# paultsw/wavenet-speech

Hardware: AMD Instinct MI355X
Metric: samples/sec fwd+bwd, 256-ch 30-block WaveNet @16k seq (higher is better)
Workload: dtype f32; 1 GPU; BASELINE.json configs[2]: WaveNet 256 ch, 30 blocks (3 x dilation 1..512), k=2, seq_len 16000, batch 16 per GPU, f32, full step (fwd+bwd+grad all-reduce+Adam); channels=256, blocks=30, seq_len=16000, batch_per_gpu=16, global_batch=16, parallelism=dp1, params=16037632, input=dense one-hot, init=reference

## Files before the change

include/wavenet_amd.h:

```cpp
#ifndef WAVENET_AMD_H
#define WAVENET_AMD_H

#include <stddef.h>

#ifdef __cplusplus
extern "C" {
#endif

#define WN_VERSION 300

typedef void* wn_stream_t;

typedef enum wn_status {
    WN_OK = 0,
    WN_ERR_BAD_SHAPE = -1,
    WN_ERR_UNSUPPORTED = -2,
    WN_ERR_NULL = -3,
    WN_ERR_HIP = -4,
    WN_ERR_WORKSPACE = -5
} wn_status;

#define WN_MAX_TAPS 8
#define WN_MAX_CHANNELS 1024

typedef struct wn_block_shape {
    int batch;
    int length;
    int in_channels;
    int out_channels;
    int skip_rows;
    int kernel_width;
    int dilation;
    int causal;
    int ld;
    int halo;
} wn_block_shape;

typedef struct wn_block_params {
    float* w_tanh;
    float* b_tanh;
    float* w_sigmoid;
    float* b_sigmoid;
    float* w_res;
    float* b_res;
    float* w_skip;
    float* b_skip;
    float* w_proj;
    float* b_proj;
} wn_block_params;

int wn_version(void);
const char* wn_strerror(int status);
const char* wn_last_hip_error(void);

int wn_round_up(int x, int multiple);
int wn_autopad(int kernel_width, int dilation);
int wn_tap_offsets(int kernel_width, int dilation, int causal, int* off );
int wn_series_layout(int length, int max_abs_offset, int* ld, int* halo);
size_t wn_series_floats(int batch, int channels, int ld);

size_t wn_block_packed_bytes(const wn_block_shape* s);
int wn_block_pack(const wn_block_shape* s, const wn_block_params* p, void* packed, wn_stream_t stream);

int wn_block_forward(const wn_block_shape* s, const void* packed, const float* x,
                     float* r_out, float* skip, int skip_accumulate,
                     float* sg, float* z, wn_stream_t stream);

#define WN_MAX_STACK_GROUP 32
typedef struct wn_skipsum_shape {
    int batch, length, skip_rows, nblocks, ld, halo;
    int channels[WN_MAX_STACK_GROUP];
} wn_skipsum_shape;
size_t wn_skipsum_packed_bytes(const wn_skipsum_shape* s);
int wn_skipsum_pack(const wn_skipsum_shape* s, const float* const* w_skip, const float* bias_total ,
                    void* packed, wn_stream_t stream);
int wn_skipsum_forward(const wn_skipsum_shape* s, const void* packed, const float* const* z, float* skip,
                       int accumulate, wn_stream_t stream);

int wn_block_backward_data(const wn_block_shape* s, const void* packed,
                           const float* dr, const float* dskip, const float* z, const float* sg,
                           float* da, float* dg, float* dx, wn_stream_t stream);

size_t wn_block_wgrad_workspace_bytes(const wn_block_shape* s);
int wn_block_backward_weights(const wn_block_shape* s, const float* x, const float* z,
                              const float* da, const float* dg, const float* dr, const float* dskip,
                              const wn_block_params* grads, void* workspace, size_t workspace_bytes,
                              wn_stream_t stream);

typedef struct wn_conv_shape {
    int batch, length, in_channels, out_channels, kernel_width, dilation, causal, ld, halo;
} wn_conv_shape;
size_t wn_conv_packed_bytes(const wn_conv_shape* s);
int wn_conv_pack(const wn_conv_shape* s, const float* weight , const float* bias ,
                 void* packed, wn_stream_t stream);
int wn_conv_forward(const wn_conv_shape* s, const void* packed, const float* x, float* y, wn_stream_t stream);
int wn_conv_backward_data(const wn_conv_shape* s, const void* packed, const float* dy, float* dx, wn_stream_t stream);
size_t wn_conv_wgrad_workspace_bytes(const wn_conv_shape* s);
int wn_conv_backward_weights(const wn_conv_shape* s, const float* x, const float* dy,
                             float* dweight, float* dbias ,
                             void* workspace, size_t workspace_bytes, wn_stream_t stream);

size_t wn_nll_partials(int batch, int length);
int wn_nll_forward(const float* logits, const long long* target, float* lse, float* partial, int* bad_targets,
                   int batch, int classes, int length, wn_stream_t stream);
int wn_nll_backward(const float* logits, const long long* target, const float* lse, const float* gscale, float* dlogits,
                    int batch, int classes, int length, wn_stream_t stream);

int wn_embed_forward(const long long* levels, const float* weight, const float* bias, float* y, int batch, int length,
                     int classes, int out_channels, int kernel_width, int* bad_levels, wn_stream_t stream);
size_t wn_synth_workspace_bytes(int batch, int length);
int wn_synth_bases(unsigned long long seed, int batch, int nbases, long long* bases, wn_stream_t stream);
int wn_synth_signal(const long long* bases, int batch, int nbases, int length, int upsampling, const double* means,
                    const double* stdvs, unsigned long long seed, const double* noise , double* picoamps,
                    void* workspace, size_t workspace_bytes, int* bad_bases , wn_stream_t stream);
int wn_synth_quantize(const double* picoamps, const void* workspace, size_t workspace_bytes, int batch, int length,
                      int num_levels, const double* edges, long long* levels, float* one_hot ,
                      wn_stream_t stream);

size_t wn_ctc_workspace_bytes(int batch, int classes, int length, int max_label_len);
int wn_ctc_loss(const float* logits, const long long* labels, const long long* label_lengths,
                const long long* input_lengths , int batch, int classes, int length, int max_label_len,
                int blank, float* nll, float* dlogits , void* workspace, size_t workspace_bytes,
                int* bad_labels , wn_stream_t stream);

size_t wn_ctc_decode_workspace_bytes(int batch, int classes, int length, int beam_width);
int wn_ctc_greedy_decode(const float* x, long long sb, long long sc, long long st, const long long* input_lengths ,
                         int batch, int classes, int length, int blank, int* labels, int* frames , int* lengths,
                         int* bad , wn_stream_t stream);
int wn_ctc_beam_decode(const float* x, long long sb, long long sc, long long st, int input_kind,
                       const long long* input_lengths , int batch, int classes, int length, int blank,
                       int beam_width, int* labels, int* frames , int* lengths, float* scores, void* workspace,
                       size_t workspace_bytes, int* bad , wn_stream_t stream);

size_t wn_ctc_align_workspace_bytes(int batch, int classes, int length, int max_label_len);
int wn_ctc_align(const float* x, long long sb, long long sc, long long st, int input_kind, const long long* labels,
                 const long long* label_lengths, const long long* input_lengths , int batch, int classes,
                 int length, int max_label_len, int blank, int* states, int* frame_labels ,
                 int* spans , float* score, void* workspace, size_t workspace_bytes, int* bad ,
                 wn_stream_t stream);

size_t wn_pair_align_workspace_bytes(int batch, int max_ref_len, int max_query_len);
int wn_pair_align(const int* ref, long long ref_stride, const int* ref_lengths, const int* query, long long query_stride,
                  const int* query_lengths, int batch, int max_ref_len, int max_query_len, int match, int mismatch,
                  int gap_open, int gap_extend, int end_gaps_free, int* score, int* stats ,
                  unsigned char* ops , int* ops_len , void* workspace, size_t workspace_bytes,
                  int* bad , wn_stream_t stream);

enum { WN_DWELL_FIXED = 0, WN_DWELL_UNIFORM = 1, WN_DWELL_GAMMA = 2 };
size_t wn_reads_workspace_bytes(int batch, int max_bases);
int wn_reads_plan(unsigned long long seed, int batch, int min_bases, int max_bases, int window, int dwell_model, double dwell_p0,
                  double dwell_p1, double dwell_p2, int max_dwell, const int* base_lengths_in ,
                  const int* bases_in , const int* dwell_in , int* base_lengths, int* bases,
                  int* dwell, int* starts, int* signal_lengths, void* workspace, size_t workspace_bytes,
                  int* bad , int* clamped , wn_stream_t stream);
int wn_reads_signal(const int* base_lengths, const int* starts, const int* signal_lengths, const void* workspace,
                    size_t workspace_bytes, int batch, int max_bases, int window, int ld, const double* means,
                    const double* stdvs, unsigned long long seed, const double* noise , float* signal,
                    int* sample_kmer , int* clipped_lengths , int* bad ,
                    wn_stream_t stream);

int wn_chunk_gather(const void* signal, int signal_is_int16, int batch, int ld, const int* signal_lengths,
                    const float* scale , const float* shift , const int* plan, int n_chunks,
                    int chunk, float* out, int* bad , wn_stream_t stream);
int wn_chunk_stitch(const float* y, long long stride_n, long long stride_c, long long stride_t, int y_frames, const int* plan,
                    int n_chunks, int classes, int batch, float* out, long long out_stride_b, long long out_stride_c,
                    int out_frames, const int* frame_lengths, int* bad , wn_stream_t stream);

size_t wn_read_select_workspace_bytes(int batch, int K, int signal_is_int16, int has_center);
int wn_read_select(const void* signal, int signal_is_int16, int batch, int ld, const int* signal_lengths, const int* ranks, int K,
                   const float* center , float* out, void* workspace, size_t workspace_bytes,
                   int* bad , wn_stream_t stream);

int wn_ctc_base_quality(const float* x, long long sb, long long sc, long long st, int input_kind,
                        const long long* input_lengths , const int* labels, long long labels_stride,
                        const int* frames, long long frames_stride, const int* lengths, int batch, int classes, int length,
                        int max_labels, int blank, int stat , float qscale, float qbias,
                        float* error , unsigned char* qual , int* dwell ,
                        float* read_error , int* bad , wn_stream_t stream);

int wn_quality_profile(const unsigned char* ops, long long ops_stride, const int* ops_len, const int* ref, long long ref_stride,
                       const int* ref_lengths, const int* query, long long query_stride, const int* query_lengths,
                       const unsigned char* qual , long long qual_stride, const int* dwell ,
                       long long dwell_stride, int batch, int max_ref_len, int max_query_len, int max_ops, int classes,
                       int count_ends, long long* q_counts , long long* dwell_counts ,
                       long long* confusion , int* read_counts ,
                       unsigned char* outcome , int* ref_index , int* bad ,
                       wn_stream_t stream);

typedef enum wn_precision { WN_F32 = 0, WN_F16X3 = 1, WN_F16 = 2, WN_BF16 = 3 } wn_precision;

int wn_hseries_layout(int length, int max_abs_offset, int* ld, int* halo);
size_t wn_hseries_bytes(int precision, int batch, int channels, int ld);
float wn_hseries_residual_scale(void);
int wn_hseries_load(int precision, const float* dense, void* series, int batch, int channels, int length, int ld, int halo,
                    float scale, const float* dyn_scale, unsigned* overflow_flag, wn_stream_t stream);

size_t wn_hblock_packed_bytes(const wn_block_shape* s, int precision);
int wn_hblock_pack(const wn_block_shape* s, int precision, const wn_block_params* p, void* packed, wn_stream_t stream);
int wn_hblock_pack_checked(const wn_block_shape* s, int precision, const wn_block_params* p, void* packed, unsigned* overflow_flag,
                           wn_stream_t stream);
int wn_hblock_forward_is_fused(const wn_block_shape* s, int precision);
int wn_hblock_forward(const wn_block_shape* s, int precision, const void* packed, const void* x, void* r_out,
                      float* skip_dense, int skip_accumulate, void* sg, void* z, unsigned* overflow_flag,
                      wn_stream_t stream);
size_t wn_hskipsum_packed_bytes(const wn_skipsum_shape* s, int precision);
int wn_hskipsum_pack(const wn_skipsum_shape* s, int precision, const float* const* w_skip, const float* bias_total,
                     void* packed, wn_stream_t stream);
int wn_hskipsum_forward(const wn_skipsum_shape* s, int precision, const void* packed, const void* const* z,
                        float* skip_dense, int accumulate, wn_stream_t stream);
int wn_hblock_backward_data(const wn_block_shape* s, int precision, const void* packed, const void* dr, const void* dskip,
                            const void* z, const void* sg, void* da, void* dg, void* dx, float* dx_dense,
                            const float* dyn_inv_scale, unsigned* overflow_flag, wn_stream_t stream);
size_t wn_hblock_wgrad_workspace_bytes(const wn_block_shape* s, int precision);
int wn_hblock_backward_weights(const wn_block_shape* s, int precision, const void* x, const void* z, const void* da,
                               const void* dg, const void* dr, const void* dskip, const wn_block_params* grads,
                               const float* dyn_inv_scale, void* workspace, size_t workspace_bytes, wn_stream_t stream);

int wn_hskipsum_forward_series(const wn_skipsum_shape* s, int precision, const void* packed, const void* const* z, void* out_series,
                               float out_scale, float leaky_slope, unsigned* overflow_flag, wn_stream_t stream);
int wn_hconv_forward_series(const wn_conv_shape* s, int precision, const void* packed, const void* x, void* y_series, float out_scale,
                            float leaky_slope, unsigned* overflow_flag, wn_stream_t stream);
int wn_hconv_backward_data_series(const wn_conv_shape* s, int precision, const void* packed, const void* dy, const void* act,
                                  float leaky_slope, void* dx_series, unsigned* overflow_flag, wn_stream_t stream);

int wn_hblock_backward_pair_is_fused(const wn_block_shape* upper, const wn_block_shape* lower, int precision);
int wn_hblock_backward_pair(const wn_block_shape* upper, const void* packed_upper, const wn_block_shape* lower, const void* packed_lower,
                            int precision, const void* dr_upper, const void* da_upper, const void* dg_upper, const void* dskip,
                            const void* z_lower, const void* sg_lower, void* dx_upper, void* da_lower, void* dg_lower,
                            unsigned* overflow_flag, wn_stream_t stream);
int wn_hblock_backward_input(const wn_block_shape* s, int precision, const void* packed, const void* dr, const void* da, const void* dg,
                             void* dx, float* dx_dense, const float* dyn_inv_scale, const void* x_act, float leaky_slope,
                             unsigned* overflow_flag, wn_stream_t stream);

int wn_hblock_backward_data_masked(const wn_block_shape* s, int precision, const void* packed, const void* dr, const void* dskip,
                                   const void* z, const void* sg, void* da, void* dg, void* dx, const void* x_act, float leaky_slope,
                                   unsigned* overflow_flag, wn_stream_t stream);

int wn_hfeature_forward(int precision, const float* x, const float* weight, const float* bias, void* y_series, int batch, int length,
                        int features, int kernel_width, int ld, int halo, float out_scale, float leaky_slope, unsigned* overflow_flag,
                        wn_stream_t stream);
size_t wn_hfeature_wgrad_workspace_bytes(int batch, int length, int features, int kernel_width);
int wn_hfeature_backward_weights(int precision, const float* x, const void* dy_series, float dy_scale, float* dweight, float* dbias,
                                 int batch, int length, int features, int kernel_width, int ld, int halo, const float* dyn_inv_scale,
                                 void* workspace, size_t workspace_bytes, wn_stream_t stream);
int wn_hseries_load_pooled(int precision, const float* dense, void* series, int batch, int channels, int length, int pool, int ld, int halo,
                           float scale, const float* dyn_scale, unsigned* overflow_flag, wn_stream_t stream);
int wn_series_load_pooled(const float* dense, float* series, int batch, int channels, int length, int pool, int ld, int halo,
                          wn_stream_t stream);
int wn_pool_backward(const float* dpooled, float* dx, int batch, int channels, int length, int pool, wn_stream_t stream);
int wn_grad_scale(const float* x, long long count, float target, float* scale_and_inverse, unsigned* accumulator, wn_stream_t stream);

int wn_hblocks_wgrad_group_max(const wn_block_shape* s, int precision);
size_t wn_hblocks_wgrad_workspace_bytes(const wn_block_shape* shapes, int nblocks, int precision);
int wn_hblocks_backward_weights(const wn_block_shape* shapes, int nblocks, int precision, const void* const* x, const void* const* z,
                                const void* const* da, const void* const* dg, const void* const* dr, const void* const* dskip,
                                const wn_block_params* grads, const float* dyn_inv_scale, void* workspace, size_t workspace_bytes,
                                wn_stream_t stream);

typedef struct wn_mem_range { const void* base; size_t bytes; } wn_mem_range;
size_t wn_hstack_pack_table_bytes(int nblocks);
int wn_hstack_pack_table_build(const wn_block_shape* shapes, const wn_block_params* params, int nblocks, int precision,
                               int with_skipsum, const wn_mem_range* dynamic, int ndynamic, void* table_host, size_t table_bytes,
                               size_t* block_offsets, size_t* skipsum_offsets, size_t* packed_total, int* njobs,
                               int* launch_blocks);
int wn_hstack_pack_run(const void* table_dev, int nblocks, int njobs, int launch_blocks, const void* const* dynamic_bases,
                       int ndynamic, void* packed, unsigned* overflow_flag , wn_stream_t stream);

int wn_prof_enable(int on);
int wn_prof_reset(void);
int wn_prof_collect(void);
int wn_prof_num_kernels(void);
const char* wn_prof_kernel_name(int kernel_class);
int wn_prof_get(int kernel_class, double* total_ms, long long* launches, double* flops);

size_t wn_hconv_packed_bytes(const wn_conv_shape* s, int precision);
int wn_hconv_pack(const wn_conv_shape* s, int precision, const float* weight , const float* bias ,
                  float input_scale, void* packed, wn_stream_t stream);
int wn_hconv_forward(const wn_conv_shape* s, int precision, const void* packed, const void* x, float* y_dense, wn_stream_t stream);
int wn_hconv_backward_data(const wn_conv_shape* s, int precision, const void* packed, const void* dy, float* dx_dense,
                           const float* dyn_inv_scale , wn_stream_t stream);
size_t wn_hconv_wgrad_workspace_bytes(const wn_conv_shape* s, int precision);
int wn_hconv_backward_weights(const wn_conv_shape* s, int precision, const void* x, const void* dy, float input_scale,
                              float* dweight, float* dbias , const float* dyn_inv_scale ,
                              void* workspace, size_t workspace_bytes, wn_stream_t stream);

#ifdef __cplusplus
}
#endif
#endif
```

wavenet_speech_amd/_lib.py:

```python
import ctypes
import os
from ctypes import POINTER, Structure, c_char_p, c_double, c_float, c_int, c_longlong, c_size_t, c_ulonglong, c_void_p

_HERE = os.path.dirname(os.path.abspath(__file__))
LIB_PATH = os.path.join(_HERE, "libwavenet_amd.so")

MAX_TAPS = 8
MAX_CHANNELS = 1024

c_float_p = c_void_p


class BlockShape(Structure):
    _fields_ = [("batch", c_int), ("length", c_int), ("in_channels", c_int), ("out_channels", c_int),
                ("skip_rows", c_int), ("kernel_width", c_int), ("dilation", c_int), ("causal", c_int),
                ("ld", c_int), ("halo", c_int)]


class BlockParams(Structure):
    _fields_ = [(n, c_float_p) for n in ("w_tanh", "b_tanh", "w_sigmoid", "b_sigmoid", "w_res", "b_res",
                                         "w_skip", "b_skip", "w_proj", "b_proj")]


MAX_STACK_GROUP = 32


class SkipSumShape(Structure):
    _fields_ = [("batch", c_int), ("length", c_int), ("skip_rows", c_int), ("nblocks", c_int), ("ld", c_int),
                ("halo", c_int), ("channels", c_int * MAX_STACK_GROUP)]


class MemRange(Structure):
    _fields_ = [("base", c_void_p), ("bytes", c_size_t)]


class ConvShape(Structure):
    _fields_ = [("batch", c_int), ("length", c_int), ("in_channels", c_int), ("out_channels", c_int),
                ("kernel_width", c_int), ("dilation", c_int), ("causal", c_int), ("ld", c_int), ("halo", c_int)]


SIGNATURES = {
    "wn_version": (c_int, []),
    "wn_strerror": (c_char_p, [c_int]),
    "wn_last_hip_error": (c_char_p, []),
    "wn_round_up": (c_int, [c_int, c_int]),
    "wn_autopad": (c_int, [c_int, c_int]),
    "wn_tap_offsets": (c_int, [c_int, c_int, c_int, POINTER(c_int)]),
    "wn_series_layout": (c_int, [c_int, c_int, POINTER(c_int), POINTER(c_int)]),
    "wn_series_floats": (c_size_t, [c_int, c_int, c_int]),
    "wn_block_packed_bytes": (c_size_t, [POINTER(BlockShape)]),
    "wn_block_pack": (c_int, [POINTER(BlockShape), POINTER(BlockParams), c_void_p, c_void_p]),
    "wn_block_forward": (c_int, [POINTER(BlockShape), c_void_p, c_float_p, c_float_p, c_float_p, c_int,
                                 c_float_p, c_float_p, c_void_p]),
    "wn_skipsum_packed_bytes": (c_size_t, [POINTER(SkipSumShape)]),
    "wn_skipsum_pack": (c_int, [POINTER(SkipSumShape), POINTER(c_void_p), c_float_p, c_void_p, c_void_p]),
    "wn_skipsum_forward": (c_int, [POINTER(SkipSumShape), c_void_p, POINTER(c_void_p), c_float_p, c_int, c_void_p]),
    "wn_block_backward_data": (c_int, [POINTER(BlockShape), c_void_p, c_float_p, c_float_p, c_float_p, c_float_p,
                                       c_float_p, c_float_p, c_float_p, c_void_p]),
    "wn_block_wgrad_workspace_bytes": (c_size_t, [POINTER(BlockShape)]),
    "wn_block_backward_weights": (c_int, [POINTER(BlockShape), c_float_p, c_float_p, c_float_p, c_float_p, c_float_p,
                                          c_float_p, POINTER(BlockParams), c_void_p, c_size_t, c_void_p]),
    "wn_conv_packed_bytes": (c_size_t, [POINTER(ConvShape)]),
    "wn_conv_pack": (c_int, [POINTER(ConvShape), c_float_p, c_float_p, c_void_p, c_void_p]),
    "wn_conv_forward": (c_int, [POINTER(ConvShape), c_void_p, c_float_p, c_float_p, c_void_p]),
    "wn_conv_backward_data": (c_int, [POINTER(ConvShape), c_void_p, c_float_p, c_float_p, c_void_p]),
    "wn_conv_wgrad_workspace_bytes": (c_size_t, [POINTER(ConvShape)]),
    "wn_conv_backward_weights": (c_int, [POINTER(ConvShape), c_float_p, c_float_p, c_float_p, c_float_p,
                                         c_void_p, c_size_t, c_void_p]),
    "wn_hseries_layout": (c_int, [c_int, c_int, POINTER(c_int), POINTER(c_int)]),
    "wn_hseries_bytes": (c_size_t, [c_int, c_int, c_int, c_int]),
    "wn_hseries_residual_scale": (c_float, []),
    "wn_hseries_load": (c_int, [c_int, c_float_p, c_void_p, c_int, c_int, c_int, c_int, c_int, c_float, c_float_p, c_void_p,
                                c_void_p]),
    "wn_hblock_packed_bytes": (c_size_t, [POINTER(BlockShape), c_int]),
    "wn_hblock_pack": (c_int, [POINTER(BlockShape), c_int, POINTER(BlockParams), c_void_p, c_void_p]),
    "wn_hblock_pack_checked": (c_int, [POINTER(BlockShape), c_int, POINTER(BlockParams), c_void_p, c_void_p, c_void_p]),
    "wn_hblock_forward_is_fused": (c_int, [POINTER(BlockShape), c_int]),
    "wn_hblock_backward_pair_is_fused": (c_int, [POINTER(BlockShape), POINTER(BlockShape), c_int]),
    "wn_hblock_backward_pair": (c_int, [POINTER(BlockShape), c_void_p, POINTER(BlockShape), c_void_p, c_int, c_void_p, c_void_p, c_void_p,
                                        c_void_p, c_void_p, c_void_p, c_void_p, c_void_p, c_void_p, c_void_p, c_void_p]),
    "wn_hblock_backward_input": (c_int, [POINTER(BlockShape), c_int, c_void_p, c_void_p, c_void_p, c_void_p, c_void_p, c_float_p, c_float_p,
                                         c_void_p, c_float, c_void_p, c_void_p]),
    "wn_hblock_forward": (c_int, [POINTER(BlockShape), c_int, c_void_p, c_void_p, c_void_p, c_float_p, c_int, c_void_p,
                                  c_void_p, c_void_p, c_void_p]),
    "wn_hskipsum_packed_bytes": (c_size_t, [POINTER(SkipSumShape), c_int]),
    "wn_hskipsum_pack": (c_int, [POINTER(SkipSumShape), c_int, POINTER(c_void_p), c_float_p, c_void_p, c_void_p]),
    "wn_hskipsum_forward": (c_int, [POINTER(SkipSumShape), c_int, c_void_p, POINTER(c_void_p), c_float_p, c_int, c_void_p]),
    "wn_hblock_backward_data": (c_int, [POINTER(BlockShape), c_int, c_void_p, c_void_p, c_void_p, c_void_p, c_void_p,
                                        c_void_p, c_void_p, c_void_p, c_float_p, c_float_p, c_void_p, c_void_p]),
    "wn_hblock_backward_data_masked": (c_int, [POINTER(BlockShape), c_int, c_void_p, c_void_p, c_void_p, c_void_p, c_void_p, c_void_p,
                                               c_void_p, c_void_p, c_void_p, c_float, c_void_p, c_void_p]),
    "wn_hfeature_forward": (c_int, [c_int, c_float_p, c_float_p, c_float_p, c_void_p, c_int, c_int, c_int, c_int, c_int, c_int, c_float,
                                    c_float, c_void_p, c_void_p]),
    "wn_hfeature_wgrad_workspace_bytes": (c_size_t, [c_int, c_int, c_int, c_int]),
    "wn_hfeature_backward_weights": (c_int, [c_int, c_float_p, c_void_p, c_float, c_float_p, c_float_p, c_int, c_int, c_int, c_int, c_int,
                                             c_int, c_float_p, c_void_p, c_size_t, c_void_p]),
    "wn_hseries_load_pooled": (c_int, [c_int, c_float_p, c_void_p, c_int, c_int, c_int, c_int, c_int, c_int, c_float, c_float_p, c_void_p,
                                       c_void_p]),
    "wn_series_load_pooled": (c_int, [c_float_p, c_float_p, c_int, c_int, c_int, c_int, c_int, c_int, c_void_p]),
    "wn_grad_scale": (c_int, [c_float_p, c_longlong, c_float, c_float_p, c_void_p, c_void_p]),
    "wn_pool_backward": (c_int, [c_float_p, c_float_p, c_int, c_int, c_int, c_int, c_void_p]),
    "wn_hskipsum_forward_series": (c_int, [POINTER(SkipSumShape), c_int, c_void_p, POINTER(c_void_p), c_void_p, c_float, c_float, c_void_p,
                                           c_void_p]),
    "wn_hconv_forward_series": (c_int, [POINTER(ConvShape), c_int, c_void_p, c_void_p, c_void_p, c_float, c_float, c_void_p, c_void_p]),
    "wn_hconv_backward_data_series": (c_int, [POINTER(ConvShape), c_int, c_void_p, c_void_p, c_void_p, c_float, c_void_p, c_void_p,
                                              c_void_p]),
    "wn_hblocks_wgrad_group_max": (c_int, [POINTER(BlockShape), c_int]),
    "wn_hblocks_wgrad_workspace_bytes": (c_size_t, [POINTER(BlockShape), c_int, c_int]),
    "wn_hblocks_backward_weights": (c_int, [POINTER(BlockShape), c_int, c_int, POINTER(c_void_p), POINTER(c_void_p), POINTER(c_void_p),
                                            POINTER(c_void_p), POINTER(c_void_p), POINTER(c_void_p), POINTER(BlockParams), c_float_p,
                                            c_void_p, c_size_t, c_void_p]),
    "wn_hstack_pack_table_bytes": (c_size_t, [c_int]),
    "wn_hstack_pack_table_build": (c_int, [POINTER(BlockShape), POINTER(BlockParams), c_int, c_int, c_int, POINTER(MemRange), c_int,
                                           c_void_p, c_size_t, POINTER(c_size_t), POINTER(c_size_t), POINTER(c_size_t),
                                           POINTER(c_int), POINTER(c_int)]),
    "wn_hstack_pack_run": (c_int, [c_void_p, c_int, c_int, c_int, POINTER(c_void_p), c_int, c_void_p, c_void_p, c_void_p]),
    "wn_hblock_wgrad_workspace_bytes": (c_size_t, [POINTER(BlockShape), c_int]),
    "wn_hblock_backward_weights": (c_int, [POINTER(BlockShape), c_int, c_void_p, c_void_p, c_void_p, c_void_p, c_void_p,
                                           c_void_p, POINTER(BlockParams), c_float_p, c_void_p, c_size_t, c_void_p]),
    "wn_hconv_packed_bytes": (c_size_t, [POINTER(ConvShape), c_int]),
    "wn_hconv_pack": (c_int, [POINTER(ConvShape), c_int, c_float_p, c_float_p, c_float, c_void_p, c_void_p]),
    "wn_hconv_forward": (c_int, [POINTER(ConvShape), c_int, c_void_p, c_void_p, c_float_p, c_void_p]),
    "wn_hconv_backward_data": (c_int, [POINTER(ConvShape), c_int, c_void_p, c_void_p, c_float_p, c_float_p, c_void_p]),
    "wn_hconv_wgrad_workspace_bytes": (c_size_t, [POINTER(ConvShape), c_int]),
    "wn_hconv_backward_weights": (c_int, [POINTER(ConvShape), c_int, c_void_p, c_void_p, c_float, c_float_p, c_float_p, c_float_p,
                                          c_void_p, c_size_t, c_void_p]),
    "wn_embed_forward": (c_int, [c_void_p, c_float_p, c_float_p, c_float_p, c_int, c_int, c_int, c_int, c_int, c_void_p, c_void_p]),
    "wn_synth_workspace_bytes": (c_size_t, [c_int, c_int]),
    "wn_synth_bases": (c_int, [c_ulonglong, c_int, c_int, c_void_p, c_void_p]),
    "wn_synth_signal": (c_int, [c_void_p, c_int, c_int, c_int, c_int, c_void_p, c_void_p, c_ulonglong, c_void_p, c_void_p,
                                c_void_p, c_size_t, c_void_p, c_void_p]),
    "wn_synth_quantize": (c_int, [c_void_p, c_void_p, c_size_t, c_int, c_int, c_int, c_void_p, c_void_p, c_void_p, c_void_p]),
    "wn_ctc_workspace_bytes": (c_size_t, [c_int, c_int, c_int, c_int]),
    "wn_ctc_loss": (c_int, [c_float_p, c_void_p, c_void_p, c_void_p, c_int, c_int, c_int, c_int, c_int, c_float_p, c_float_p,
                            c_void_p, c_size_t, c_void_p, c_void_p]),
    "wn_ctc_decode_workspace_bytes": (c_size_t, [c_int, c_int, c_int, c_int]),
    "wn_ctc_greedy_decode": (c_int, [c_float_p, c_longlong, c_longlong, c_longlong, c_void_p, c_int, c_int, c_int, c_int, c_void_p,
                                     c_void_p, c_void_p, c_void_p, c_void_p]),
    "wn_ctc_beam_decode": (c_int, [c_float_p, c_longlong, c_longlong, c_longlong, c_int, c_void_p, c_int, c_int, c_int, c_int, c_int,
                                   c_void_p, c_void_p, c_void_p, c_float_p, c_void_p, c_size_t, c_void_p, c_void_p]),
    "wn_ctc_align_workspace_bytes": (c_size_t, [c_int, c_int, c_int, c_int]),
    "wn_ctc_align": (c_int, [c_float_p, c_longlong, c_longlong, c_longlong, c_int, c_void_p, c_void_p, c_void_p, c_int, c_int, c_int,
                             c_int, c_int, c_void_p, c_void_p, c_void_p, c_float_p, c_void_p, c_size_t, c_void_p, c_void_p]),
    "wn_pair_align_workspace_bytes": (c_size_t, [c_int, c_int, c_int]),
    "wn_pair_align": (c_int, [c_void_p, c_longlong, c_void_p, c_void_p, c_longlong, c_void_p, c_int, c_int, c_int, c_int, c_int, c_int,
                              c_int, c_int, c_void_p, c_void_p, c_void_p, c_void_p, c_void_p, c_size_t, c_void_p, c_void_p]),
    "wn_reads_workspace_bytes": (c_size_t, [c_int, c_int]),
    "wn_reads_plan": (c_int, [c_ulonglong, c_int, c_int, c_int, c_int, c_int, c_double, c_double, c_double, c_int, c_void_p, c_void_p,
                              c_void_p, c_void_p, c_void_p, c_void_p, c_void_p, c_void_p, c_void_p, c_size_t, c_void_p, c_void_p,
                              c_void_p]),
    "wn_reads_signal": (c_int, [c_void_p, c_void_p, c_void_p, c_void_p, c_size_t, c_int, c_int, c_int, c_int, c_void_p, c_void_p,
                                c_ulonglong, c_void_p, c_void_p, c_void_p, c_void_p, c_void_p, c_void_p]),
    "wn_chunk_gather": (c_int, [c_void_p, c_int, c_int, c_int, c_void_p, c_void_p, c_void_p, c_void_p, c_int, c_int, c_void_p,
                                c_void_p, c_void_p]),
    "wn_chunk_stitch": (c_int, [c_void_p, c_longlong, c_longlong, c_longlong, c_int, c_void_p, c_int, c_int, c_int, c_void_p,
                                c_longlong, c_longlong, c_int, c_void_p, c_void_p, c_void_p]),
    "wn_read_select_workspace_bytes": (c_size_t, [c_int, c_int, c_int, c_int]),
    "wn_read_select": (c_int, [c_void_p, c_int, c_int, c_int, c_void_p, c_void_p, c_int, c_void_p, c_void_p, c_void_p, c_size_t,
                               c_void_p, c_void_p]),
    "wn_ctc_base_quality": (c_int, [c_float_p, c_longlong, c_longlong, c_longlong, c_int, c_void_p, c_void_p, c_longlong, c_void_p,
                                    c_longlong, c_void_p, c_int, c_int, c_int, c_int, c_int, c_int, c_float, c_float, c_float_p,
                                    c_void_p, c_void_p, c_float_p, c_void_p, c_void_p]),
    "wn_quality_profile": (c_int, [c_void_p, c_longlong, c_void_p, c_void_p, c_longlong, c_void_p, c_void_p, c_longlong, c_void_p,
                                   c_void_p, c_longlong, c_void_p, c_longlong, c_int, c_int, c_int, c_int, c_int, c_int, c_void_p,
                                   c_void_p, c_void_p, c_void_p, c_void_p, c_void_p, c_void_p, c_void_p]),
    "wn_nll_partials":(c_size_t, [c_int, c_int]),
    "wn_nll_forward": (c_int, [c_float_p, c_void_p, c_float_p, c_float_p, c_void_p, c_int, c_int, c_int, c_void_p]),
    "wn_nll_backward": (c_int, [c_float_p, c_void_p, c_float_p, c_float_p, c_float_p, c_int, c_int, c_int, c_void_p]),
    "wn_prof_enable": (c_int, [c_int]),
    "wn_prof_reset": (c_int, []),
    "wn_prof_collect": (c_int, []),
    "wn_prof_num_kernels": (c_int, []),
    "wn_prof_kernel_name": (c_char_p, [c_int]),
    "wn_prof_get": (c_int, [c_int, POINTER(c_double), POINTER(c_longlong), POINTER(c_double)]),
}

_lib = None


def load():
    global _lib
    if _lib is not None:
        return _lib
    if not os.path.exists(LIB_PATH):
        raise RuntimeError(
            "wavenet_speech_amd: %s not found. Build it with `python __graft_entry__.py` or "
            "`make -C wavenet_speech_amd/csrc` (hipcc, --offload-arch=gfx950). There is no CPU fallback." % LIB_PATH)
    lib = ctypes.CDLL(LIB_PATH)
    for name, (res, args) in SIGNATURES.items():
        fn = getattr(lib, name)
        fn.restype = res
        fn.argtypes = args
    if lib.wn_version() < 300:
        raise RuntimeError("libwavenet_amd.so too old")
    _lib = lib
    return lib


def check(status, what):
    if status != 0:
        lib = load()
        msg = lib.wn_strerror(status).decode()
        hip = lib.wn_last_hip_error().decode()
        raise RuntimeError("%s failed: %s%s" % (what, msg, (" [" + hip + "]") if hip and status == -4 else ""))


def tap_offsets(k, d, causal):
    off = (c_int * k)()
    check(load().wn_tap_offsets(k, d, int(bool(causal)), off), "wn_tap_offsets")
    return list(off)


def series_layout(length, max_abs_offset):
    ld, halo = c_int(), c_int()
    check(load().wn_series_layout(length, max_abs_offset, ctypes.byref(ld), ctypes.byref(halo)), "wn_series_layout")
    return ld.value, halo.value


PRECISIONS = {"f32": 0, "f16x3": 1, "f16": 2, "bf16": 3}


def hseries_layout(length, max_abs_offset):
    ld, halo = c_int(), c_int()
    check(load().wn_hseries_layout(length, max_abs_offset, ctypes.byref(ld), ctypes.byref(halo)), "wn_hseries_layout")
    return ld.value, halo.value


def profile_read():
    lib = load()
    check(lib.wn_prof_collect(), "wn_prof_collect")
    out = {}
    for i in range(lib.wn_prof_num_kernels()):
        ms, n, fl = c_double(), c_longlong(), c_double()
        check(lib.wn_prof_get(i, ctypes.byref(ms), ctypes.byref(n), ctypes.byref(fl)), "wn_prof_get")
        out[lib.wn_prof_kernel_name(i).decode()] = (ms.value, n.value, fl.value)
    return out
```

wavenet_speech_amd/csrc/wn_api.hip:

```cpp
#include <hip/hip_runtime.h>

#include <algorithm>
#include <cstdio>
#include <cstdlib>
#include <cstdint>
#include <cstring>
#include <mutex>
#include <string>
#include <vector>

#include "../../include/wavenet_amd.h"
#include "wn_kernels.h"

using namespace wn;

#ifdef WN_STAMPS
namespace wn { extern int g_debug_kc; }
#endif

namespace {

thread_local std::string g_hip_err;

int hip_fail(hipError_t e, const char* what) {
    g_hip_err = std::string(what) + ": " + hipGetErrorString(e);
    return WN_ERR_HIP;
}
#define WN_HIP(call, what)                                  \
    do {                                                    \
        hipError_t e__ = (call);                            \
        if (e__ != hipSuccess) return hip_fail(e__, what);  \
    } while (0)

}
namespace wn {
int hip_fail_shared(hipError_t e, const char* what) { return hip_fail(e, what); }
}
namespace {
inline int rup(int x, int m) { return (x + m - 1) / m * m; }
inline int cdiv(int a, int b) { return (a + b - 1) / b; }
inline int tiles32(int c) { return cdiv(c, 32); }
inline int cp8(int c) { return rup(c, 8); }
inline int pick_mt(int ntiles) { return ntiles > 2 ? 4 : (ntiles == 2 ? 2 : 1); }
inline size_t align256(size_t b) { return (b + 255) / 256 * 256; }

enum KernelClass {
    KC_PACK = 0, KC_GATE_GEMM, KC_OUT_GEMM, KC_DZ_GEMM, KC_DX_GEMM, KC_WGRAD, KC_WGRAD_REDUCE,
    KC_CONV_FWD, KC_CONV_BWD_DATA, KC_SKIP_GEMM, KC_HLOAD, KC_HGATE, KC_HRES, KC_HDZ, KC_HDX, KC_HSKIP, KC_HWGRAD, KC_EMBED,
    KC_SYNTH, KC_CTC, KC_HFUSED, KC_HCONV_FWD, KC_HCONV_BWD_DATA, KC_HCOL_DZ, KC_HCOL_DX, KC_HCOL_DXDZ, KC_HCOL_SKIP,
    KC_COUNT
};
const char* const kKernelNames[KC_COUNT] = {
    "pack_kernel", "series_gemm_kernel<gate>", "series_gemm_kernel<res>", "series_gemm_kernel<dz,dgate>",
    "series_gemm_kernel<dx>", "wgrad_kernel", "wgrad_reduce_kernel", "series_gemm_kernel<conv_fwd>",
    "series_gemm_kernel<conv_bwd_data>", "series_gemm_kernel<skips_sum>", "hload_kernel", "hgemm_kernel<gate>",
    "hgemm_kernel<res>", "hgemm_kernel<dz,dgate>", "hgemm_kernel<dx>", "hgemm_kernel<skips_sum>", "hwgrad_kernel",
    "embed_kernel", "synth_kernel", "ctc_kernel", "hfused_fwd_kernel",
    "hgemm_kernel<conv_fwd>", "hgemm_kernel<conv_bwd_data>", "hcol_kernel<dz,dgate>", "hcol_kernel<dx>", "hcol2_kernel<dx+dz>", "hcol_kernel<skips_sum>"};

struct ProfRec { int kc; hipEvent_t e0, e1; double flops; };
struct Prof {
    std::mutex mu;
    bool on = false;
    std::vector<ProfRec> pending;
    std::vector<hipEvent_t> pool;
    double ms[KC_COUNT] = {0};
    long long n[KC_COUNT] = {0};
    double flops[KC_COUNT] = {0};
} g_prof;

struct ProfScope {
    bool active = false;
    ProfRec rec{};
    hipStream_t st;
    ProfScope(int kc, double flops, hipStream_t s) : st(s) {
#ifdef WN_STAMPS
        wn::g_debug_kc = kc;
#endif
        std::lock_guard<std::mutex> lk(g_prof.mu);
        if (!g_prof.on) return;
        auto get = [&]() {
            hipEvent_t e;
            if (!g_prof.pool.empty()) { e = g_prof.pool.back(); g_prof.pool.pop_back(); return e; }
            if (hipEventCreate(&e) != hipSuccess) return (hipEvent_t) nullptr;
            return e;
        };
        rec.kc = kc; rec.flops = flops; rec.e0 = get(); rec.e1 = get();
        if (!rec.e0 || !rec.e1) return;
        active = hipEventRecord(rec.e0, st) == hipSuccess;
    }
    ~ProfScope() {
        if (!active) return;
        (void)hipEventRecord(rec.e1, st);
        std::lock_guard<std::mutex> lk(g_prof.mu);
        g_prof.pending.push_back(rec);
    }
};

}
namespace wn {
struct ProfScopeShared {
    void* impl;
    ProfScopeShared(int kc, double flops, hipStream_t st);
    ~ProfScopeShared();
};
ProfScopeShared::ProfScopeShared(int kc, double flops, hipStream_t st) : impl(new ProfScope(kc, flops, st)) {}
ProfScopeShared::~ProfScopeShared() { delete static_cast<ProfScope*>(impl); }
}
namespace {
int tap_offsets(int k, int d, int causal, int* off) {
    const int p = causal ? (k - 1) * d : wn_autopad(k, d);
    for (int j = 0; j < k; ++j) off[j] = j * d - p;
    return 0;
}

int check_layout(int B, int L, int ld, int halo, int max_abs_off) {
    if (B <= 0 || L <= 0) return WN_ERR_BAD_SHAPE;
    if (halo < 0 || (halo & 3) || (ld & 3)) return WN_ERR_BAD_SHAPE;
    if (halo < max_abs_off) return WN_ERR_BAD_SHAPE;
    if (ld < 2 * halo + rup(L, kColTile)) return WN_ERR_BAD_SHAPE;
    if ((double)WN_MAX_CHANNELS * (double)ld * 4.0 >= 4294967296.0) return WN_ERR_UNSUPPORTED;
    return WN_OK;
}

int check_block(const wn_block_shape* s, int* off) {
    if (!s) return WN_ERR_NULL;
    if (s->in_channels <= 0 || s->out_channels <= 0 || s->skip_rows <= 0 || s->dilation <= 0) return WN_ERR_BAD_SHAPE;
    if (s->kernel_width < 1) return WN_ERR_BAD_SHAPE;
    if (s->kernel_width > WN_MAX_TAPS) return WN_ERR_UNSUPPORTED;
    if (s->in_channels > WN_MAX_CHANNELS || s->out_channels > WN_MAX_CHANNELS || s->skip_rows > WN_MAX_CHANNELS)
        return WN_ERR_UNSUPPORTED;
    tap_offsets(s->kernel_width, s->dilation, s->causal, off);
    int mx = 0;
    for (int j = 0; j < s->kernel_width; ++j) mx = std::max(mx, std::abs(off[j]));
    return check_layout(s->batch, s->length, s->ld, s->halo, mx);
}

struct GemmPlan {
    int MT = 1, nslab = 0, nseg = 0;
    int seg_nkb[kMaxSeg] = {0};
    long long slab_woff[kMaxSlab] = {0};
    int slab_nseg[kMaxSlab] = {0}, slab_row0[kMaxSlab] = {0}, slab_dst[kMaxSlab] = {0}, slab_boff[kMaxSlab] = {0};
    long long wfloats = 0;
    int bfloats = 0;
    void add_slab(int nseg_used, int row0, int dst) {
        const int s = nslab++;
        long long kb = 0;
        for (int i = 0; i < nseg_used; ++i) kb += seg_nkb[i];
        slab_woff[s] = wfloats;
        slab_nseg[s] = nseg_used;
        slab_row0[s] = row0;
        slab_dst[s] = dst;
        slab_boff[s] = bfloats;
        wfloats += kb * MT * 256;
        bfloats += MT * 32;
    }
    size_t bytes() const { return align256((size_t)wfloats * 4) + align256((size_t)bfloats * 4); }
};

struct BlockPlan {
    GemmPlan fa, fb, ka, kb;
    int fb_first_skip_slab = 0;
    size_t off_fa = 0, off_fb = 0, off_ka = 0, off_kb = 0, total = 0;
};

BlockPlan plan_block(const wn_block_shape* s) {
    BlockPlan p;
    static const int mt2 = getenv("WN_MT2_MASK") ? atoi(getenv("WN_MT2_MASK")) : 0;
    const int Ci = s->in_channels, Co = s->out_channels, Ms = s->skip_rows, k = s->kernel_width;
    {
        GemmPlan& g = p.fa;
        const int pairs = tiles32(Co);
        g.MT = (pairs >= 2 && !(mt2 & 1)) ? 4 : 2;
        g.nseg = k;
        for (int j = 0; j < k; ++j) g.seg_nkb[j] = cp8(Ci) / 8;
        const int ns = cdiv(2 * pairs, g.MT);
        for (int i = 0; i < ns; ++i) g.add_slab(k, i * (g.MT / 2) * 32, 0);
    }
    {
        GemmPlan& g = p.fb;
        const int rt = tiles32(Co), st = tiles32(Ms);
        g.MT = pick_mt(std::max(rt, st));
        if ((mt2 & 2) && g.MT == 4) g.MT = 2;
        g.nseg = 2;
        g.seg_nkb[0] = cp8(Co) / 8;
        g.seg_nkb[1] = cp8(Ci) / 8;
        for (int i = 0; i < cdiv(rt, g.MT); ++i) g.add_slab(2, i * g.MT * 32, 0);
        p.fb_first_skip_slab = g.nslab;
        for (int i = 0; i < cdiv(st, g.MT); ++i) g.add_slab(1, i * g.MT * 32, 1);
    }
    {
        GemmPlan& g = p.ka;
        const int zt = tiles32(Co);
        g.MT = pick_mt(zt);
        static const int dz_mt = getenv("WN_DZ_MT") ? atoi(getenv("WN_DZ_MT")) : 2;
        if (dz_mt == 2 && zt >= 2) g.MT = 2;
        g.nseg = 2;
        g.seg_nkb[0] = cp8(Ms) / 8;
        g.seg_nkb[1] = cp8(Co) / 8;
        for (int i = 0; i < cdiv(zt, g.MT); ++i) g.add_slab(2, i * g.MT * 32, 0);
    }
    {
        GemmPlan& g = p.kb;
        const int xt = tiles32(Ci);
        g.MT = pick_mt(xt);
        if ((mt2 & 4) && g.MT == 4) g.MT = 2;
        g.nseg = 2 * k + 1;
        for (int j = 0; j < 2 * k + 1; ++j) g.seg_nkb[j] = cp8(Co) / 8;
        for (int i = 0; i < cdiv(xt, g.MT); ++i) g.add_slab(2 * k + 1, i * g.MT * 32, 0);
    }
    p.off_fa = 0;
    p.off_fb = p.off_fa + p.fa.bytes();
    p.off_ka = p.off_fb + p.fb.bytes();
    p.off_kb = p.off_ka + p.ka.bytes();
    p.total = p.off_kb + p.kb.bytes();
    return p;
}

inline const float* plan_w(const void* packed, size_t off) { return reinterpret_cast<const float*>((const char*)packed + off); }
inline const float* plan_b(const void* packed, size_t off, const GemmPlan& g) {
    return reinterpret_cast<const float*>((const char*)packed + off + align256((size_t)g.wfloats * 4));
}

void fill_pack_common(PackArgs& a, const GemmPlan& g, void* packed, size_t off) {
    std::memset(&a, 0, sizeof(a));
    a.nslab = g.nslab;
    a.MT = g.MT;
    for (int i = 0; i < kMaxSeg; ++i) a.seg_nkb[i] = g.seg_nkb[i];
    for (int i = 0; i < g.nslab; ++i) {
        a.slab_woff[i] = g.slab_woff[i];
        a.slab_nseg[i] = g.slab_nseg[i];
        a.slab_boff[i] = g.slab_boff[i];
    }
    a.wpacked = reinterpret_cast<float*>((char*)packed + off);
    a.bias = reinterpret_cast<float*>((char*)packed + off + align256((size_t)g.wfloats * 4));
    a.total = g.wfloats;
}

void fill_gemm_common(GemmArgs& a, const GemmPlan& g, const void* packed, size_t off, int first_slab, int nslab,
                      int B, int L, int ld, int halo) {
    std::memset(&a, 0, sizeof(a));
    a.wpacked = plan_w(packed, off);
    a.bias = plan_b(packed, off, g);
    a.nslab = nslab;
    for (int i = 0; i < nslab; ++i) {
        GemmSlab& s = a.slab[i];
        s.woff = g.slab_woff[first_slab + i];
        s.nseg = g.slab_nseg[first_slab + i];
        s.dst = g.slab_dst[first_slab + i];
        s.row0 = g.slab_row0[first_slab + i];
        s.boff = g.slab_boff[first_slab + i];
    }
    a.B = B; a.L = L; a.ld = ld; a.halo = halo;
    a.tiles_per_row = cdiv(L, kColTile);
    a.ncol = B * a.tiles_per_row;
}

inline void set_seg(GemmArgs& a, int i, const float* base, int c, int off, int nkb) {
    a.seg[i].base = base; a.seg[i].cp = cp8(c); a.seg[i].off = off; a.seg[i].nkb = nkb;
}

inline PackSrc mk_src(const float* p, int rows, int cols, int sr, int sc) {
    PackSrc s; s.ptr = p; s.rows = rows; s.cols = cols; s.stride_r = sr; s.stride_c = sc; return s;
}

struct WgradPlan {
    int WT = 1, npair = 0, ntile_total = 0, nsplit = 1;
    int Mp[kMaxPair], Np[kMaxPair], mt[kMaxPair], nt[kMaxPair], tile0[kMaxPair], rs_off[kMaxPair];
    long long slab_off[kMaxPair];
    long long slab_floats = 0;
    int rs_floats = 0;
    void add(int M, int N) {
        const int T = 64 * WT, i = npair++;
        mt[i] = cdiv(M, T); nt[i] = cdiv(N, T);
        Mp[i] = mt[i] * T; Np[i] = nt[i] * T;
        tile0[i] = ntile_total; ntile_total += mt[i] * nt[i];
        slab_off[i] = slab_floats; slab_floats += (long long)Mp[i] * Np[i];
        rs_off[i] = rs_floats; rs_floats += Mp[i];
    }
    void finish(int nchunk) {
        nsplit = std::max(1, 512 / std::max(1, ntile_total));
        nsplit = std::min(nsplit, std::max(1, nchunk));
        if (nsplit >= 16) nsplit = nsplit / 8 * 8;
    }
    bool xcd_map() const { return nsplit % 8 == 0; }
    size_t bytes() const { return (size_t)nsplit * (size_t)(slab_floats + rs_floats) * 4; }
};
inline int pick_wt(int maxdim) { return maxdim > 128 ? 4 : (maxdim > 64 ? 2 : 1); }

}


int wn_version(void) { return WN_VERSION; }

const char* wn_strerror(int status) {
    switch (status) {
        case WN_OK: return "ok";
        case WN_ERR_BAD_SHAPE: return "bad shape or series layout (dimension <= 0, ld/halo not multiples of 4, halo smaller than the taps reach, or ld too small)";
        case WN_ERR_UNSUPPORTED: return "unsupported configuration (kernel_width > WN_MAX_TAPS or channels > WN_MAX_CHANNELS)";
        case WN_ERR_NULL: return "required pointer is NULL";
        case WN_ERR_HIP: return "HIP runtime / kernel launch error (see wn_last_hip_error)";
        case WN_ERR_WORKSPACE: return "workspace too small";
    }
    return "unknown wn_status";
}

const char* wn_last_hip_error(void) { return g_hip_err.c_str(); }

int wn_round_up(int x, int multiple) { return multiple > 0 ? rup(x, multiple) : x; }

int wn_autopad(int k, int d) {
    const int total = (k - 1) * d;
    return (total % 2 == 1) ? (total - 1) / 2 + 1 : total / 2;
}

int wn_tap_offsets(int k, int d, int causal, int* off) {
    if (!off) return WN_ERR_NULL;
    if (k < 1 || d < 1) return WN_ERR_BAD_SHAPE;
    return tap_offsets(k, d, causal, off);
}

int wn_series_layout(int length, int max_abs_offset, int* ld, int* halo) {
    if (!ld || !halo) return WN_ERR_NULL;
    if (length <= 0 || max_abs_offset < 0) return WN_ERR_BAD_SHAPE;
    *halo = rup(max_abs_offset, 4);
    *ld = 2 * (*halo) + rup(length, kColTile);
    return WN_OK;
}

size_t wn_series_floats(int batch, int channels, int ld) { return (size_t)batch * cp8(channels) * (size_t)ld; }

size_t wn_block_packed_bytes(const wn_block_shape* s) {
    int off[WN_MAX_TAPS];
    if (check_block(s, off) != WN_OK) return 0;
    return plan_block(s).total;
}

int wn_block_pack(const wn_block_shape* s, const wn_block_params* p, void* packed, wn_stream_t stream) {
    int off[WN_MAX_TAPS];
    int rc = check_block(s, off);
    if (rc != WN_OK) return rc;
    if (!p || !packed || !p->w_tanh || !p->w_sigmoid || !p->w_res || !p->w_skip || !p->w_proj) return WN_ERR_NULL;
    hipStream_t st = (hipStream_t)stream;
    const BlockPlan bp = plan_block(s);
    const int Ci = s->in_channels, Co = s->out_channels, Ms = s->skip_rows, k = s->kernel_width;
    ProfScope prof(KC_PACK, 0.0, st);
    PackArgs a;
    {
        const GemmPlan& g = bp.fa;
        fill_pack_common(a, g, packed, bp.off_fa);
        for (int j = 0; j < k; ++j) {
            a.set[0].seg[j] = mk_src(p->w_tanh + j, Co, Ci, Ci * k, k);
            a.set[1].seg[j] = mk_src(p->w_sigmoid + j, Co, Ci, Ci * k, k);
        }
        a.set[0].bias0 = p->b_tanh; a.set[0].bias_rows = Co;
        a.set[1].bias0 = p->b_sigmoid; a.set[1].bias_rows = Co;
        const int pairs = tiles32(Co);
        for (int sl = 0; sl < g.nslab; ++sl)
            for (int m = 0; m < g.MT; ++m) {
                const int pair = sl * (g.MT / 2) + m / 2;
                a.tile[sl * g.MT + m].set = m & 1;
                a.tile[sl * g.MT + m].row0 = pair < pairs ? 32 * pair : -1;
            }
        WN_HIP(launch_pack(a, st), "pack(gate)");
    }
    {
        const GemmPlan& g = bp.fb;
        fill_pack_common(a, g, packed, bp.off_fb);
        a.set[0].seg[0] = mk_src(p->w_res, Co, Co, Co, 1);
        a.set[0].seg[1] = mk_src(p->w_proj, Co, Ci, Ci, 1);
        a.set[0].bias0 = p->b_res; a.set[0].bias1 = p->b_proj; a.set[0].bias_rows = Co;
        a.set[1].seg[0] = mk_src(p->w_skip, Ms, Co, Co, 1);
        a.set[1].bias0 = p->b_skip; a.set[1].bias_rows = Ms;
        for (int sl = 0; sl < g.nslab; ++sl)
            for (int m = 0; m < g.MT; ++m) {
                const bool skip = sl >= bp.fb_first_skip_slab;
                const int row0 = g.slab_row0[sl] + 32 * m;
                a.tile[sl * g.MT + m].set = skip ? 1 : 0;
                a.tile[sl * g.MT + m].row0 = row0 < (skip ? Ms : Co) ? row0 : -1;
            }
        WN_HIP(launch_pack(a, st), "pack(res+skip)");
    }
    {
        const GemmPlan& g = bp.ka;
        fill_pack_common(a, g, packed, bp.off_ka);
        a.set[0].seg[0] = mk_src(p->w_skip, Co, Ms, 1, Co);
        a.set[0].seg[1] = mk_src(p->w_res, Co, Co, 1, Co);
        for (int sl = 0; sl < g.nslab; ++sl)
            for (int m = 0; m < g.MT; ++m) {
                const int row0 = g.slab_row0[sl] + 32 * m;
                a.tile[sl * g.MT + m].set = 0;
                a.tile[sl * g.MT + m].row0 = row0 < Co ? row0 : -1;
            }
        WN_HIP(launch_pack(a, st), "pack(dz)");
    }
    {
        const GemmPlan& g = bp.kb;
        fill_pack_common(a, g, packed, bp.off_kb);
        for (int j = 0; j < k; ++j) {
            a.set[0].seg[2 * j] = mk_src(p->w_tanh + j, Ci, Co, k, Ci * k);
            a.set[0].seg[2 * j + 1] = mk_src(p->w_sigmoid + j, Ci, Co, k, Ci * k);
        }
        a.set[0].seg[2 * k] = mk_src(p->w_proj, Ci, Co, 1, Ci);
        for (int sl = 0; sl < g.nslab; ++sl)
            for (int m = 0; m < g.MT; ++m) {
                const int row0 = g.slab_row0[sl] + 32 * m;
                a.tile[sl * g.MT + m].set = 0;
                a.tile[sl * g.MT + m].row0 = row0 < Ci ? row0 : -1;
            }
        WN_HIP(launch_pack(a, st), "pack(dx)");
    }
    return WN_OK;
}

int wn_block_forward(const wn_block_shape* s, const void* packed, const float* x, float* r_out, float* skip,
                     int skip_accumulate, float* sg, float* z, wn_stream_t stream) {
    int off[WN_MAX_TAPS];
    int rc = check_block(s, off);
    if (rc != WN_OK) return rc;
    if (!packed || !x || !z) return WN_ERR_NULL;
    hipStream_t st = (hipStream_t)stream;
    const BlockPlan bp = plan_block(s);
    const int Ci = s->in_channels, Co = s->out_channels, Ms = s->skip_rows, k = s->kernel_width;
    const double BL = (double)s->batch * s->length;
    GemmArgs a;
    {
        const GemmPlan& g = bp.fa;
        fill_gemm_common(a, g, packed, bp.off_fa, 0, g.nslab, s->batch, s->length, s->ld, s->halo);
        for (int j = 0; j < k; ++j) set_seg(a, j, x, Ci, off[j], g.seg_nkb[j]);
        a.sg = sg; a.z = z; a.gate_cp = cp8(Co); a.gate_rows = Co;
        ProfScope prof(KC_GATE_GEMM, 2.0 * (2.0 * Co) * (double)(k * Ci) * BL, st);
        WN_HIP(launch_gemm(g.MT, EPI_GATE, a, st), "series_gemm<gate>");
    }
    {
        const GemmPlan& g = bp.fb;
        const double fl_r = 2.0 * Co * (double)(Co + Ci) * BL, fl_s = 2.0 * Ms * (double)Co * BL;
        if (r_out) {
            fill_gemm_common(a, g, packed, bp.off_fb, 0, bp.fb_first_skip_slab, s->batch, s->length, s->ld, s->halo);
            set_seg(a, 0, z, Co, 0, g.seg_nkb[0]);
            set_seg(a, 1, x, Ci, 0, g.seg_nkb[1]);
            a.dst[0].base = r_out; a.dst[0].cp = cp8(Co); a.dst[0].rows = Co; a.dst[0].accumulate = 0;
            ProfScope prof(KC_OUT_GEMM, fl_r, st);
            WN_HIP(launch_gemm(g.MT, EPI_LINEAR, a, st), "series_gemm<res>");
        }
        if (skip) {
            fill_gemm_common(a, g, packed, bp.off_fb, bp.fb_first_skip_slab, g.nslab - bp.fb_first_skip_slab, s->batch,
                             s->length, s->ld, s->halo);
            set_seg(a, 0, z, Co, 0, g.seg_nkb[0]);
            a.dst[1].base = skip; a.dst[1].cp = cp8(Ms); a.dst[1].rows = Ms; a.dst[1].accumulate = skip_accumulate ? 1 : 0;
            ProfScope prof(KC_SKIP_GEMM, fl_s, st);
            WN_HIP(launch_gemm(g.MT, skip_accumulate ? EPI_ACCUM : EPI_LINEAR, a, st), "series_gemm<skip>");
        }
    }
    return WN_OK;
}

int wn_block_backward_data(const wn_block_shape* s, const void* packed, const float* dr, const float* dskip,
                           const float* z, const float* sg, float* da, float* dg, float* dx, wn_stream_t stream) {
    int off[WN_MAX_TAPS];
    int rc = check_block(s, off);
    if (rc != WN_OK) return rc;
    if (!packed || !dskip || !z || !sg || !da || !dg) return WN_ERR_NULL;
    hipStream_t st = (hipStream_t)stream;
    const BlockPlan bp = plan_block(s);
    const int Ci = s->in_channels, Co = s->out_channels, Ms = s->skip_rows, k = s->kernel_width;
    const double BL = (double)s->batch * s->length;
    GemmArgs a;
    {
        const GemmPlan& g = bp.ka;
        fill_gemm_common(a, g, packed, bp.off_ka, 0, g.nslab, s->batch, s->length, s->ld, s->halo);
        a.bias = nullptr;
        set_seg(a, 0, dskip, Ms, 0, g.seg_nkb[0]);
        set_seg(a, 1, dr, Co, 0, g.seg_nkb[1]);
        const int nseg = dr ? 2 : 1;
        for (int i = 0; i < a.nslab; ++i) a.slab[i].nseg = nseg;
        a.z = const_cast<float*>(z); a.sg = const_cast<float*>(sg); a.da = da; a.dg = dg;
        a.gate_cp = cp8(Co); a.gate_rows = Co;
        ProfScope prof(KC_DZ_GEMM, 2.0 * Co * (double)(Ms + (dr ? Co : 0)) * BL, st);
        WN_HIP(launch_gemm(g.MT, EPI_DGATE, a, st), "series_gemm<dz>");
    }
    if (dx) {
        const GemmPlan& g = bp.kb;
        fill_gemm_common(a, g, packed, bp.off_kb, 0, g.nslab, s->batch, s->length, s->ld, s->halo);
        a.bias = nullptr;
        for (int j = 0; j < k; ++j) {
            set_seg(a, 2 * j, da, Co, -off[j], g.seg_nkb[2 * j]);
            set_seg(a, 2 * j + 1, dg, Co, -off[j], g.seg_nkb[2 * j + 1]);
        }
        set_seg(a, 2 * k, dr, Co, 0, g.seg_nkb[2 * k]);
        const int nseg = 2 * k + (dr ? 1 : 0);
        for (int i = 0; i < a.nslab; ++i) a.slab[i].nseg = nseg;
        a.dst[0].base = dx; a.dst[0].cp = cp8(Ci); a.dst[0].rows = Ci; a.dst[0].accumulate = 0;
        ProfScope prof(KC_DX_GEMM, 2.0 * Ci * (double)(2 * k * Co + (dr ? Co : 0)) * BL, st);
        WN_HIP(launch_gemm(g.MT, EPI_LINEAR, a, st), "series_gemm<dx>");
    }
    return WN_OK;
}

namespace {
int check_skipsum(const wn_skipsum_shape* s) {
    if (!s) return WN_ERR_NULL;
    if (s->nblocks < 1 || s->skip_rows <= 0) return WN_ERR_BAD_SHAPE;
    if (s->nblocks > WN_MAX_STACK_GROUP || s->skip_rows > WN_MAX_CHANNELS) return WN_ERR_UNSUPPORTED;
    for (int l = 0; l < s->nblocks; ++l) {
        if (s->channels[l] <= 0) return WN_ERR_BAD_SHAPE;
        if (s->channels[l] > WN_MAX_CHANNELS) return WN_ERR_UNSUPPORTED;
    }
    return check_layout(s->batch, s->length, s->ld, s->halo, 0);
}
GemmPlan plan_skipsum(const wn_skipsum_shape* s) {
    GemmPlan g;
    const int t = tiles32(s->skip_rows);
    g.MT = pick_mt(t);
    g.nseg = s->nblocks;
    for (int l = 0; l < s->nblocks; ++l) g.seg_nkb[l] = cp8(s->channels[l]) / 8;
    for (int i = 0; i < cdiv(t, g.MT); ++i) g.add_slab(s->nblocks, i * g.MT * 32, 0);
    return g;
}
}

size_t wn_skipsum_packed_bytes(const wn_skipsum_shape* s) {
    if (check_skipsum(s) != WN_OK) return 0;
    return plan_skipsum(s).bytes();
}

int wn_skipsum_pack(const wn_skipsum_shape* s, const float* const* w_skip, const float* bias_total, void* packed,
                    wn_stream_t stream) {
    int rc = check_skipsum(s);
    if (rc != WN_OK) return rc;
    if (!w_skip || !packed) return WN_ERR_NULL;
    for (int l = 0; l < s->nblocks; ++l) if (!w_skip[l]) return WN_ERR_NULL;
    hipStream_t st = (hipStream_t)stream;
    const GemmPlan g = plan_skipsum(s);
    ProfScope prof(KC_PACK, 0.0, st);
    PackArgs a;
    fill_pack_common(a, g, packed, 0);
    for (int l = 0; l < s->nblocks; ++l) a.set[0].seg[l] = mk_src(w_skip[l], s->skip_rows, s->channels[l], s->channels[l], 1);
    a.set[0].bias0 = bias_total; a.set[0].bias_rows = s->skip_rows;
    for (int sl = 0; sl < g.nslab; ++sl)
        for (int m = 0; m < g.MT; ++m) {
            const int row0 = g.slab_row0[sl] + 32 * m;
            a.tile[sl * g.MT + m].set = 0;
            a.tile[sl * g.MT + m].row0 = row0 < s->skip_rows ? row0 : -1;
        }
    WN_HIP(launch_pack(a, st), "pack(skipsum)");
    return WN_OK;
}

int wn_skipsum_forward(const wn_skipsum_shape* s, const void* packed, const float* const* z, float* skip, int accumulate,
                       wn_stream_t stream) {
    int rc = check_skipsum(s);
    if (rc != WN_OK) return rc;
    if (!packed || !z || !skip) return WN_ERR_NULL;
    for (int l = 0; l < s->nblocks; ++l) if (!z[l]) return WN_ERR_NULL;
    hipStream_t st = (hipStream_t)stream;
    const GemmPlan g = plan_skipsum(s);
    GemmArgs a;
    fill_gemm_common(a, g, packed, 0, 0, g.nslab, s->batch, s->length, s->ld, s->halo);
    double ksum = 0;
    for (int l = 0; l < s->nblocks; ++l) { set_seg(a, l, z[l], s->channels[l], 0, g.seg_nkb[l]); ksum += s->channels[l]; }
    a.dst[0].base = skip; a.dst[0].cp = cp8(s->skip_rows); a.dst[0].rows = s->skip_rows; a.dst[0].accumulate = accumulate ? 1 : 0;
    ProfScope prof(KC_SKIP_GEMM, 2.0 * s->skip_rows * ksum * (double)s->batch * s->length, st);
    WN_HIP(launch_gemm(g.MT, accumulate ? EPI_ACCUM : EPI_LINEAR, a, st), "series_gemm<skipsum>");
    return WN_OK;
}

namespace {
struct PairSpec { const float* A; int a_rows; const float* Bm; int b_rows; int off; int rowsum;
                  float* w; int sm, sn; float* b0; float* b1; };

int run_wgrad(const std::vector<PairSpec>& ps, int maxdim, int B, int L, int ld, int halo, void* workspace,
              size_t workspace_bytes, bool dry, size_t* need, int kc, hipStream_t st) {
    WgradPlan wp;
    wp.WT = pick_wt(maxdim);
    for (const PairSpec& p : ps) wp.add(p.a_rows, p.b_rows);
    const int cpr = cdiv(L, 32);
    wp.finish(B * cpr);
    if (need) *need = wp.bytes();
    if (dry) return WN_OK;
    for (const PairSpec& p : ps)
        if ((double)cp8(std::max(p.a_rows, p.b_rows)) * (double)ld * 4.0 >= 4294967296.0) return WN_ERR_UNSUPPORTED;
    if (ps.empty()) return WN_OK;
    if (!workspace) return WN_ERR_NULL;
    if (workspace_bytes < wp.bytes() || (reinterpret_cast<uintptr_t>(workspace) & 15)) return WN_ERR_WORKSPACE;
    WgradArgs a;
    std::memset(&a, 0, sizeof(a));
    ReduceArgs r;
    std::memset(&r, 0, sizeof(r));
    double flops = 0;
    for (int i = 0; i < wp.npair; ++i) {
        WgradPair& q = a.pair[i];
        q.A = ps[i].A; q.Bm = ps[i].Bm; q.a_cp = cp8(ps[i].a_rows); q.b_cp = cp8(ps[i].b_rows);
        q.off = ps[i].off; q.mt = wp.mt[i]; q.nt = wp.nt[i]; q.tile0 = wp.tile0[i];
        q.slab_off = wp.slab_off[i]; q.Mp = wp.Mp[i]; q.Np = wp.Np[i];
        q.rowsum = ps[i].rowsum; q.rs_off = wp.rs_off[i];
        ReduceDst& d = r.d[i];
        d.w = ps[i].w; d.M = ps[i].a_rows; d.N = ps[i].b_rows; d.sm = ps[i].sm; d.sn = ps[i].sn;
        d.slab_off = wp.slab_off[i]; d.Np = wp.Np[i];
        d.b0 = ps[i].rowsum ? ps[i].b0 : nullptr; d.b1 = ps[i].rowsum ? ps[i].b1 : nullptr; d.rs_off = wp.rs_off[i];
        d.post = 1.0f;
        flops += 2.0 * ps[i].a_rows * (double)ps[i].b_rows * (double)B * L;
    }
    a.npair = wp.npair; a.ntile_total = wp.ntile_total; a.nsplit = wp.nsplit; a.xcd_map = wp.xcd_map() ? 1 : 0;
    a.B = B; a.L = L; a.ld = ld; a.halo = halo; a.chunks_per_row = cpr; a.nchunk = B * cpr;
    a.slab = reinterpret_cast<float*>(workspace);
    a.rowsum = a.slab + (size_t)wp.nsplit * wp.slab_floats;
    a.slab_floats = wp.slab_floats; a.rs_floats = wp.rs_floats;
    r.npair = wp.npair; r.nsplit = wp.nsplit; r.slab = a.slab; r.rowsum = a.rowsum;
    r.slab_floats = wp.slab_floats; r.rs_floats = wp.rs_floats;
    {
        ProfScope prof(kc, flops, st);
        WN_HIP(launch_wgrad(wp.WT, a, st), "wgrad");
    }
    {
        ProfScope prof(KC_WGRAD_REDUCE, 0.0, st);
        WN_HIP(launch_wgrad_reduce(r, st), "wgrad_reduce");
    }
    return WN_OK;
}

std::vector<PairSpec> block_pairs(const wn_block_shape* s, const int* off, const float* x, const float* z,
                                  const float* da, const float* dg, const float* dr, const float* dskip,
                                  const wn_block_params* g) {
    const int Ci = s->in_channels, Co = s->out_channels, Ms = s->skip_rows, k = s->kernel_width;
    std::vector<PairSpec> ps;
    for (int j = 0; j < k; ++j) {
        ps.push_back({da, Co, x, Ci, off[j], j == 0, g ? g->w_tanh + j : nullptr, Ci * k, k, g ? g->b_tanh : nullptr, nullptr});
        ps.push_back({dg, Co, x, Ci, off[j], j == 0, g ? g->w_sigmoid + j : nullptr, Ci * k, k, g ? g->b_sigmoid : nullptr, nullptr});
    }
    ps.push_back({dskip, Ms, z, Co, 0, 1, g ? g->w_skip : nullptr, Co, 1, g ? g->b_skip : nullptr, nullptr});
    if (dr) {
        ps.push_back({dr, Co, z, Co, 0, 1, g ? g->w_res : nullptr, Co, 1, g ? g->b_res : nullptr, g ? g->b_proj : nullptr});
        ps.push_back({dr, Co, x, Ci, 0, 0, g ? g->w_proj : nullptr, Ci, 1, nullptr, nullptr});
    }
    return ps;
}
}

size_t wn_block_wgrad_workspace_bytes(const wn_block_shape* s) {
    int off[WN_MAX_TAPS];
    if (check_block(s, off) != WN_OK) return 0;
    static const float dummy = 0;
    size_t need = 0;
    for (int with_dr = 0; with_dr < 2; ++with_dr) {
        std::vector<PairSpec> ps = block_pairs(s, off, &dummy, &dummy, &dummy, &dummy, with_dr ? &dummy : nullptr, &dummy, nullptr);
        size_t n = 0;
        run_wgrad(ps, std::max(std::max(s->in_channels, s->out_channels), s->skip_rows), s->batch, s->length, s->ld,
                  s->halo, nullptr, 0, true, &n, KC_WGRAD, nullptr);
        need = std::max(need, n);
    }
    return need;
}

int wn_block_backward_weights(const wn_block_shape* s, const float* x, const float* z, const float* da, const float* dg,
                              const float* dr, const float* dskip, const wn_block_params* grads, void* workspace,
                              size_t workspace_bytes, wn_stream_t stream) {
    int off[WN_MAX_TAPS];
    int rc = check_block(s, off);
    if (rc != WN_OK) return rc;
    if (!x || !z || !da || !dg || !dskip || !grads) return WN_ERR_NULL;
    if (!grads->w_tanh || !grads->b_tanh || !grads->w_sigmoid || !grads->b_sigmoid || !grads->w_skip || !grads->b_skip)
        return WN_ERR_NULL;
    if (dr && (!grads->w_res || !grads->b_res || !grads->w_proj || !grads->b_proj)) return WN_ERR_NULL;
    hipStream_t st = (hipStream_t)stream;
    const int Ci = s->in_channels, Co = s->out_channels;
    if (!dr) {
        if (grads->w_res) WN_HIP(hipMemsetAsync(grads->w_res, 0, (size_t)Co * Co * 4, st), "memset dW_res");
        if (grads->b_res) WN_HIP(hipMemsetAsync(grads->b_res, 0, (size_t)Co * 4, st), "memset db_res");
        if (grads->w_proj) WN_HIP(hipMemsetAsync(grads->w_proj, 0, (size_t)Co * Ci * 4, st), "memset dW_proj");
        if (grads->b_proj) WN_HIP(hipMemsetAsync(grads->b_proj, 0, (size_t)Co * 4, st), "memset db_proj");
    }
    std::vector<PairSpec> ps = block_pairs(s, off, x, z, da, dg, dr, dskip, grads);
    return run_wgrad(ps, std::max(std::max(Ci, Co), s->skip_rows), s->batch, s->length, s->ld, s->halo, workspace,
                     workspace_bytes, false, nullptr, KC_WGRAD, st);
}

namespace {
int check_conv(const wn_conv_shape* s, int* off) {
    if (!s) return WN_ERR_NULL;
    if (s->in_channels <= 0 || s->out_channels <= 0 || s->dilation <= 0 || s->kernel_width < 1) return WN_ERR_BAD_SHAPE;
    if (s->kernel_width > WN_MAX_TAPS) return WN_ERR_UNSUPPORTED;
    if (s->in_channels > WN_MAX_CHANNELS || s->out_channels > WN_MAX_CHANNELS) return WN_ERR_UNSUPPORTED;
    tap_offsets(s->kernel_width, s->dilation, s->causal, off);
    int mx = 0;
    for (int j = 0; j < s->kernel_width; ++j) mx = std::max(mx, std::abs(off[j]));
    return check_layout(s->batch, s->length, s->ld, s->halo, mx);
}
struct ConvPlan { GemmPlan cf, cb; size_t off_cf = 0, off_cb = 0, total = 0; };
ConvPlan plan_conv(const wn_conv_shape* s) {
    ConvPlan p;
    const int Ci = s->in_channels, Co = s->out_channels, k = s->kernel_width;
    {
        GemmPlan& g = p.cf;
        const int t = tiles32(Co);
        g.MT = pick_mt(t); g.nseg = k;
        for (int j = 0; j < k; ++j) g.seg_nkb[j] = cp8(Ci) / 8;
        for (int i = 0; i < cdiv(t, g.MT); ++i) g.add_slab(k, i * g.MT * 32, 0);
    }
    {
        GemmPlan& g = p.cb;
        const int t = tiles32(Ci);
        g.MT = pick_mt(t); g.nseg = k;
        for (int j = 0; j < k; ++j) g.seg_nkb[j] = cp8(Co) / 8;
        for (int i = 0; i < cdiv(t, g.MT); ++i) g.add_slab(k, i * g.MT * 32, 0);
    }
    p.off_cf = 0; p.off_cb = p.cf.bytes(); p.total = p.off_cb + p.cb.bytes();
    return p;
}
}

size_t wn_conv_packed_bytes(const wn_conv_shape* s) {
    int off[WN_MAX_TAPS];
    if (check_conv(s, off) != WN_OK) return 0;
    return plan_conv(s).total;
}

int wn_conv_pack(const wn_conv_shape* s, const float* weight, const float* bias, void* packed, wn_stream_t stream) {
    int off[WN_MAX_TAPS];
    int rc = check_conv(s, off);
    if (rc != WN_OK) return rc;
    if (!weight || !packed) return WN_ERR_NULL;
    hipStream_t st = (hipStream_t)stream;
    const ConvPlan cp = plan_conv(s);
    const int Ci = s->in_channels, Co = s->out_channels, k = s->kernel_width;
    ProfScope prof(KC_PACK, 0.0, st);
    PackArgs a;
    {
        const GemmPlan& g = cp.cf;
        fill_pack_common(a, g, packed, cp.off_cf);
        for (int j = 0; j < k; ++j) a.set[0].seg[j] = mk_src(weight + j, Co, Ci, Ci * k, k);
        a.set[0].bias0 = bias; a.set[0].bias_rows = Co;
        for (int sl = 0; sl < g.nslab; ++sl)
            for (int m = 0; m < g.MT; ++m) {
                const int row0 = g.slab_row0[sl] + 32 * m;
                a.tile[sl * g.MT + m].set = 0;
                a.tile[sl * g.MT + m].row0 = row0 < Co ? row0 : -1;
            }
        WN_HIP(launch_pack(a, st), "pack(conv fwd)");
    }
    {
        const GemmPlan& g = cp.cb;
        fill_pack_common(a, g, packed, cp.off_cb);
        for (int j = 0; j < k; ++j) a.set[0].seg[j] = mk_src(weight + j, Ci, Co, k, Ci * k);
        for (int sl = 0; sl < g.nslab; ++sl)
            for (int m = 0; m < g.MT; ++m) {
                const int row0 = g.slab_row0[sl] + 32 * m;
                a.tile[sl * g.MT + m].set = 0;
                a.tile[sl * g.MT + m].row0 = row0 < Ci ? row0 : -1;
            }
        WN_HIP(launch_pack(a, st), "pack(conv bwd)");
    }
    return WN_OK;
}

int wn_conv_forward(const wn_conv_shape* s, const void* packed, const float* x, float* y, wn_stream_t stream) {
    int off[WN_MAX_TAPS];
    int rc = check_conv(s, off);
    if (rc != WN_OK) return rc;
    if (!packed || !x || !y) return WN_ERR_NULL;
    hipStream_t st = (hipStream_t)stream;
    const ConvPlan cp = plan_conv(s);
    const GemmPlan& g = cp.cf;
    GemmArgs a;
    fill_gemm_common(a, g, packed, cp.off_cf, 0, g.nslab, s->batch, s->length, s->ld, s->halo);
    for (int j = 0; j < s->kernel_width; ++j) set_seg(a, j, x, s->in_channels, off[j], g.seg_nkb[j]);
    a.dst[0].base = y; a.dst[0].cp = cp8(s->out_channels); a.dst[0].rows = s->out_channels; a.dst[0].accumulate = 0;
    ProfScope prof(KC_CONV_FWD, 2.0 * s->out_channels * (double)(s->kernel_width * s->in_channels) * s->batch * s->length, st);
    WN_HIP(launch_gemm(g.MT, EPI_LINEAR, a, st), "series_gemm<conv fwd>");
    return WN_OK;
}

int wn_conv_backward_data(const wn_conv_shape* s, const void* packed, const float* dy, float* dx, wn_stream_t stream) {
    int off[WN_MAX_TAPS];
    int rc = check_conv(s, off);
    if (rc != WN_OK) return rc;
    if (!packed || !dy || !dx) return WN_ERR_NULL;
    hipStream_t st = (hipStream_t)stream;
    const ConvPlan cp = plan_conv(s);
    const GemmPlan& g = cp.cb;
    GemmArgs a;
    fill_gemm_common(a, g, packed, cp.off_cb, 0, g.nslab, s->batch, s->length, s->ld, s->halo);
    a.bias = nullptr;
    for (int j = 0; j < s->kernel_width; ++j) set_seg(a, j, dy, s->out_channels, -off[j], g.seg_nkb[j]);
    a.dst[0].base = dx; a.dst[0].cp = cp8(s->in_channels); a.dst[0].rows = s->in_channels; a.dst[0].accumulate = 0;
    ProfScope prof(KC_CONV_BWD_DATA, 2.0 * s->in_channels * (double)(s->kernel_width * s->out_channels) * s->batch * s->length, st);
    WN_HIP(launch_gemm(g.MT, EPI_LINEAR, a, st), "series_gemm<conv bwd>");
    return WN_OK;
}

namespace {
std::vector<PairSpec> conv_pairs(const wn_conv_shape* s, const int* off, const float* x, const float* dy, float* dw, float* db) {
    std::vector<PairSpec> ps;
    const int Ci = s->in_channels, Co = s->out_channels, k = s->kernel_width;
    for (int j = 0; j < k; ++j)
        ps.push_back({dy, Co, x, Ci, off[j], (j == 0 && db) ? 1 : 0, dw ? dw + j : nullptr, Ci * k, k, db, nullptr});
    return ps;
}
}

size_t wn_conv_wgrad_workspace_bytes(const wn_conv_shape* s) {
    int off[WN_MAX_TAPS];
    if (check_conv(s, off) != WN_OK) return 0;
    static const float dummy = 0;
    std::vector<PairSpec> ps = conv_pairs(s, off, &dummy, &dummy, nullptr, nullptr);
    size_t need = 0;
    run_wgrad(ps, std::max(s->in_channels, s->out_channels), s->batch, s->length, s->ld, s->halo, nullptr, 0, true, &need,
              KC_WGRAD, nullptr);
    return need;
}

int wn_conv_backward_weights(const wn_conv_shape* s, const float* x, const float* dy, float* dweight, float* dbias,
                             void* workspace, size_t workspace_bytes, wn_stream_t stream) {
    int off[WN_MAX_TAPS];
    int rc = check_conv(s, off);
    if (rc != WN_OK) return rc;
    if (!x || !dy || !dweight) return WN_ERR_NULL;
    std::vector<PairSpec> ps = conv_pairs(s, off, x, dy, dweight, dbias);
    return run_wgrad(ps, std::max(s->in_channels, s->out_channels), s->batch, s->length, s->ld, s->halo, workspace,
                     workspace_bytes, false, nullptr, KC_WGRAD, (hipStream_t)stream);
}

size_t wn_nll_partials(int batch, int length) {
    if (batch <= 0 || length <= 0) return 0;
    return (size_t)(((long long)batch * ((length + 3) / 4) + 255) / 256);
}

int wn_nll_forward(const float* logits, const long long* target, float* lse, float* partial, int* bad_targets, int batch,
                   int classes, int length, wn_stream_t stream) {
    if (batch <= 0 || classes <= 0 || length <= 0) return WN_ERR_BAD_SHAPE;
    if (!logits || !target || !lse || !partial) return WN_ERR_NULL;
    WN_HIP(launch_nll_forward(logits, target, lse, partial, bad_targets, batch, classes, length, (hipStream_t)stream), "nll_forward");
    return WN_OK;
}

int wn_nll_backward(const float* logits, const long long* target, const float* lse, const float* gscale, float* dlogits,
                    int batch, int classes, int length, wn_stream_t stream) {
    if (batch <= 0 || classes <= 0 || length <= 0) return WN_ERR_BAD_SHAPE;
    if (!logits || !target || !lse || !gscale || !dlogits) return WN_ERR_NULL;
    WN_HIP(launch_nll_backward(logits, target, lse, gscale, dlogits, batch, classes, length, (hipStream_t)stream), "nll_backward");
    return WN_OK;
}

int wn_prof_enable(int on) {
    std::lock_guard<std::mutex> lk(g_prof.mu);
    g_prof.on = on != 0;
    return WN_OK;
}

int wn_prof_reset(void) {
    std::lock_guard<std::mutex> lk(g_prof.mu);
    for (ProfRec& r : g_prof.pending) { g_prof.pool.push_back(r.e0); g_prof.pool.push_back(r.e1); }
    g_prof.pending.clear();
    for (int i = 0; i < KC_COUNT; ++i) { g_prof.ms[i] = 0; g_prof.n[i] = 0; g_prof.flops[i] = 0; }
    return WN_OK;
}

int wn_prof_collect(void) {
    std::lock_guard<std::mutex> lk(g_prof.mu);
    for (ProfRec& r : g_prof.pending) {
        WN_HIP(hipEventSynchronize(r.e1), "hipEventSynchronize");
        float ms = 0;
        WN_HIP(hipEventElapsedTime(&ms, r.e0, r.e1), "hipEventElapsedTime");
        g_prof.ms[r.kc] += ms; g_prof.n[r.kc] += 1; g_prof.flops[r.kc] += r.flops;
        g_prof.pool.push_back(r.e0); g_prof.pool.push_back(r.e1);
    }
    g_prof.pending.clear();
    return WN_OK;
}

int wn_prof_num_kernels(void) { return KC_COUNT; }
const char* wn_prof_kernel_name(int kc) { return (kc >= 0 && kc < KC_COUNT) ? kKernelNames[kc] : ""; }

int wn_prof_get(int kc, double* total_ms, long long* launches, double* flops) {
    if (kc < 0 || kc >= KC_COUNT) return WN_ERR_BAD_SHAPE;
    std::lock_guard<std::mutex> lk(g_prof.mu);
    if (total_ms) *total_ms = g_prof.ms[kc];
    if (launches) *launches = g_prof.n[kc];
    if (flops) *flops = g_prof.flops[kc];
    return WN_OK;
}
```

wavenet_speech_amd/csrc/wn_gemm.hip:

```cpp
#include <cstdlib>

#include "wn_kernels.h"

namespace wn {

__device__ __forceinline__ int rowof(int r, int h) { return (r & 3) + 8 * (r >> 2) + 4 * h; }

__device__ __forceinline__ float sigmoid_f(float x) {
    const float e = __builtin_amdgcn_exp2f(-1.44269504088896341f * x);
    return __builtin_amdgcn_rcpf(1.0f + e);
}
__device__ __forceinline__ float tanh_f(float x) {
    const float ax = __builtin_fabsf(x);
    const float e = __builtin_amdgcn_exp2f(-2.88539008177792681f * ax);
    const float big = (1.0f - e) * __builtin_amdgcn_rcpf(1.0f + e);
    const float x2 = x * x;
    const float small = ax * (1.0f + x2 * (-0.333333333f + x2 * (0.133333333f + x2 * -0.0539682540f)));
    return __builtin_copysignf(ax < 0.125f ? small : big, x);
}

template <int NT> struct BVec;
template <> struct BVec<4> { typedef f32x4 reg_t; };
template <> struct BVec<2> { typedef float __attribute__((ext_vector_type(2))) reg_t; };

template <int MT, int NT, int EPI, int PFB, int WPS>
__global__ __launch_bounds__(64, WPS) void series_gemm_kernel(const GemmArgs a) {
    typedef typename BVec<NT>::reg_t breg_t;
    constexpr int COLS = 32 * NT;
    const int lane = threadIdx.x;
    const int n0 = lane & 31, h0 = lane >> 5;
#ifdef WN_STAMPS
    const unsigned long long st_t0 = __builtin_amdgcn_s_memtime(), st_r0 = __builtin_amdgcn_s_memrealtime();
    unsigned long long st_t1 = 0, st_t2 = 0;
#endif

    const int id = blockIdx.x;
    const int xcd = id & 7, local = id >> 3;
    const int slab_i = local % a.nslab;
    const int coltile = (local / a.nslab) * 8 + xcd;
    if (coltile >= a.ncol) return;
    const int b = coltile / a.tiles_per_row;
    const int t0 = (coltile - b * a.tiles_per_row) * COLS;
    const GemmSlab sl = a.slab[slab_i];
    const int ld = a.ld;

    f32x16 acc[MT][NT];
    const float* bias_p = (a.bias ? a.bias : a.wpacked) + sl.boff;
    const float bias_on = a.bias ? 1.0f : 0.0f;
#pragma unroll
    for (int m = 0; m < MT; ++m) {
#pragma unroll
        for (int r = 0; r < 16; ++r) {
            const float bv = bias_p[32 * m + rowof(r, h0)] * bias_on;
#pragma unroll
            for (int t = 0; t < NT; ++t) acc[m][t][r] = bv;
        }
    }

    int nkb = 0;
    for (int s = 0; s < sl.nseg; ++s) nkb += a.seg[s].nkb;

    constexpr unsigned kRsrcFlags = 0x00020000u;
    auto resource = [&](const float* base) {
        return __builtin_amdgcn_make_buffer_rsrc(const_cast<float*>(base), 0, 0xffffffffu, kRsrcFlags);
    };
    const __amdgpu_buffer_rsrc_t wrs = resource(a.wpacked + sl.woff);
    const unsigned a_off = lane * 16u;
    unsigned a_soff = 0;
    const long tilebase = (long)a.halo + t0;
    unsigned b_off[4];
#pragma unroll
    for (int q = 0; q < 4; ++q) b_off[q] = 4u * ((unsigned)(4 * h0 + q) * (unsigned)ld + (unsigned)(NT * n0));
    int seg = 0;
    int seg_left = a.seg[0].nkb;
    __amdgpu_buffer_rsrc_t brs = resource(a.seg[0].base + (long)b * a.seg[0].cp * ld);
    unsigned b_soff = 4u * (unsigned)(tilebase + a.seg[0].off);
    int b_left = nkb;
    const unsigned a_last = (unsigned)(nkb > 0 ? nkb - 1 : 0) * (MT * 1024u);

    f32x4 A[2][MT];
    breg_t B[4][4];
    auto loadA = [&](f32x4 (&dst)[MT]) {
#pragma unroll
        for (int m = 0; m < MT; ++m)
            dst[m] = __builtin_bit_cast(f32x4, __builtin_amdgcn_raw_buffer_load_b128(wrs, a_off + m * 1024u, a_soff, 0));
        a_soff = min(a_soff + MT * 1024u, a_last);
    };
    auto loadB = [&](breg_t (&dst)[4]) {
#pragma unroll
        for (int q = 0; q < 4; ++q) {
            if constexpr (NT == 4) dst[q] = __builtin_bit_cast(breg_t, __builtin_amdgcn_raw_buffer_load_b128(brs, b_off[q], b_soff, 0));
            else dst[q] = __builtin_bit_cast(breg_t, __builtin_amdgcn_raw_buffer_load_b64(brs, b_off[q], b_soff, 0));
        }
        const int more = min(b_left - 1, 1);
        b_left -= more;
        b_soff += (unsigned)more * (32u * (unsigned)ld);
        seg_left -= more;
        if (b_left > 1 - more && seg_left == 0) {
            ++seg;
            const GemmSeg ns = a.seg[seg];
            seg_left = ns.nkb;
            brs = resource(ns.base + (long)b * ns.cp * ld);
            b_soff = 4u * (unsigned)(tilebase + ns.off);
        }
    };
    auto compute = [&](const f32x4 (&fa)[MT], const breg_t (&fb)[4]) {
#pragma unroll
        for (int q = 0; q < 4; ++q)
#pragma unroll
            for (int m = 0; m < MT; ++m)
#pragma unroll
                for (int t = 0; t < NT; ++t)
                    acc[m][t] = __builtin_amdgcn_mfma_f32_32x32x2f32(fa[m][q], fb[q][t], acc[m][t], 0, 0, 0);
    };

    loadA(A[0]);
#pragma unroll
    for (int p = 0; p < PFB; ++p) loadB(B[p]);
#ifdef WN_STAMPS
    __builtin_amdgcn_sched_barrier(0);
    st_t1 = __builtin_amdgcn_s_memtime();
    __builtin_amdgcn_sched_barrier(0);
#endif
    int g0 = 0;
    for (; g0 + 4 <= nkb; g0 += 4) {
#pragma unroll
        for (int j = 0; j < 4; ++j) {
            loadA(A[(j + 1) & 1]);
            loadB(B[(j + PFB) & 3]);
            __builtin_amdgcn_sched_barrier(0);
            compute(A[j & 1], B[j & 3]);
            __builtin_amdgcn_sched_barrier(0);
        }
    }
#pragma unroll
    for (int j = 0; j < 3; ++j) {
        if (g0 + j < nkb) {
            loadA(A[(j + 1) & 1]);
            loadB(B[(j + PFB) & 3]);
            __builtin_amdgcn_sched_barrier(0);
            compute(A[j & 1], B[j & 3]);
            __builtin_amdgcn_sched_barrier(0);
        }
    }

#ifdef WN_STAMPS
    __builtin_amdgcn_sched_barrier(0);
    st_t2 = __builtin_amdgcn_s_memtime();
    __builtin_amdgcn_sched_barrier(0);
    struct StampOut {
        unsigned long long* p; unsigned long long t0, r0, t1, t2; int lane;
        __device__ ~StampOut() {
            __builtin_amdgcn_sched_barrier(0);
            const unsigned long long t_issued = __builtin_amdgcn_s_memtime();
            __builtin_amdgcn_sched_barrier(0);
            asm volatile("s_waitcnt vmcnt(0)" ::: "memory");
            if (p && lane == 0) {
                p[0] = t0; p[1] = t1; p[2] = t2; p[3] = __builtin_amdgcn_s_memtime();
                p[4] = r0; p[5] = __builtin_amdgcn_s_memrealtime();
                p[6] = __builtin_amdgcn_s_getreg(63492);
                p[7] = (unsigned long long)__builtin_amdgcn_s_getreg(63508) | ((t_issued - t2) << 32);
            }
        }
    } stamp_out{a.stamps ? a.stamps + 8ull * blockIdx.x : nullptr, st_t0, st_r0, st_t1, st_t2, lane};
#endif
    const int lane_e = (int)__builtin_amdgcn_mbcnt_hi(~0u, __builtin_amdgcn_mbcnt_lo(~0u, 0u));
    const int n = lane_e & 31, h = lane_e >> 5;
    const long colbase = tilebase + NT * n;
    const int c0 = t0 + NT * n;
    if (c0 >= a.L) return;
    auto clip = [&](breg_t v) {
#pragma unroll
        for (int t = 1; t < NT; ++t)
            if (c0 + t >= a.L) v[t] = 0.0f;
        return v;
    };

    if constexpr (EPI == EPI_LINEAR) {
        const GemmDst d = a.dst[sl.dst];
#pragma unroll
        for (int m = 0; m < MT; ++m) {
#pragma unroll
            for (int r = 0; r < 16; ++r) {
                const int row = sl.row0 + 32 * m + rowof(r, h);
                if (row < d.rows) {
                    float* p = d.base + ((long)b * d.cp + row) * ld + colbase;
                    breg_t v;
#pragma unroll
                    for (int t = 0; t < NT; ++t) v[t] = acc[m][t][r];
                    *reinterpret_cast<breg_t*>(p) = clip(v);
                }
            }
            __builtin_amdgcn_sched_barrier(0);
        }
    } else if constexpr (EPI == EPI_ACCUM) {
        const GemmDst d = a.dst[sl.dst];
        constexpr int RB = 8, BPT = 16 / RB, NBATCH = MT * BPT;
        breg_t old[2][RB];
        float* const tile = d.base + (long)b * d.cp * ld + colbase;
        auto fetch = [&](int bi, breg_t (&dst)[RB]) {
            const int m = bi / BPT, r0 = (bi % BPT) * RB;
#pragma unroll
            for (int i = 0; i < RB; ++i) {
                int row = sl.row0 + 32 * m + rowof(r0 + i, h);
                row = row < d.rows ? row : d.rows - 1;
                dst[i] = *reinterpret_cast<const breg_t*>(tile + (long)row * ld);
            }
        };
        fetch(0, old[0]);
#pragma unroll
        for (int bi = 0; bi < NBATCH; ++bi) {
            if (bi + 1 < NBATCH) fetch(bi + 1, old[(bi + 1) & 1]);
            __builtin_amdgcn_sched_barrier(0);
            const int m = bi / BPT, r0 = (bi % BPT) * RB;
#pragma unroll
            for (int i = 0; i < RB; ++i) {
                const int row = sl.row0 + 32 * m + rowof(r0 + i, h);
                if (row < d.rows) {
                    breg_t v;
#pragma unroll
                    for (int t = 0; t < NT; ++t) v[t] = acc[m][t][r0 + i] + old[bi & 1][i][t];
                    *reinterpret_cast<breg_t*>(tile + (long)row * ld) = clip(v);
                }
            }
            __builtin_amdgcn_sched_barrier(0);
        }
    } else if constexpr (EPI == EPI_GATE) {
#pragma unroll
        for (int i = 0; i < MT / 2; ++i) {
#pragma unroll
            for (int r = 0; r < 16; ++r) {
                const int ch = sl.row0 + 32 * i + rowof(r, h);
                if (ch < a.gate_rows) {
                    breg_t vs, vz;
#pragma unroll
                    for (int t = 0; t < NT; ++t) {
                        const float tt = tanh_f(acc[2 * i][t][r]);
                        const float ss = sigmoid_f(acc[2 * i + 1][t][r]);
                        vs[t] = ss;
                        vz[t] = tt * ss;
                    }
                    const long o = ((long)b * a.gate_cp + ch) * ld + colbase;
                    *reinterpret_cast<breg_t*>(a.z + o) = clip(vz);
                    if (a.sg) *reinterpret_cast<breg_t*>(a.sg + o) = clip(vs);
                }
            }
            __builtin_amdgcn_sched_barrier(0);
        }
    } else {
        constexpr int RB = (MT == 4) ? 8 : 4;
        constexpr int BPT = 16 / RB;
        constexpr int NBATCH = MT * BPT;
        breg_t vt[2][RB], vs[2][RB];
        auto fetch = [&](int bi, breg_t (&ft)[RB], breg_t (&fs)[RB]) {
            const int m = bi / BPT, r0 = (bi % BPT) * RB;
#pragma unroll
            for (int i = 0; i < RB; ++i) {
                int ch = sl.row0 + 32 * m + rowof(r0 + i, h);
                ch = ch < a.gate_rows ? ch : a.gate_rows - 1;
                const long o = ((long)b * a.gate_cp + ch) * ld + colbase;
                ft[i] = *reinterpret_cast<const breg_t*>(a.z + o);
                fs[i] = *reinterpret_cast<const breg_t*>(a.sg + o);
            }
        };
        fetch(0, vt[0], vs[0]);
#pragma unroll
        for (int bi = 0; bi < NBATCH; ++bi) {
            if (bi + 1 < NBATCH) fetch(bi + 1, vt[(bi + 1) & 1], vs[(bi + 1) & 1]);
            __builtin_amdgcn_sched_barrier(0);
            const int m = bi / BPT, r0 = (bi % BPT) * RB;
#pragma unroll
            for (int i = 0; i < RB; ++i) {
                const int r = r0 + i;
                const int ch = sl.row0 + 32 * m + rowof(r, h);
                if (ch < a.gate_rows) {
                    const long o = ((long)b * a.gate_cp + ch) * ld + colbase;
                    const breg_t z_ = vt[bi & 1][i], sg_ = vs[bi & 1][i];
                    breg_t va, vg;
#pragma unroll
                    for (int t = 0; t < NT; ++t) {
                        const float dz = acc[m][t][r];
                        const float tt = sg_[t] > 0.0f ? z_[t] / sg_[t] : 0.0f;
                        va[t] = dz * (sg_[t] - z_[t] * tt);
                        vg[t] = dz * z_[t] * (1.0f - sg_[t]);
                    }
                    *reinterpret_cast<breg_t*>(a.da + o) = clip(va);
                    *reinterpret_cast<breg_t*>(a.dg + o) = clip(vg);
                }
            }
            __builtin_amdgcn_sched_barrier(0);
        }
    }
}

#ifdef WN_STAMPS
static unsigned long long* g_stamp_buf = nullptr;
static int g_stamp_kc = -1;
int g_debug_kc = -1;
extern "C" void wn_debug_set_stamp_buffer(void* p) { g_stamp_buf = (unsigned long long*)p; }
extern "C" void wn_debug_set_stamp_class(int kc) { g_stamp_kc = kc; }
extern "C" unsigned wn_debug_last_grid = 0;
#endif

template <int MT, int NT, int EPI, int PFB, int WPS>
static hipError_t launch_one(GemmArgs a, hipStream_t st) {
#ifdef WN_STAMPS
    const bool stamp_this = g_stamp_buf && (g_stamp_kc < 0 || g_stamp_kc == g_debug_kc);
    a.stamps = stamp_this ? g_stamp_buf : nullptr;
#endif
    a.tiles_per_row = (a.L + 32 * NT - 1) / (32 * NT);
    a.ncol = a.B * a.tiles_per_row;
    const int ncol8 = (a.ncol + 7) / 8 * 8;
    const unsigned grid = (unsigned)(a.nslab * ncol8);
#ifdef WN_STAMPS
    if (stamp_this) wn_debug_last_grid = grid;
#endif
    hipLaunchKernelGGL((series_gemm_kernel<MT, NT, EPI, PFB, WPS>), dim3(grid), dim3(64), 0, st, a);
    return hipGetLastError();
}

static int gemm_variant() {
    static int v = -1;
    if (v < 0) {
        const char* e = getenv("WN_GEMM_VARIANT");
        v = e ? atoi(e) : 0;
    }
    return v;
}

template <int EPI>
static hipError_t launch_epi(int MT, const GemmArgs& a, hipStream_t st) {
    const int v = gemm_variant();
    if (MT == 4) {
        if (v == 1) return launch_one<4, 4, EPI, 1, 1>(a, st);
        return launch_one<4, 4, EPI, 3, 1>(a, st);
    }
    if (MT == 2) return launch_one<2, 4, EPI, 3, 2>(a, st);
    if constexpr (EPI != EPI_GATE) {
        if (MT == 1) return launch_one<1, 4, EPI, 3, 2>(a, st);
    }
    return hipErrorInvalidValue;
}

hipError_t launch_gemm(int MT, int epi, const GemmArgs& a, hipStream_t st) {
    if (a.nslab <= 0 || a.B <= 0 || a.L <= 0) return hipSuccess;
    switch (epi) {
        case EPI_LINEAR: return launch_epi<EPI_LINEAR>(MT, a, st);
        case EPI_GATE: return launch_epi<EPI_GATE>(MT, a, st);
        case EPI_DGATE: return launch_epi<EPI_DGATE>(MT, a, st);
        case EPI_ACCUM: return launch_epi<EPI_ACCUM>(MT, a, st);
    }
    return hipErrorInvalidValue;
}

}
```

wavenet_speech_amd/csrc/wn_kernels.h:

```cpp
#pragma once
#include <hip/hip_runtime.h>
#include <stdint.h>

namespace wn {

typedef float f32x16 __attribute__((ext_vector_type(16)));
typedef float f32x4 __attribute__((ext_vector_type(4)));

constexpr int kMaxSeg = 32;
constexpr int kMaxSlab = 32;
constexpr int kMaxDst = 2;
constexpr int kColTile = 128;

struct GemmSeg {
    const float* base;
    int cp;
    int off;
    int nkb;
    int _pad;
};

struct GemmSlab {
    long long woff;
    int nseg;
    int dst;
    int row0;
    int boff;
};

struct GemmDst {
    float* base;
    int cp;
    int rows;
    int accumulate;
    int _pad;
};

struct GemmArgs {
    const float* wpacked;
    const float* bias;
    GemmSeg seg[kMaxSeg];
    GemmSlab slab[kMaxSlab];
    GemmDst dst[kMaxDst];
    float* sg;
    float* z;
    float* da;
    float* dg;
    int gate_cp;
    int gate_rows;
    int nslab;
    int B, L, ld, halo;
    int tiles_per_row;
    int ncol;
    unsigned long long* stamps;
};

enum { EPI_LINEAR = 0, EPI_GATE = 1, EPI_DGATE = 2, EPI_ACCUM = 3 };

struct PackSrc {
    const float* ptr;
    int rows, cols;
    int stride_r, stride_c;
};
struct PackSet {
    PackSrc seg[kMaxSeg];
    const float* bias0;
    const float* bias1;
    int bias_rows;
    int _pad;
};
struct PackTile { int set; int row0; };
struct PackArgs {
    PackSet set[2];
    PackTile tile[kMaxSlab * 4];
    int seg_nkb[kMaxSeg];
    long long slab_woff[kMaxSlab];
    int slab_nseg[kMaxSlab];
    int slab_boff[kMaxSlab];
    int nslab, MT;
    float* wpacked;
    float* bias;
    long long total;
};

constexpr int kMaxPair = 2 * 8 + 3;
constexpr int kMaxReduceDst = 56;
struct WgradPair {
    const float* A; const float* Bm;
    int a_cp, b_cp;
    int off;
    int mt, nt;
    int tile0;
    long long slab_off;
    int Mp, Np;
    int rowsum;
    int rs_off;
};
struct WgradArgs {
    WgradPair pair[kMaxPair];
    int npair;
    int ntile_total;
    int nsplit;
    int B, L, ld, halo;
    int chunks_per_row;
    int nchunk;
    float* slab;
    float* rowsum;
    long long slab_floats;
    int rs_floats;
    int xcd_map;
};

struct ReduceDst {
    float* w;
    int M, N, sm, sn;
    long long slab_off; int Np;
    float* b0; float* b1;
    int rs_off;
    float post;
};
struct ReduceArgs {
    ReduceDst d[kMaxReduceDst];
    int npair, nsplit;
    const float* slab; const float* rowsum;
    long long slab_floats; int rs_floats;
    const float* dyn_inv;
};

static_assert(sizeof(ReduceArgs) <= 4096 && sizeof(WgradArgs) <= 4096, "kernel arguments are limited to 4 KiB");

hipError_t launch_gemm(int MT, int epi, const GemmArgs& a, hipStream_t st);
hipError_t launch_pack(const PackArgs& a, hipStream_t st);
hipError_t launch_wgrad(int WT, const WgradArgs& a, hipStream_t st);
hipError_t launch_wgrad_reduce(const ReduceArgs& a, hipStream_t st);
hipError_t launch_nll_forward(const float* logits, const long long* target, float* lse, float* partial, int* bad_targets, int B,
                              int C, int L, hipStream_t st);
hipError_t launch_nll_backward(const float* logits, const long long* target, const float* lse, const float* gscale,
                               float* dlogits, int B, int C, int L, hipStream_t st);

}
```

wavenet_speech_amd/csrc/wn_pack.hip:

```cpp
#include "wn_kernels.h"

namespace wn {

__global__ __launch_bounds__(256) void pack_kernel(const PackArgs a) {
    const long long idx = (long long)blockIdx.x * 256 + threadIdx.x;
    if (idx < a.total) {
        int slab = 0;
        while (slab + 1 < a.nslab && idx >= a.slab_woff[slab + 1]) ++slab;
        const long long rel = idx - a.slab_woff[slab];
        const int q = (int)(rel & 3);
        const int lane = (int)((rel >> 2) & 63);
        const long long gm = rel >> 8;
        const int m = (int)(gm % a.MT);
        int g = (int)(gm / a.MT);
        int s = 0;
        while (g >= a.seg_nkb[s]) { g -= a.seg_nkb[s]; ++s; }
        const int c = 8 * g + 4 * (lane >> 5) + q;
        const PackTile t = a.tile[slab * a.MT + m];
        float v = 0.0f;
        if (t.row0 >= 0) {
            const PackSrc src = a.set[t.set].seg[s];
            const int r = t.row0 + (lane & 31);
            if (src.ptr && r < src.rows && c < src.cols) v = src.ptr[(long long)r * src.stride_r + (long long)c * src.stride_c];
        }
        a.wpacked[idx] = v;
    }
    const long long nb = (long long)a.nslab * a.MT * 32;
    if (idx < nb && a.bias) {
        const int slab = (int)(idx / (a.MT * 32));
        const int rr = (int)(idx % (a.MT * 32));
        const PackTile t = a.tile[slab * a.MT + rr / 32];
        float v = 0.0f;
        if (t.row0 >= 0) {
            const PackSet& ps = a.set[t.set];
            const int r = t.row0 + (rr & 31);
            if (r < ps.bias_rows) {
                if (ps.bias0) v += ps.bias0[r];
                if (ps.bias1) v += ps.bias1[r];
            }
        }
        a.bias[a.slab_boff[slab] + rr] = v;
    }
}

hipError_t launch_pack(const PackArgs& a, hipStream_t st) {
    long long n = a.total;
    const long long nb = (long long)a.nslab * a.MT * 32;
    if (nb > n) n = nb;
    if (n <= 0) return hipSuccess;
    hipLaunchKernelGGL(pack_kernel, dim3((unsigned)((n + 255) / 256)), dim3(256), 0, st, a);
    return hipGetLastError();
}

}
```

wavenet_speech_amd/functional.py:

```python
import ctypes
import os

import torch
from torch.autograd.function import once_differentiable

from . import _flags, _lib
from .series import Lease, SeriesLayout, fresh_series, load_series, window

PARAMS_PER_BLOCK = 10


class BlockSpec(object):
    __slots__ = ("ci", "co", "ms", "k", "d", "causal")

    def __init__(self, ci, co, ms, k, d, causal):
        self.ci, self.co, self.ms, self.k, self.d, self.causal = int(ci), int(co), int(ms), int(k), int(d), bool(causal)

    def offsets(self):
        return _lib.tap_offsets(self.k, self.d, self.causal)

    def reach(self):
        return max(abs(o) for o in self.offsets())


def _on_device_of_first_tensor(fn):
    import functools

    @functools.wraps(fn)
    def wrapper(ctx, *args):
        dev = next((a.device for a in args if isinstance(a, torch.Tensor) and a.is_cuda), None)
        if dev is None:
            return fn(ctx, *args)
        with torch.cuda.device(dev):
            return fn(ctx, *args)
    return wrapper


def _require_device(t, what):
    if not t.is_cuda:
        raise RuntimeError("wavenet_speech_amd: %s is a CPU tensor; the HIP path needs ROCm device tensors "
                           "(there is no CPU fallback)" % what)
    if t.dtype != torch.float32:
        raise RuntimeError("wavenet_speech_amd: %s must be float32, got %s" % (what, t.dtype))


def _own(view):
    return view.clone(memory_format=torch.contiguous_format)


def _stream():
    return ctypes.c_void_p(torch.cuda.current_stream().cuda_stream)


def _p(x):
    if x is None:
        return None
    if isinstance(x, int):
        return ctypes.c_void_p(x)
    if isinstance(x, Lease):
        return ctypes.c_void_p(x.ptr)
    return ctypes.c_void_p(x.data_ptr())


def _shape(spec, batch, layout):
    return _lib.BlockShape(batch, layout.length, spec.ci, spec.co, spec.ms, spec.k, spec.d, int(spec.causal),
                           layout.ld, layout.halo)


def _params_struct(tensors):
    return _lib.BlockParams(*[_p(t) for t in tensors])


def _prep_params(tensors, spec):
    want = [(spec.co, spec.ci, spec.k), (spec.co,), (spec.co, spec.ci, spec.k), (spec.co,),
            (spec.co, spec.co), (spec.co,), (spec.ms, spec.co), (spec.ms,), (spec.co, spec.ci), (spec.co,)]
    out = []
    for t, w in zip(tensors, want):
        _require_device(t, "parameter")
        if t.dim() == 3 and len(w) == 2:
            t = t[:, :, 0]
        if tuple(t.shape) != w:
            raise RuntimeError("wavenet_speech_amd: parameter shape %s, expected %s" % (tuple(t.shape), w))
        out.append(t.detach().contiguous())
    return out


def _pack_block(lib, shape, params, device):
    nbytes = lib.wn_block_packed_bytes(ctypes.byref(shape))
    if nbytes == 0:
        _lib.check(-1, "wn_block_packed_bytes")
    packed = torch.empty(nbytes, dtype=torch.uint8, device=device)
    ps = _params_struct(params)
    _lib.check(lib.wn_block_pack(ctypes.byref(shape), ctypes.byref(ps), _p(packed), _stream()), "wn_block_pack")
    return packed


def _block_backward(lib, shape, spec, packed, x, sg, z, dr, dskip, want_dx, layout, batch, device):
    da, dg = Lease(batch, spec.co, layout, device), Lease(batch, spec.co, layout, device)
    dx = Lease(batch, spec.ci, layout, device) if want_dx else None
    _lib.check(lib.wn_block_backward_data(ctypes.byref(shape), _p(packed), _p(dr), _p(dskip), _p(z), _p(sg),
                                          _p(da), _p(dg), _p(dx), _stream()), "wn_block_backward_data")
    k = spec.k
    shapes = [(spec.co, spec.ci, k), (spec.co,), (spec.co, spec.ci, k), (spec.co,), (spec.co, spec.co), (spec.co,),
              (spec.ms, spec.co), (spec.ms,), (spec.co, spec.ci), (spec.co,)]
    unused = (4, 5, 8, 9) if dr is None else ()
    grads = [None if i in unused else torch.empty(s, dtype=torch.float32, device=device) for i, s in enumerate(shapes)]
    ws_bytes = lib.wn_block_wgrad_workspace_bytes(ctypes.byref(shape))
    ws = torch.empty(max(ws_bytes, 16), dtype=torch.uint8, device=device)
    gs = _params_struct(grads)
    _lib.check(lib.wn_block_backward_weights(ctypes.byref(shape), _p(x), _p(z), _p(da), _p(dg), _p(dr), _p(dskip),
                                             ctypes.byref(gs), _p(ws), ws_bytes, _stream()),
               "wn_block_backward_weights")
    return dx, grads


def _stack_skip_sum(lib, specs, zs, skip_w, skip_b, S, batch, layout, device):
    bias_total = torch.stack(skip_b).sum(0).contiguous()
    G = _lib.MAX_STACK_GROUP
    for g0 in range(0, len(specs), G):
        idx = range(g0, min(g0 + G, len(specs)))
        n = len(idx)
        shape = _lib.SkipSumShape(batch, layout.length, specs[0].ms, n, layout.ld, layout.halo)
        for i, l in enumerate(idx):
            shape.channels[i] = specs[l].co
        nbytes = lib.wn_skipsum_packed_bytes(ctypes.byref(shape))
        if nbytes == 0:
            _lib.check(-1, "wn_skipsum_packed_bytes")
        packed = torch.empty(nbytes, dtype=torch.uint8, device=device)
        wptrs = (ctypes.c_void_p * n)(*[skip_w[l].data_ptr() for l in idx])
        zptrs = (ctypes.c_void_p * n)(*[zs[l].ptr for l in idx])
        _lib.check(lib.wn_skipsum_pack(ctypes.byref(shape), wptrs, _p(bias_total) if g0 == 0 else None, _p(packed),
                                       _stream()), "wn_skipsum_pack")
        _lib.check(lib.wn_skipsum_forward(ctypes.byref(shape), _p(packed), zptrs, _p(S), 0 if g0 == 0 else 1, _stream()),
                   "wn_skipsum_forward")


class _ResidualStackFn(torch.autograd.Function):

    @staticmethod
    @_on_device_of_first_tensor
    def forward(ctx, x, specs, grad_enabled, pack_cache, pool, *flat):
        lib = _lib.load()
        _require_device(x, "input")
        n = len(specs)
        assert len(flat) == n * PARAMS_PER_BLOCK
        B, C0, L = x.shape
        ctx.pool, ctx.in_length = int(pool), L
        if pool > 1:
            L = L // pool
            if L < 1:
                raise RuntimeError("wavenet_speech_amd: sequence shorter than the pooling window")
        if C0 != specs[0].ci:
            raise RuntimeError("wavenet_speech_amd: input has %d channels, first block expects %d" % (C0, specs[0].ci))
        for l in range(1, n):
            if specs[l].ci != specs[l - 1].co:
                raise RuntimeError("wavenet_speech_amd: block %d expects %d input channels but block %d produces %d"
                                   % (l, specs[l].ci, l - 1, specs[l - 1].co))
        dev = x.device
        layout = SeriesLayout(L, max(s.reach() for s in specs))
        training = bool(grad_enabled) and any(ctx.needs_input_grad)
        ctx.training = training
        cur = Lease(B, C0, layout, dev)
        if pool > 1:
            _lib.check(lib.wn_series_load_pooled(_p(x.detach().contiguous()), _p(cur), B, C0, ctx.in_length, int(pool), layout.ld,
                                                 layout.halo, _stream()), "wn_series_load_pooled")
        else:
            load_series(cur.t, x.detach(), layout)
        ms = specs[0].ms
        S = fresh_series(B, ms, layout, dev)
        saved, skip_w, skip_b = [], [], []
        zbuf = None
        for l, spec in enumerate(specs):
            if spec.ms != ms:
                raise RuntimeError("wavenet_speech_amd: all blocks of a stack must share out_dim")
            shape = _shape(spec, B, layout)
            params = _prep_params(flat[l * PARAMS_PER_BLOCK:(l + 1) * PARAMS_PER_BLOCK], spec)
            if pack_cache is not None and pack_cache.frozen and not grad_enabled:
                packed = pack_cache.get(l, layout, B)
                if packed is None:
                    packed = pack_cache.put(l, layout, B, _pack_block(lib, shape, params, dev))
            else:
                packed = _pack_block(lib, shape, params, dev)
            r = Lease(B, spec.co, layout, dev) if l + 1 < n else None
            if training:
                sg, z = (Lease(B, spec.co, layout, dev) for _ in range(2))
            else:
                sg = None
                if zbuf is None or zbuf.channels != spec.co:
                    zbuf = Lease(B, spec.co, layout, dev)
                z = zbuf
            _lib.check(lib.wn_block_forward(ctypes.byref(shape), _p(packed), _p(cur), _p(r), None if training else _p(S),
                                            1, _p(sg), _p(z), _stream()), "wn_block_forward")
            if training:
                saved.append((cur, sg, z, packed, shape))
                skip_w.append(params[6])
                skip_b.append(params[7])
            cur = r
        if training:
            _stack_skip_sum(lib, specs, [sv[2] for sv in saved], skip_w, skip_b, S, B, layout, dev)
        ctx.specs, ctx.saved, ctx.layout, ctx.batch = specs, saved, layout, B
        ctx.param_shapes = [tuple(t.shape) for t in flat]
        return window(S, ms, layout).clone(memory_format=torch.contiguous_format)

    @staticmethod
    @once_differentiable
    @_on_device_of_first_tensor
    def backward(ctx, d_skips):
        lib = _lib.load()
        specs, layout, B = ctx.specs, ctx.layout, ctx.batch
        dev = d_skips.device
        dS = Lease(B, specs[0].ms, layout, dev)
        load_series(dS.t, d_skips, layout)
        dr = None
        grads_flat = [None] * (len(specs) * PARAMS_PER_BLOCK)
        for l in range(len(specs) - 1, -1, -1):
            spec = specs[l]
            x, sg, z, packed, shape = ctx.saved[l]
            want_dx = l > 0 or ctx.needs_input_grad[0]
            dx, grads = _block_backward(lib, shape, spec, packed, x, sg, z, dr, dS, want_dx, layout, B, dev)
            grads_flat[l * PARAMS_PER_BLOCK:(l + 1) * PARAMS_PER_BLOCK] = grads
            dr = dx
            ctx.saved[l] = None
        dx0 = window(dr.t, specs[0].ci, layout).clone(memory_format=torch.contiguous_format) if ctx.needs_input_grad[0] else None
        if dx0 is not None and ctx.pool > 1:
            dx0 = _unpool(lib, dx0, ctx.in_length, ctx.pool)
        grads_flat = [None if g is None else g.view(shp) for g, shp in zip(grads_flat, ctx.param_shapes)]
        return (dx0, None, None, None, None) + tuple(grads_flat)


def _unpool(lib, dpooled, length, pool):
    B, C, _ = dpooled.shape
    dx = torch.empty(B, C, length, dtype=torch.float32, device=dpooled.device)
    _lib.check(lib.wn_pool_backward(_p(dpooled.contiguous()), _p(dx), B, C, length, int(pool), _stream()), "wn_pool_backward")
    return dx


class PackCache(object):

    def __init__(self):
        self.key = None
        self.packed = {}
        self.hits = 0
        self.tables = {}
        self.frozen = False

    def validate(self, params, extra=()):
        key = tuple((id(p), p._version, p.data_ptr(), p.device) for p in params) + tuple(extra)
        if key != self.key:
            self.key = key
            self.packed = {}
            self.__dict__["_shapes"] = []

    MAX_SHAPES = 4

    def get(self, l, layout, batch):
        shape = (layout.key(), batch)
        t = self.packed.get((l,) + shape)
        if t is not None:
            self.hits += 1
            self._touch(shape)
        return t

    def put(self, l, layout, batch, t):
        shape = (layout.key(), batch)
        self._touch(shape)
        self.packed[(l,) + shape] = t
        return t

    def _touch(self, shape):
        order = self.__dict__.setdefault("_shapes", [])
        if shape in order:
            order.remove(shape)
        order.append(shape)
        while len(order) > self.MAX_SHAPES:
            old = order.pop(0)
            for k in [k for k in self.packed if k[1:] == old]:
                del self.packed[k]


def residual_stack(x, specs, flat_params, precision="f32", pack_cache=None, head=None, front=None, pool=1):
    if precision != "f32":
        from . import functional_half
        return functional_half.residual_stack(x, specs, flat_params, precision, pack_cache, head, front, pool)
    if head is not None or front is not None:
        raise ValueError("the fused output block / feature layer exist in the half-precision modes only")
    return _ResidualStackFn.apply(x, tuple(specs), torch.is_grad_enabled(), pack_cache, int(pool), *flat_params)


class _ResidualBlockFn(torch.autograd.Function):

    @staticmethod
    @_on_device_of_first_tensor
    def forward(ctx, x, spec, grad_enabled, *params):
        lib = _lib.load()
        _require_device(x, "input")
        B, C0, L = x.shape
        if C0 != spec.ci:
            raise RuntimeError("wavenet_speech_amd: input has %d channels, block expects %d" % (C0, spec.ci))
        dev = x.device
        layout = SeriesLayout(L, spec.reach())
        shape = _shape(spec, B, layout)
        prm = _prep_params(params, spec)
        packed = _pack_block(lib, shape, prm, dev)
        xin = Lease(B, C0, layout, dev)
        load_series(xin.t, x.detach(), layout)
        r = Lease(B, spec.co, layout, dev)
        s = Lease(B, spec.ms, layout, dev)
        training = bool(grad_enabled) and any(ctx.needs_input_grad)
        sg = Lease(B, spec.co, layout, dev) if training else None
        z = Lease(B, spec.co, layout, dev)
        _lib.check(lib.wn_block_forward(ctypes.byref(shape), _p(packed), _p(xin), _p(r), _p(s), 0,
                                        _p(sg), _p(z), _stream()), "wn_block_forward")
        if training:
            ctx.saved = (xin, sg, z, packed, shape)
        ctx.spec, ctx.layout, ctx.batch = spec, layout, B
        ctx.param_shapes = [tuple(t.shape) for t in params]
        return _own(r.view()), _own(s.view())

    @staticmethod
    @once_differentiable
    @_on_device_of_first_tensor
    def backward(ctx, d_r, d_s):
        lib = _lib.load()
        spec, layout, B = ctx.spec, ctx.layout, ctx.batch
        dev = d_r.device
        x, sg, z, packed, shape = ctx.saved
        dr, ds = Lease(B, spec.co, layout, dev), Lease(B, spec.ms, layout, dev)
        load_series(dr.t, d_r, layout)
        load_series(ds.t, d_s, layout)
        dx, grads = _block_backward(lib, shape, spec, packed, x, sg, z, dr, ds, ctx.needs_input_grad[0], layout, B, dev)
        grads = [g.view(shp) for g, shp in zip(grads, ctx.param_shapes)]
        dx0 = _own(dx.view()) if dx is not None else None
        ctx.saved = None
        return (dx0, None, None) + tuple(grads)


def residual_block(x, spec, params):
    return _ResidualBlockFn.apply(x, spec, torch.is_grad_enabled(), *params)


class _DilatedConvFn(torch.autograd.Function):

    @staticmethod
    @_on_device_of_first_tensor
    def forward(ctx, x, weight, bias, dilation, causal, grad_enabled):
        lib = _lib.load()
        _require_device(x, "input")
        _require_device(weight, "weight")
        B, Ci, L = x.shape
        Co, Ci_w, k = weight.shape
        if Ci_w != Ci:
            raise RuntimeError("wavenet_speech_amd: input has %d channels, conv expects %d" % (Ci, Ci_w))
        dev = x.device
        reach = max(abs(o) for o in _lib.tap_offsets(k, dilation, causal))
        layout = SeriesLayout(L, reach)
        shape = _lib.ConvShape(B, L, Ci, Co, k, int(dilation), int(bool(causal)), layout.ld, layout.halo)
        nbytes = lib.wn_conv_packed_bytes(ctypes.byref(shape))
        if nbytes == 0:
            _lib.check(-1 if k <= _lib.MAX_TAPS else -2, "wn_conv_packed_bytes")
        packed = torch.empty(nbytes, dtype=torch.uint8, device=dev)
        w = weight.detach().contiguous()
        b = bias.detach().contiguous() if bias is not None else None
        _lib.check(lib.wn_conv_pack(ctypes.byref(shape), _p(w), _p(b), _p(packed), _stream()), "wn_conv_pack")
        xin = Lease(B, Ci, layout, dev)
        load_series(xin.t, x.detach(), layout)
        y = Lease(B, Co, layout, dev)
        _lib.check(lib.wn_conv_forward(ctypes.byref(shape), _p(packed), _p(xin), _p(y), _stream()), "wn_conv_forward")
        if grad_enabled and any(ctx.needs_input_grad):
            ctx.saved = (xin, packed, shape)
        ctx.layout, ctx.dims, ctx.has_bias = layout, (B, Ci, Co, k), bias is not None
        return _own(y.view())

    @staticmethod
    @once_differentiable
    @_on_device_of_first_tensor
    def backward(ctx, d_y):
        lib = _lib.load()
        xin, packed, shape = ctx.saved
        layout = ctx.layout
        B, Ci, Co, k = ctx.dims
        dev = d_y.device
        dy = Lease(B, Co, layout, dev)
        load_series(dy.t, d_y, layout)
        dx0 = None
        if ctx.needs_input_grad[0]:
            dx = Lease(B, Ci, layout, dev)
            _lib.check(lib.wn_conv_backward_data(ctypes.byref(shape), _p(packed), _p(dy), _p(dx), _stream()),
                       "wn_conv_backward_data")
            dx0 = _own(dx.view())
        dw = torch.empty(Co, Ci, k, dtype=torch.float32, device=dev)
        db = torch.empty(Co, dtype=torch.float32, device=dev) if ctx.has_bias else None
        ws_bytes = lib.wn_conv_wgrad_workspace_bytes(ctypes.byref(shape))
        ws = torch.empty(max(ws_bytes, 16), dtype=torch.uint8, device=dev)
        _lib.check(lib.wn_conv_backward_weights(ctypes.byref(shape), _p(xin), _p(dy), _p(dw), _p(db), _p(ws), ws_bytes,
                                                _stream()), "wn_conv_backward_weights")
        ctx.saved = None
        return dx0, dw, db, None, None, None


def dilated_conv(x, weight, bias, dilation=1, causal=True, precision="f32"):
    if precision != "f32":
        from . import functional_half
        return functional_half.conv(x, weight, bias, dilation, causal, precision)
    return _DilatedConvFn.apply(x, weight, bias, int(dilation), bool(causal), torch.is_grad_enabled())


class _SequenceNLLFn(torch.autograd.Function):

    @staticmethod
    @_on_device_of_first_tensor
    def forward(ctx, logits, target, grad_enabled=True):
        lib = _lib.load()
        _require_device(logits, "logits")
        if target.dtype != torch.int64 or not target.is_cuda:
            raise RuntimeError("wavenet_speech_amd: target must be an int64 device tensor")
        B, C, L = logits.shape
        x = logits.detach().contiguous()
        tg = target.contiguous()
        lse = torch.empty(2, B, L, dtype=torch.float32, device=x.device)
        partial = torch.empty(lib.wn_nll_partials(B, L), dtype=torch.float32, device=x.device)
        bad = torch.zeros(1, dtype=torch.int32, device=x.device)
        _lib.check(lib.wn_nll_forward(_p(x), _p(tg), _p(lse), _p(partial), _p(bad), B, C, L, _stream()), "wn_nll_forward")
        if os.environ.get("WN_NLL_CHECK", "1") != "0":
            _flags.WATCH.poll()
            _flags.WATCH.note(bad, lambda n, C=C: "wavenet_speech_amd: sequence_nll got %d target(s) outside [0, %d)" % (n, C),
                              at_once=not (grad_enabled and ctx.needs_input_grad[0]))
        ctx.save_for_backward(x, tg, lse)
        return partial.sum() / B

    @staticmethod
    @once_differentiable
    @_on_device_of_first_tensor
    def backward(ctx, g):
        lib = _lib.load()
        x, tg, lse = ctx.saved_tensors
        B, C, L = x.shape
        gscale = (g / B).to(torch.float32).reshape(1).contiguous()
        dx = torch.empty_like(x)
        _lib.check(lib.wn_nll_backward(_p(x), _p(tg), _p(lse), _p(gscale), _p(dx), B, C, L, _stream()), "wn_nll_backward")
        return dx, None, None


def sequence_nll(logits, target):
    return _SequenceNLLFn.apply(logits, target, torch.is_grad_enabled())


class _EmbedConvFn(torch.autograd.Function):

    @staticmethod
    @_on_device_of_first_tensor
    def forward(ctx, weight, bias, levels, grad_enabled=True):
        lib = _lib.load()
        _require_device(weight, "weight")
        if levels.dtype != torch.int64 or not levels.is_cuda or levels.dim() != 2:
            raise RuntimeError("wavenet_speech_amd: levels must be an int64 device tensor [B, L]")
        Co, classes, k = weight.shape
        B, L = levels.shape
        q = levels.contiguous()
        w = weight.detach().contiguous()
        b = bias.detach().contiguous() if bias is not None else None
        y = torch.empty(B, Co, L, dtype=torch.float32, device=weight.device)
        bad = torch.zeros(1, dtype=torch.int32, device=weight.device)
        _lib.check(lib.wn_embed_forward(_p(q), _p(w), _p(b), _p(y), B, L, classes, Co, k, _p(bad), _stream()), "wn_embed_forward")
        if os.environ.get("WN_NLL_CHECK", "1") != "0":
            _flags.WATCH.poll()
            _flags.WATCH.note(bad, lambda n, classes=classes: "wavenet_speech_amd: %d thread(s) saw a level outside [0, %d)" % (n, classes),
                              at_once=not (grad_enabled and any(ctx.needs_input_grad)))
        ctx.save_for_backward(q)
        ctx.dims, ctx.has_bias = (B, L, classes, Co, k), bias is not None
        return y

    @staticmethod
    @once_differentiable
    @_on_device_of_first_tensor
    def backward(ctx, d_y):
        lib = _lib.load()
        (q,) = ctx.saved_tensors
        B, L, classes, Co, k = ctx.dims
        dev = d_y.device
        dy = d_y.contiguous()
        dw = torch.empty(Co, classes, k, dtype=torch.float32, device=dev)
        db = torch.empty(Co, dtype=torch.float32, device=dev) if ctx.has_bias else None
        layout = SeriesLayout(L, k - 1)
        shape = _lib.ConvShape(B, L, classes, Co, k, 1, 1, layout.ld, layout.halo)
        xin = Lease(B, classes, layout, dev)
        ok = (q >= 0) & (q < classes)
        window(xin.t, classes, layout).zero_().scatter_(1, q.clamp(0, classes - 1).unsqueeze(1), ok.unsqueeze(1).to(torch.float32))
        dyl = Lease(B, Co, layout, dev)
        load_series(dyl.t, dy, layout)
        ws_bytes = lib.wn_conv_wgrad_workspace_bytes(ctypes.byref(shape))
        ws = torch.empty(max(ws_bytes, 16), dtype=torch.uint8, device=dev)
        _lib.check(lib.wn_conv_backward_weights(ctypes.byref(shape), _p(xin), _p(dyl), _p(dw), _p(db), _p(ws), ws_bytes,
                                                _stream()), "wn_conv_backward_weights")
        return dw, db, None, None


def embed_conv(levels, weight, bias):
    return _EmbedConvFn.apply(weight, bias, levels, torch.is_grad_enabled())


def profile_enable(on=True):
    lib = _lib.load()
    _lib.check(lib.wn_prof_enable(1 if on else 0), "wn_prof_enable")


def profile_reset():
    _lib.check(_lib.load().wn_prof_reset(), "wn_prof_reset")


def profile_read():
    return _lib.profile_read()
```

wavenet_speech_amd/modules/block.py:

```python
import torch
import torch.nn as nn

from .. import functional as HF
from .conv_ops import CausalConv1d, NonCausalConv1d


class GatedActivationUnit(nn.Module):

    def forward(self, x, y):
        return torch.tanh(x) * torch.sigmoid(y)

    def __repr__(self):
        return self.__class__.__name__ + ' ()'


class ResidualBlock(nn.Module):

    def __init__(self, in_channels, out_channels, kernel_width, dilation, causal=True, conditioning=None):
        super(ResidualBlock, self).__init__()
        self.in_channels, self.out_channels = in_channels, out_channels
        self.kernel_width, self.dilation = kernel_width, dilation
        self.causal = causal
        self.conditioning = conditioning is not None
        conv = CausalConv1d if causal else NonCausalConv1d
        self.conv_tanh = conv(in_channels, out_channels, kernel_width, dilation=dilation)
        self.conv_sigmoid = conv(in_channels, out_channels, kernel_width, dilation=dilation)
        self.conv1x1_residual = nn.Conv1d(out_channels, out_channels, kernel_size=1)
        self.conv1x1_skip = nn.Conv1d(out_channels, out_channels, kernel_size=1)
        self.gated_activation = GatedActivationUnit()
        self.residual_proj = nn.Linear(in_channels, out_channels)
        self.receptive_field = self.conv_tanh.receptive_field

    def hip_params(self, skip_weight=None, skip_bias=None):
        return [self.conv_tanh.conv1d.weight, self.conv_tanh.conv1d.bias,
                self.conv_sigmoid.conv1d.weight, self.conv_sigmoid.conv1d.bias,
                self.conv1x1_residual.weight, self.conv1x1_residual.bias,
                self.conv1x1_skip.weight if skip_weight is None else skip_weight,
                self.conv1x1_skip.bias if skip_bias is None else skip_bias,
                self.residual_proj.weight, self.residual_proj.bias]

    def spec(self, skip_rows=None):
        return HF.BlockSpec(self.in_channels, self.out_channels,
                            self.out_channels if skip_rows is None else skip_rows,
                            self.kernel_width, self.dilation, self.causal)

    def forward(self, seq):
        return HF.residual_block(seq, self.spec(), self.hip_params())


def fold_bottleneck(block, bottleneck):
    wb = bottleneck.weight.squeeze(2)
    wk = block.conv1x1_skip.weight.squeeze(2)
    return wb @ wk, wb @ block.conv1x1_skip.bias + bottleneck.bias


def fold_bottlenecks(blocks, bottlenecks):
    shapes = set((tuple(b.weight.shape), tuple(k.conv1x1_skip.weight.shape)) for k, b in zip(blocks, bottlenecks))
    if len(shapes) != 1:
        folded = [fold_bottleneck(k, b) for k, b in zip(blocks, bottlenecks)]
        return [w for w, _ in folded], [b for _, b in folded]
    wb = torch.stack([b.weight.squeeze(2) for b in bottlenecks])
    wk = torch.stack([k.conv1x1_skip.weight.squeeze(2) for k in blocks])
    bk = torch.stack([k.conv1x1_skip.bias for k in blocks]).unsqueeze(2)
    bb = torch.stack([b.bias for b in bottlenecks]).unsqueeze(2)
    wf = torch.bmm(wb, wk)
    bf = torch.baddbmm(bb, wb, bk).squeeze(2)
    return list(wf.unbind(0)), list(bf.unbind(0))


class StackState(object):

    def __init__(self):
        self.precision = "f32"
        self.cache = HF.PackCache()
        self.folded = None


PRECISIONS = ("f32", "f16x3", "f16", "bf16")


def pointwise_precision(precision):
    return precision if precision in ("f16", "bf16") else "f32"


def head_precision(precision):
    import os
    if precision == "f16x3" and not os.environ.get("WN_HEAD_F32"):
        return "f16x3"
    return pointwise_precision(precision)


def set_precision(module, precision):
    if precision not in PRECISIONS:
        raise ValueError("precision must be one of %s" % (PRECISIONS,))
    n = 0
    from .conv_ops import _DilatedConv1d
    for m in module.modules():
        st = getattr(m, "stack_state", None)
        if isinstance(st, StackState):
            st.precision = precision
            st.cache = HF.PackCache()
            n += 1
        if isinstance(m, _DilatedConv1d):
            m.precision = pointwise_precision(precision)
    if n == 0:
        raise ValueError("set_precision: no residual stack in %s" % type(module).__name__)
    return module


def freeze_for_inference(module, on=True):
    n = 0
    for m in module.modules():
        st = getattr(m, "stack_state", None)
        if isinstance(st, StackState):
            tables = st.cache.tables
            st.cache = HF.PackCache()
            st.cache.tables = tables
            st.cache.frozen = bool(on)
            st.folded = None
            n += 1
    if n == 0:
        raise ValueError("freeze_for_inference: no residual stack in %s" % type(module).__name__)
    return module


def fusable_head(head, precision):
    import os
    import torch.nn as nn
    if head is None or os.environ.get("WN_SERIES_HEAD", "1") == "0":
        return None
    if precision == "f32" or head_precision(precision) != precision:
        return None
    mods = list(head)
    if len(mods) != 4 or not (isinstance(mods[0], nn.LeakyReLU) and isinstance(mods[2], nn.LeakyReLU)):
        return None
    for c in (mods[1], mods[3]):
        if not isinstance(c, nn.Conv1d) or c.kernel_size != (1,) or c.stride != (1,) or c.padding != (0,) or c.groups != 1 \
                or c.bias is None:
            return None
    if not (mods[0].negative_slope >= 0 and mods[2].negative_slope >= 0):
        return None
    return (mods[0].negative_slope, mods[2].negative_slope), [mods[1].weight, mods[1].bias, mods[3].weight, mods[3].bias]


def fusable_front(front, precision, x):
    import os
    import torch.nn as nn
    knob = os.environ.get("WN_SERIES_FRONT", "1")
    if front is None or knob == "0":
        return None
    if precision == "f32" or (pointwise_precision(precision) != precision and knob != "force"):
        return None
    if x.requires_grad or x.dim() != 3 or x.shape[1] != 1:
        return None
    mods = list(front)
    if len(mods) != 4 or not (isinstance(mods[1], nn.LeakyReLU) and isinstance(mods[3], nn.LeakyReLU)):
        return None
    c0, c1 = mods[0], mods[2]
    if not (isinstance(c0, nn.Conv1d) and isinstance(c1, nn.Conv1d)) or c0.bias is None or c1.bias is None:
        return None
    k = c0.kernel_size[0]
    if c0.in_channels != 1 or c0.stride != (1,) or c0.dilation != (1,) or c0.groups != 1 or c0.padding != (k - 1,) or k > 8:
        return None
    if c1.kernel_size != (1,) or c1.stride != (1,) or c1.padding != (0,) or c1.groups != 1:
        return None
    if not (mods[1].negative_slope >= 0 and mods[3].negative_slope >= 0):
        return None
    return (mods[1].negative_slope, mods[3].negative_slope), [c0.weight, c0.bias, c1.weight, c1.bias]


def run_stack(out, blocks, bottlenecks, state=None, head=None, front=None, pool=1):
    specs, flat = [], []
    out_dim = bottlenecks[0].out_channels
    blocks, bottlenecks = list(blocks), list(bottlenecks)
    precision = state.precision if state is not None else "f32"
    cache = state.cache if state is not None else None
    if state is not None and cache.frozen and not torch.is_grad_enabled():
        params = [p for m in blocks + bottlenecks for p in m.parameters()]
        old_key = cache.key
        cache.validate(params, (precision,))
        if state.folded is None or cache.key != old_key:
            state.folded = fold_bottlenecks(blocks, bottlenecks)
        wfs, bfs = state.folded
    else:
        wfs, bfs = fold_bottlenecks(blocks, bottlenecks)
        if state is not None:
            state.folded = None
    for blk, w, b in zip(blocks, wfs, bfs):
        specs.append(blk.spec(out_dim))
        flat.extend(blk.hip_params(w, b))
    fh = fusable_head(head, precision)
    res = HF.residual_stack(out, specs, flat, precision=precision, pack_cache=cache, head=fh, front=front, pool=pool)
    return res if head is None else (res, fh is not None)
```

wavenet_speech_amd/modules/wavenet.py:

```python
import torch
import torch.nn as nn
import torch.nn.functional as F

from .. import functional as HF
from .block import ResidualBlock, StackState, run_stack, pointwise_precision, head_precision
from .conv_ops import CausalConv1d
from .pointwise import run_sequential


def _init_weights_and_zero_bias(params):
    for p in params:
        if p.dim() > 1:
            nn.init.kaiming_uniform_(p)
        else:
            p.data.zero_()


class WaveNet(nn.Module):
    def __init__(self, in_dim, entry_kwidth, layers, out_dim, softmax=True):
        super(WaveNet, self).__init__()
        self.in_dim, self.entry_kwidth = in_dim, entry_kwidth
        self.layers, self.num_layers = layers, len(layers)
        self.out_dim, self.softmax = out_dim, softmax
        self.stack_state = StackState()

        self.entry_conv1d = CausalConv1d(in_dim, layers[0][0], entry_kwidth, dilation=1)
        self.convolutions = nn.ModuleList([ResidualBlock(ci, co, k, d) for (ci, co, k, d) in layers])
        self.bottlenecks = nn.ModuleList([nn.Conv1d(co, out_dim, 1) for (_ci, co, _k, _d) in layers])
        self.output_stack = nn.Sequential(nn.LeakyReLU(0.01), nn.Conv1d(out_dim, out_dim, kernel_size=1),
                                          nn.LeakyReLU(0.01), nn.Conv1d(out_dim, out_dim, kernel_size=1))
        _init_weights_and_zero_bias(self.entry_conv1d.parameters())
        _init_weights_and_zero_bias(self.convolutions.parameters())
        for p in self.bottlenecks.parameters():
            if p.dim() == 1:
                p.data.zero_()
        _init_weights_and_zero_bias(self.output_stack.parameters())

    def forward_levels(self, levels):
        if self.entry_conv1d.dilation != 1:
            raise RuntimeError("wavenet_speech_amd: forward_levels needs the reference's dilation-1 entry conv")
        out = HF.embed_conv(levels, self.entry_conv1d.conv1d.weight, self.entry_conv1d.conv1d.bias)
        return self._after_entry(out)

    def forward(self, signal):
        out = self.entry_conv1d(signal)
        return self._after_entry(out)

    def _after_entry(self, out):
        skips_sum, done = run_stack(out, self.convolutions, self.bottlenecks, self.stack_state, head=self.output_stack)
        output_seq = skips_sum if done else run_sequential(self.output_stack, skips_sum, head_precision(self.stack_state.precision))
        if not self.softmax:
            return output_seq
        return F.softmax(output_seq, dim=1)
```

Before: 99.23 samples/s.

## Fuse entry conv and output head into f32 residual stack with batched packing

Extends the f32 residual-stack autograd function so the entry causal conv and the LeakyReLU/1x1-conv output head run inside it on the series layout. The skip-sum GEMM applies the first LeakyReLU in its epilogue, and new series conv forward/backward-data entry points fold in the second activation and its derivative. A table-driven stack packer builds every block, skipsum and conv pack job at once so weights can be packed in one launch instead of many small ones. This is meant to remove layout round-trips, separate PyTorch head and entry ops, and per-block pack launch overhead, at the cost of more complex backward bookkeeping and new code paths.

```diff
diff --git a/include/wavenet_amd.h b/include/wavenet_amd.h
--- a/include/wavenet_amd.h
+++ b/include/wavenet_amd.h
@@ -284,6 +284,23 @@
                               float* dweight, float* dbias , const float* dyn_inv_scale ,
                               void* workspace, size_t workspace_bytes, wn_stream_t stream);
 
+int wn_skipsum_forward_series(const wn_skipsum_shape* s, const void* packed, const float* const* z, float* out_series,
+                              float leaky_slope, wn_stream_t stream);
+int wn_conv_forward_series(const wn_conv_shape* s, const void* packed, const float* x, float* y, float leaky_slope,
+                           wn_stream_t stream);
+int wn_conv_backward_data_series(const wn_conv_shape* s, const void* packed, const float* dy, const float* act,
+                                 float leaky_slope, float* dx, wn_stream_t stream);
+
+typedef struct wn_pack_conv { wn_conv_shape shape; const float* weight ; const float* bias ; } wn_pack_conv;
+size_t wn_stack_pack_table_bytes(int nblocks, int nconvs);
+int wn_stack_pack_table_build(const wn_block_shape* shapes, const wn_block_params* params, int nblocks, int with_skipsum,
+                              const float* skip_bias_total, const wn_pack_conv* convs, int nconvs,
+                              const wn_mem_range* dynamic, int ndynamic, void* table_host, size_t table_bytes,
+                              size_t* block_offsets, size_t* skipsum_offsets, size_t* conv_offsets, size_t* packed_total,
+                              int* njobs, int* launch_blocks);
+int wn_stack_pack_run(const void* table_dev, int njobs, int launch_blocks, const void* const* dynamic_bases, int ndynamic,
+                      void* packed, wn_stream_t stream);
+
 #ifdef __cplusplus
 }
 #endif
diff --git a/wavenet_speech_amd/_lib.py b/wavenet_speech_amd/_lib.py
--- a/wavenet_speech_amd/_lib.py
+++ b/wavenet_speech_amd/_lib.py
@@ -37,6 +37,10 @@
 class ConvShape(Structure):
     _fields_ = [("batch", c_int), ("length", c_int), ("in_channels", c_int), ("out_channels", c_int),
                 ("kernel_width", c_int), ("dilation", c_int), ("causal", c_int), ("ld", c_int), ("halo", c_int)]
+
+
+class PackConv(Structure):
+    _fields_ = [("shape", ConvShape), ("weight", c_float_p), ("bias", c_float_p)]
 
 
 SIGNATURES = {
@@ -67,6 +71,14 @@
     "wn_conv_wgrad_workspace_bytes": (c_size_t, [POINTER(ConvShape)]),
     "wn_conv_backward_weights": (c_int, [POINTER(ConvShape), c_float_p, c_float_p, c_float_p, c_float_p,
                                          c_void_p, c_size_t, c_void_p]),
+    "wn_skipsum_forward_series": (c_int, [POINTER(SkipSumShape), c_void_p, POINTER(c_void_p), c_float_p, c_float, c_void_p]),
+    "wn_conv_forward_series": (c_int, [POINTER(ConvShape), c_void_p, c_float_p, c_float_p, c_float, c_void_p]),
+    "wn_conv_backward_data_series": (c_int, [POINTER(ConvShape), c_void_p, c_float_p, c_float_p, c_float, c_float_p, c_void_p]),
+    "wn_stack_pack_table_bytes": (c_size_t, [c_int, c_int]),
+    "wn_stack_pack_table_build": (c_int, [POINTER(BlockShape), POINTER(BlockParams), c_int, c_int, c_float_p, POINTER(PackConv), c_int,
+                                          POINTER(MemRange), c_int, c_void_p, c_size_t, POINTER(c_size_t), POINTER(c_size_t),
+                                          POINTER(c_size_t), POINTER(c_size_t), POINTER(c_int), POINTER(c_int)]),
+    "wn_stack_pack_run": (c_int, [c_void_p, c_int, c_int, POINTER(c_void_p), c_int, c_void_p, c_void_p]),
     "wn_hseries_layout": (c_int, [c_int, c_int, POINTER(c_int), POINTER(c_int)]),
     "wn_hseries_bytes": (c_size_t, [c_int, c_int, c_int, c_int]),
     "wn_hseries_residual_scale": (c_float, []),
diff --git a/wavenet_speech_amd/csrc/wn_api.hip b/wavenet_speech_amd/csrc/wn_api.hip
--- a/wavenet_speech_amd/csrc/wn_api.hip
+++ b/wavenet_speech_amd/csrc/wn_api.hip
@@ -336,17 +336,11 @@
     return plan_block(s).total;
 }
 
-int wn_block_pack(const wn_block_shape* s, const wn_block_params* p, void* packed, wn_stream_t stream) {
-    int off[WN_MAX_TAPS];
-    int rc = check_block(s, off);
-    if (rc != WN_OK) return rc;
-    if (!p || !packed || !p->w_tanh || !p->w_sigmoid || !p->w_res || !p->w_skip || !p->w_proj) return WN_ERR_NULL;
-    hipStream_t st = (hipStream_t)stream;
-    const BlockPlan bp = plan_block(s);
+namespace {
+void block_pack_jobs(const wn_block_shape* s, const wn_block_params* p, const BlockPlan& bp, void* packed, PackArgs (&out)[4]) {
     const int Ci = s->in_channels, Co = s->out_channels, Ms = s->skip_rows, k = s->kernel_width;
-    ProfScope prof(KC_PACK, 0.0, st);
-    PackArgs a;
-    {
+    {
+        PackArgs& a = out[0];
         const GemmPlan& g = bp.fa;
         fill_pack_common(a, g, packed, bp.off_fa);
         for (int j = 0; j < k; ++j) {
@@ -362,9 +356,9 @@
                 a.tile[sl * g.MT + m].set = m & 1;
                 a.tile[sl * g.MT + m].row0 = pair < pairs ? 32 * pair : -1;
             }
-        WN_HIP(launch_pack(a, st), "pack(gate)");
-    }
-    {
+    }
+    {
+        PackArgs& a = out[1];
         const GemmPlan& g = bp.fb;
         fill_pack_common(a, g, packed, bp.off_fb);
         a.set[0].seg[0] = mk_src(p->w_res, Co, Co, Co, 1);
@@ -379,9 +373,9 @@
                 a.tile[sl * g.MT + m].set = skip ? 1 : 0;
                 a.tile[sl * g.MT + m].row0 = row0 < (skip ? Ms : Co) ? row0 : -1;
             }
-        WN_HIP(launch_pack(a, st), "pack(res+skip)");
-    }
-    {
+    }
+    {
+        PackArgs& a = out[2];
         const GemmPlan& g = bp.ka;
         fill_pack_common(a, g, packed, bp.off_ka);
         a.set[0].seg[0] = mk_src(p->w_skip, Co, Ms, 1, Co);
@@ -392,9 +386,9 @@
                 a.tile[sl * g.MT + m].set = 0;
                 a.tile[sl * g.MT + m].row0 = row0 < Co ? row0 : -1;
             }
-        WN_HIP(launch_pack(a, st), "pack(dz)");
-    }
-    {
+    }
+    {
+        PackArgs& a = out[3];
         const GemmPlan& g = bp.kb;
         fill_pack_common(a, g, packed, bp.off_kb);
         for (int j = 0; j < k; ++j) {
@@ -408,8 +402,25 @@
                 a.tile[sl * g.MT + m].set = 0;
                 a.tile[sl * g.MT + m].row0 = row0 < Ci ? row0 : -1;
             }
-        WN_HIP(launch_pack(a, st), "pack(dx)");
-    }
+    }
+}
+inline bool block_params_complete(const wn_block_params* p) {
+    return p && p->w_tanh && p->w_sigmoid && p->w_res && p->w_skip && p->w_proj;
+}
+}
+
+int wn_block_pack(const wn_block_shape* s, const wn_block_params* p, void* packed, wn_stream_t stream) {
+    int off[WN_MAX_TAPS];
+    int rc = check_block(s, off);
+    if (rc != WN_OK) return rc;
+    if (!packed || !block_params_complete(p)) return WN_ERR_NULL;
+    hipStream_t st = (hipStream_t)stream;
+    const BlockPlan bp = plan_block(s);
+    ProfScope prof(KC_PACK, 0.0, st);
+    PackArgs jobs[4];
+    block_pack_jobs(s, p, bp, packed, jobs);
+    static const char* const what[4] = {"pack(gate)", "pack(res+skip)", "pack(dz)", "pack(dx)"};
+    for (int i = 0; i < 4; ++i) WN_HIP(launch_pack(jobs[i], st), what[i]);
     return WN_OK;
 }
 
@@ -524,6 +535,21 @@
     return plan_skipsum(s).bytes();
 }
 
+namespace {
+void skipsum_pack_job(const wn_skipsum_shape* s, const GemmPlan& g, const float* const* w_skip, const float* bias_total,
+                      void* packed, PackArgs& a) {
+    fill_pack_common(a, g, packed, 0);
+    for (int l = 0; l < s->nblocks; ++l) a.set[0].seg[l] = mk_src(w_skip[l], s->skip_rows, s->channels[l], s->channels[l], 1);
+    a.set[0].bias0 = bias_total; a.set[0].bias_rows = s->skip_rows;
+    for (int sl = 0; sl < g.nslab; ++sl)
+        for (int m = 0; m < g.MT; ++m) {
+            const int row0 = g.slab_row0[sl] + 32 * m;
+            a.tile[sl * g.MT + m].set = 0;
+            a.tile[sl * g.MT + m].row0 = row0 < s->skip_rows ? row0 : -1;
+        }
+}
+}
+
 int wn_skipsum_pack(const wn_skipsum_shape* s, const float* const* w_skip, const float* bias_total, void* packed,
                     wn_stream_t stream) {
     int rc = check_skipsum(s);
@@ -534,21 +560,14 @@
     const GemmPlan g = plan_skipsum(s);
     ProfScope prof(KC_PACK, 0.0, st);
     PackArgs a;
-    fill_pack_common(a, g, packed, 0);
-    for (int l = 0; l < s->nblocks; ++l) a.set[0].seg[l] = mk_src(w_skip[l], s->skip_rows, s->channels[l], s->channels[l], 1);
-    a.set[0].bias0 = bias_total; a.set[0].bias_rows = s->skip_rows;
-    for (int sl = 0; sl < g.nslab; ++sl)
-        for (int m = 0; m < g.MT; ++m) {
-            const int row0 = g.slab_row0[sl] + 32 * m;
-            a.tile[sl * g.MT + m].set = 0;
-            a.tile[sl * g.MT + m].row0 = row0 < s->skip_rows ? row0 : -1;
-        }
+    skipsum_pack_job(s, g, w_skip, bias_total, packed, a);
     WN_HIP(launch_pack(a, st), "pack(skipsum)");
     return WN_OK;
 }
 
-int wn_skipsum_forward(const wn_skipsum_shape* s, const void* packed, const float* const* z, float* skip, int accumulate,
-                       wn_stream_t stream) {
+namespace {
+int skipsum_forward(const wn_skipsum_shape* s, const void* packed, const float* const* z, float* skip, int accumulate,
+                    bool leaky, float slope, wn_stream_t stream) {
     int rc = check_skipsum(s);
     if (rc != WN_OK) return rc;
     if (!packed || !z || !skip) return WN_ERR_NULL;
@@ -560,9 +579,21 @@
     double ksum = 0;
     for (int l = 0; l < s->nblocks; ++l) { set_seg(a, l, z[l], s->channels[l], 0, g.seg_nkb[l]); ksum += s->channels[l]; }
     a.dst[0].base = skip; a.dst[0].cp = cp8(s->skip_rows); a.dst[0].rows = s->skip_rows; a.dst[0].accumulate = accumulate ? 1 : 0;
+    a.slope = slope;
     ProfScope prof(KC_SKIP_GEMM, 2.0 * s->skip_rows * ksum * (double)s->batch * s->length, st);
-    WN_HIP(launch_gemm(g.MT, accumulate ? EPI_ACCUM : EPI_LINEAR, a, st), "series_gemm<skipsum>");
-    return WN_OK;
+    WN_HIP(launch_gemm(g.MT, leaky ? EPI_LEAKY : (accumulate ? EPI_ACCUM : EPI_LINEAR), a, st), "series_gemm<skipsum>");
+    return WN_OK;
+}
+}
+
+int wn_skipsum_forward(const wn_skipsum_shape* s, const void* packed, const float* const* z, float* skip, int accumulate,
+                       wn_stream_t stream) {
+    return skipsum_forward(s, packed, z, skip, accumulate, false, 1.0f, stream);
+}
+
+int wn_skipsum_forward_series(const wn_skipsum_shape* s, const void* packed, const float* const* z, float* out_series,
+                              float leaky_slope, wn_stream_t stream) {
+    return skipsum_forward(s, packed, z, out_series, 0, true, leaky_slope, stream);
 }
 
 namespace {
@@ -715,17 +746,12 @@
     return plan_conv(s).total;
 }
 
-int wn_conv_pack(const wn_conv_shape* s, const float* weight, const float* bias, void* packed, wn_stream_t stream) {
-    int off[WN_MAX_TAPS];
-    int rc = check_conv(s, off);
-    if (rc != WN_OK) return rc;
-    if (!weight || !packed) return WN_ERR_NULL;
-    hipStream_t st = (hipStream_t)stream;
-    const ConvPlan cp = plan_conv(s);
+namespace {
+void conv_pack_jobs(const wn_conv_shape* s, const ConvPlan& cp, const float* weight, const float* bias, void* packed,
+                    PackArgs (&out)[2]) {
     const int Ci = s->in_channels, Co = s->out_channels, k = s->kernel_width;
-    ProfScope prof(KC_PACK, 0.0, st);
-    PackArgs a;
-    {
+    {
+        PackArgs& a = out[0];
         const GemmPlan& g = cp.cf;
         fill_pack_common(a, g, packed, cp.off_cf);
         for (int j = 0; j < k; ++j) a.set[0].seg[j] = mk_src(weight + j, Co, Ci, Ci * k, k);
@@ -736,9 +762,9 @@
                 a.tile[sl * g.MT + m].set = 0;
                 a.tile[sl * g.MT + m].row0 = row0 < Co ? row0 : -1;
             }
-        WN_HIP(launch_pack(a, st), "pack(conv fwd)");
-    }
-    {
+    }
+    {
+        PackArgs& a = out[1];
         const GemmPlan& g = cp.cb;
         fill_pack_common(a, g, packed, cp.off_cb);
         for (int j = 0; j < k; ++j) a.set[0].seg[j] = mk_src(weight + j, Ci, Co, k, Ci * k);
@@ -748,12 +774,154 @@
                 a.tile[sl * g.MT + m].set = 0;
                 a.tile[sl * g.MT + m].row0 = row0 < Ci ? row0 : -1;
             }
-        WN_HIP(launch_pack(a, st), "pack(conv bwd)");
-    }
-    return WN_OK;
-}
-
-int wn_conv_forward(const wn_conv_shape* s, const void* packed, const float* x, float* y, wn_stream_t stream) {
+    }
+}
+}
+
+int wn_conv_pack(const wn_conv_shape* s, const float* weight, const float* bias, void* packed, wn_stream_t stream) {
+    int off[WN_MAX_TAPS];
+    int rc = check_conv(s, off);
+    if (rc != WN_OK) return rc;
+    if (!weight || !packed) return WN_ERR_NULL;
+    hipStream_t st = (hipStream_t)stream;
+    const ConvPlan cp = plan_conv(s);
+    ProfScope prof(KC_PACK, 0.0, st);
+    PackArgs jobs[2];
+    conv_pack_jobs(s, cp, weight, bias, packed, jobs);
+    WN_HIP(launch_pack(jobs[0], st), "pack(conv fwd)");
+    WN_HIP(launch_pack(jobs[1], st), "pack(conv bwd)");
+    return WN_OK;
+}
+
+namespace {
+inline int stack_pack_max_jobs(int nblocks, int nconvs) { return 4 * nblocks + cdiv(nblocks, WN_MAX_STACK_GROUP) + 2 * nconvs; }
+
+bool finish_pack_job(PackJob& j, const wn_mem_range* dyn, int ndyn) {
+    auto rel = [&](const float*& p, signed char& mark) {
+        mark = -1;
+        if (!p) return;
+        const uintptr_t v = reinterpret_cast<uintptr_t>(p);
+        for (int i = 0; i < ndyn; ++i) {
+            const uintptr_t b = reinterpret_cast<uintptr_t>(dyn[i].base);
+            if (v >= b && v < b + dyn[i].bytes) {
+                p = reinterpret_cast<const float*>(v - b);
+                mark = (signed char)i;
+                return;
+            }
+        }
+    };
+    for (int set = 0; set < 2; ++set) {
+        for (int sg = 0; sg < kMaxSeg; ++sg) rel(j.a.set[set].seg[sg].ptr, j.seg_dyn[set][sg]);
+        rel(j.a.set[set].bias0, j.bias_dyn[set][0]);
+        rel(j.a.set[set].bias1, j.bias_dyn[set][1]);
+    }
+    return true;
+}
+}
+
+size_t wn_stack_pack_table_bytes(int nblocks, int nconvs) {
+    if (nblocks < 0 || nconvs < 0 || nblocks + nconvs == 0) return 0;
+    return (size_t)stack_pack_max_jobs(nblocks, nconvs) * sizeof(PackJob);
+}
+
+int wn_stack_pack_table_build(const wn_block_shape* shapes, const wn_block_params* params, int nblocks, int with_skipsum,
+                              const float* skip_bias_total, const wn_pack_conv* convs, int nconvs,
+                              const wn_mem_range* dynamic, int ndynamic, void* table_host, size_t table_bytes,
+                              size_t* block_offsets, size_t* skipsum_offsets, size_t* conv_offsets, size_t* packed_total,
+                              int* njobs, int* launch_blocks) {
+    if (nblocks < 0 || nconvs < 0 || nblocks + nconvs == 0 || ndynamic < 0) return WN_ERR_BAD_SHAPE;
+    if (ndynamic > kMaxPackDyn) return WN_ERR_UNSUPPORTED;
+    if (!table_host || !packed_total || !njobs || !launch_blocks) return WN_ERR_NULL;
+    if ((nblocks && (!shapes || !params || !block_offsets)) || (nconvs && (!convs || !conv_offsets))) return WN_ERR_NULL;
+    if (ndynamic && !dynamic) return WN_ERR_NULL;
+    if (with_skipsum && nblocks && !skipsum_offsets) return WN_ERR_NULL;
+    if (table_bytes < wn_stack_pack_table_bytes(nblocks, nconvs)) return WN_ERR_WORKSPACE;
+    PackJob* jobs = reinterpret_cast<PackJob*>(table_host);
+    int nj = 0;
+    long long blocks = 0;
+    size_t total = 0;
+    auto push = [&](const PackArgs& a) {
+        PackJob& j = jobs[nj];
+        std::memset(&j, 0, sizeof(j));
+        j.a = a;
+        j.first_block = (int)blocks;
+        finish_pack_job(j, dynamic, ndynamic);
+        blocks += pack_job_blocks(a);
+        ++nj;
+    };
+    int off[WN_MAX_TAPS];
+    for (int l = 0; l < nblocks; ++l) {
+        int rc = check_block(&shapes[l], off);
+        if (rc != WN_OK) return rc;
+        if (!block_params_complete(&params[l])) return WN_ERR_NULL;
+        const BlockPlan bp = plan_block(&shapes[l]);
+        PackArgs a[4];
+        block_pack_jobs(&shapes[l], &params[l], bp, reinterpret_cast<void*>(total), a);
+        for (int i = 0; i < 4; ++i) push(a[i]);
+        block_offsets[l] = total;
+        total += bp.total;
+    }
+    if (with_skipsum) {
+        for (int g0 = 0, gi = 0; g0 < nblocks; g0 += WN_MAX_STACK_GROUP, ++gi) {
+            wn_skipsum_shape ss;
+            std::memset(&ss, 0, sizeof(ss));
+            ss.batch = shapes[0].batch; ss.length = shapes[0].length; ss.skip_rows = shapes[0].skip_rows;
+            ss.ld = shapes[0].ld; ss.halo = shapes[0].halo;
+            ss.nblocks = std::min(WN_MAX_STACK_GROUP, nblocks - g0);
+            const float* w[WN_MAX_STACK_GROUP];
+            for (int i = 0; i < ss.nblocks; ++i) {
+                if (shapes[g0 + i].skip_rows != ss.skip_rows) return WN_ERR_BAD_SHAPE;
+                ss.channels[i] = shapes[g0 + i].out_channels;
+                w[i] = params[g0 + i].w_skip;
+            }
+            int rc = check_skipsum(&ss);
+            if (rc != WN_OK) return rc;
+            const GemmPlan g = plan_skipsum(&ss);
+            PackArgs a;
+            skipsum_pack_job(&ss, g, w, g0 == 0 ? skip_bias_total : nullptr, reinterpret_cast<void*>(total), a);
+            push(a);
+            skipsum_offsets[gi] = total;
+            total += g.bytes();
+        }
+    }
+    for (int c = 0; c < nconvs; ++c) {
+        int rc = check_conv(&convs[c].shape, off);
+        if (rc != WN_OK) return rc;
+        if (!convs[c].weight) return WN_ERR_NULL;
+        const ConvPlan cp = plan_conv(&convs[c].shape);
+        PackArgs a[2];
+        conv_pack_jobs(&convs[c].shape, cp, convs[c].weight, convs[c].bias, reinterpret_cast<void*>(total), a);
+        push(a[0]);
+        push(a[1]);
+        conv_offsets[c] = total;
+        total += cp.total;
+    }
+    if (blocks > 0x7fffffffLL) return WN_ERR_UNSUPPORTED;
+    *packed_total = total;
+    *njobs = nj;
+    *launch_blocks = (int)blocks;
+    return WN_OK;
+}
+
+int wn_stack_pack_run(const void* table_dev, int njobs, int launch_blocks, const void* const* dynamic_bases, int ndynamic,
+                      void* packed, wn_stream_t stream) {
+    if (njobs <= 0 || launch_blocks <= 0 || ndynamic < 0) return WN_ERR_BAD_SHAPE;
+    if (ndynamic > kMaxPackDyn) return WN_ERR_UNSUPPORTED;
+    if (!table_dev || !packed || (ndynamic && !dynamic_bases)) return WN_ERR_NULL;
+    hipStream_t st = (hipStream_t)stream;
+    PackBases bases;
+    std::memset(&bases, 0, sizeof(bases));
+    for (int i = 0; i < ndynamic; ++i) {
+        if (!dynamic_bases[i]) return WN_ERR_NULL;
+        bases.b[i] = reinterpret_cast<const char*>(dynamic_bases[i]);
+    }
+    ProfScope prof(KC_PACK, 0.0, st);
+    WN_HIP(launch_pack_table(reinterpret_cast<const PackJob*>(table_dev), njobs, launch_blocks, bases, packed, st), "pack(stack)");
+    return WN_OK;
+}
+
+namespace {
+int conv_forward(const wn_conv_shape* s, const void* packed, const float* x, float* y, bool leaky, float slope, wn_stream_t stream) {
     int off[WN_MAX_TAPS];
     int rc = check_conv(s, off);
     if (rc != WN_OK) return rc;
@@ -765,12 +933,14 @@
     fill_gemm_common(a, g, packed, cp.off_cf, 0, g.nslab, s->batch, s->length, s->ld, s->halo);
     for (int j = 0; j < s->kernel_width; ++j) set_seg(a, j, x, s->in_channels, off[j], g.seg_nkb[j]);
     a.dst[0].base = y; a.dst[0].cp = cp8(s->out_channels); a.dst[0].rows = s->out_channels; a.dst[0].accumulate = 0;
+    a.slope = slope;
     ProfScope prof(KC_CONV_FWD, 2.0 * s->out_channels * (double)(s->kernel_width * s->in_channels) * s->batch * s->length, st);
-    WN_HIP(launch_gemm(g.MT, EPI_LINEAR, a, st), "series_gemm<conv fwd>");
-    return WN_OK;
-}
-
-int wn_conv_backward_data(const wn_conv_shape* s, const void* packed, const float* dy, float* dx, wn_stream_t stream) {
+    WN_HIP(launch_gemm(g.MT, leaky ? EPI_LEAKY : EPI_LINEAR, a, st), "series_gemm<conv fwd>");
+    return WN_OK;
+}
+
+int conv_backward_data(const wn_conv_shape* s, const void* packed, const float* dy, const float* act, float slope, float* dx,
+                       wn_stream_t stream) {
     int off[WN_MAX_TAPS];
     int rc = check_conv(s, off);
     if (rc != WN_OK) return rc;
@@ -783,9 +953,29 @@
     a.bias = nullptr;
     for (int j = 0; j < s->kernel_width; ++j) set_seg(a, j, dy, s->out_channels, -off[j], g.seg_nkb[j]);
     a.dst[0].base = dx; a.dst[0].cp = cp8(s->in_channels); a.dst[0].rows = s->in_channels; a.dst[0].accumulate = 0;
+    a.mask = act; a.slope = slope;
     ProfScope prof(KC_CONV_BWD_DATA, 2.0 * s->in_channels * (double)(s->kernel_width * s->out_channels) * s->batch * s->length, st);
-    WN_HIP(launch_gemm(g.MT, EPI_LINEAR, a, st), "series_gemm<conv bwd>");
-    return WN_OK;
+    WN_HIP(launch_gemm(g.MT, act ? EPI_DMASK : EPI_LINEAR, a, st), "series_gemm<conv bwd>");
+    return WN_OK;
+}
+}
+
+int wn_conv_forward(const wn_conv_shape* s, const void* packed, const float* x, float* y, wn_stream_t stream) {
+    return conv_forward(s, packed, x, y, false, 1.0f, stream);
+}
+
+int wn_conv_forward_series(const wn_conv_shape* s, const void* packed, const float* x, float* y, float leaky_slope,
+                           wn_stream_t stream) {
+    return conv_forward(s, packed, x, y, true, leaky_slope, stream);
+}
+
+int wn_conv_backward_data(const wn_conv_shape* s, const void* packed, const float* dy, float* dx, wn_stream_t stream) {
+    return conv_backward_data(s, packed, dy, nullptr, 1.0f, dx, stream);
+}
+
+int wn_conv_backward_data_series(const wn_conv_shape* s, const void* packed, const float* dy, const float* act, float leaky_slope,
+                                 float* dx, wn_stream_t stream) {
+    return conv_backward_data(s, packed, dy, act, leaky_slope, dx, stream);
 }
 
 namespace {
diff --git a/wavenet_speech_amd/csrc/wn_gemm.hip b/wavenet_speech_amd/csrc/wn_gemm.hip
--- a/wavenet_speech_amd/csrc/wn_gemm.hip
+++ b/wavenet_speech_amd/csrc/wn_gemm.hip
@@ -247,6 +247,65 @@
             }
             __builtin_amdgcn_sched_barrier(0);
         }
+    } else if constexpr (EPI == EPI_LEAKY) {
+        const GemmDst d = a.dst[sl.dst];
+        const float slope = a.slope;
+#pragma unroll
+        for (int m = 0; m < MT; ++m) {
+#pragma unroll
+            for (int r = 0; r < 16; ++r) {
+                const int row = sl.row0 + 32 * m + rowof(r, h);
+                if (row < d.rows) {
+                    float* p = d.base + ((long)b * d.cp + row) * ld + colbase;
+                    breg_t v;
+#pragma unroll
+                    for (int t = 0; t < NT; ++t) {
+                        const float x = acc[m][t][r];
+                        v[t] = x > 0.0f ? x : x * slope;
+                    }
+                    *reinterpret_cast<breg_t*>(p) = clip(v);
+                }
+            }
+            __builtin_amdgcn_sched_barrier(0);
+        }
+    } else if constexpr (EPI == EPI_DMASK) {
+        const GemmDst d = a.dst[sl.dst];
+        const float slope = a.slope;
+        constexpr int RB = 8, BPT = 16 / RB, NBATCH = MT * BPT;
+        breg_t msk[2][RB];
+        const long tile_off = (long)b * d.cp * ld + colbase;
+        float* const tile = d.base + tile_off;
+        const float* const mtile = a.mask + tile_off;
+        auto fetch = [&](int bi, breg_t (&dst)[RB]) {
+            const int m = bi / BPT, r0 = (bi % BPT) * RB;
+#pragma unroll
+            for (int i = 0; i < RB; ++i) {
+                int row = sl.row0 + 32 * m + rowof(r0 + i, h);
+                row = row < d.rows ? row : d.rows - 1;
+                dst[i] = *reinterpret_cast<const breg_t*>(mtile + (long)row * ld);
+            }
+        };
+        fetch(0, msk[0]);
+#pragma unroll
+        for (int bi = 0; bi < NBATCH; ++bi) {
+            if (bi + 1 < NBATCH) fetch(bi + 1, msk[(bi + 1) & 1]);
+            __builtin_amdgcn_sched_barrier(0);
+            const int m = bi / BPT, r0 = (bi % BPT) * RB;
+#pragma unroll
+            for (int i = 0; i < RB; ++i) {
+                const int row = sl.row0 + 32 * m + rowof(r0 + i, h);
+                if (row < d.rows) {
+                    breg_t v;
+#pragma unroll
+                    for (int t = 0; t < NT; ++t) {
+                        const float g = acc[m][t][r0 + i];
+                        v[t] = msk[bi & 1][i][t] > 0.0f ? g : g * slope;
+                    }
+                    *reinterpret_cast<breg_t*>(tile + (long)row * ld) = clip(v);
+                }
+            }
+            __builtin_amdgcn_sched_barrier(0);
+        }
     } else {
         constexpr int RB = (MT == 4) ? 8 : 4;
         constexpr int BPT = 16 / RB;
@@ -349,6 +408,8 @@
         case EPI_GATE: return launch_epi<EPI_GATE>(MT, a, st);
         case EPI_DGATE: return launch_epi<EPI_DGATE>(MT, a, st);
         case EPI_ACCUM: return launch_epi<EPI_ACCUM>(MT, a, st);
+        case EPI_LEAKY: return launch_epi<EPI_LEAKY>(MT, a, st);
+        case EPI_DMASK: return launch_epi<EPI_DMASK>(MT, a, st);
     }
     return hipErrorInvalidValue;
 }
diff --git a/wavenet_speech_amd/csrc/wn_kernels.h b/wavenet_speech_amd/csrc/wn_kernels.h
--- a/wavenet_speech_amd/csrc/wn_kernels.h
+++ b/wavenet_speech_amd/csrc/wn_kernels.h
@@ -53,9 +53,11 @@
     int tiles_per_row;
     int ncol;
     unsigned long long* stamps;
+    const float* mask;
+    float slope;
 };
 
-enum { EPI_LINEAR = 0, EPI_GATE = 1, EPI_DGATE = 2, EPI_ACCUM = 3 };
+enum { EPI_LINEAR = 0, EPI_GATE = 1, EPI_DGATE = 2, EPI_ACCUM = 3, EPI_LEAKY = 4, EPI_DMASK = 5 };
 
 struct PackSrc {
     const float* ptr;
@@ -82,6 +84,15 @@
     float* bias;
     long long total;
 };
+
+constexpr int kMaxPackDyn = 3;
+struct PackJob {
+    PackArgs a;
+    int first_block;
+    signed char seg_dyn[2][kMaxSeg];
+    signed char bias_dyn[2][2];
+};
+struct PackBases { const char* b[kMaxPackDyn]; };
 
 constexpr int kMaxPair = 2 * 8 + 3;
 constexpr int kMaxReduceDst = 56;
@@ -131,6 +142,9 @@
 
 hipError_t launch_gemm(int MT, int epi, const GemmArgs& a, hipStream_t st);
 hipError_t launch_pack(const PackArgs& a, hipStream_t st);
+long long pack_job_blocks(const PackArgs& a);
+hipError_t launch_pack_table(const PackJob* jobs_dev, int njobs, int launch_blocks, const PackBases& bases, void* packed,
+                             hipStream_t st);
 hipError_t launch_wgrad(int WT, const WgradArgs& a, hipStream_t st);
 hipError_t launch_wgrad_reduce(const ReduceArgs& a, hipStream_t st);
 hipError_t launch_nll_forward(const float* logits, const long long* target, float* lse, float* partial, int* bad_targets, int B,
diff --git a/wavenet_speech_amd/csrc/wn_pack.hip b/wavenet_speech_amd/csrc/wn_pack.hip
--- a/wavenet_speech_amd/csrc/wn_pack.hip
+++ b/wavenet_speech_amd/csrc/wn_pack.hip
@@ -2,8 +2,9 @@
 
 namespace wn {
 
-__global__ __launch_bounds__(256) void pack_kernel(const PackArgs a) {
-    const long long idx = (long long)blockIdx.x * 256 + threadIdx.x;
+template <class SrcFn, class Bias0Fn, class Bias1Fn>
+__device__ __forceinline__ void pack_element(const PackArgs& a, long long idx, float* wpacked, float* bias, SrcFn src,
+                                             Bias0Fn bias0, Bias1Fn bias1) {
     if (idx < a.total) {
         int slab = 0;
         while (slab + 1 < a.nslab && idx >= a.slab_woff[slab + 1]) ++slab;
@@ -19,36 +20,78 @@
         const PackTile t = a.tile[slab * a.MT + m];
         float v = 0.0f;
         if (t.row0 >= 0) {
-            const PackSrc src = a.set[t.set].seg[s];
+            const PackSrc& ps = a.set[t.set].seg[s];
+            const float* ptr = src(t.set, s);
             const int r = t.row0 + (lane & 31);
-            if (src.ptr && r < src.rows && c < src.cols) v = src.ptr[(long long)r * src.stride_r + (long long)c * src.stride_c];
+            if (ptr && r < ps.rows && c < ps.cols) v = ptr[(long long)r * ps.stride_r + (long long)c * ps.stride_c];
         }
-        a.wpacked[idx] = v;
+        wpacked[idx] = v;
     }
     const long long nb = (long long)a.nslab * a.MT * 32;
-    if (idx < nb && a.bias) {
+    if (idx < nb && bias) {
         const int slab = (int)(idx / (a.MT * 32));
         const int rr = (int)(idx % (a.MT * 32));
         const PackTile t = a.tile[slab * a.MT + rr / 32];
         float v = 0.0f;
         if (t.row0 >= 0) {
-            const PackSet& ps = a.set[t.set];
             const int r = t.row0 + (rr & 31);
-            if (r < ps.bias_rows) {
-                if (ps.bias0) v += ps.bias0[r];
-                if (ps.bias1) v += ps.bias1[r];
+            if (r < a.set[t.set].bias_rows) {
+                const float* p0 = bias0(t.set);
+                const float* p1 = bias1(t.set);
+                if (p0) v += p0[r];
+                if (p1) v += p1[r];
             }
         }
-        a.bias[a.slab_boff[slab] + rr] = v;
+        bias[a.slab_boff[slab] + rr] = v;
     }
 }
 
-hipError_t launch_pack(const PackArgs& a, hipStream_t st) {
+__global__ __launch_bounds__(256) void pack_kernel(const PackArgs a) {
+    const long long idx = (long long)blockIdx.x * 256 + threadIdx.x;
+    pack_element(a, idx, a.wpacked, a.bias,
+                 [&](int set, int seg) { return a.set[set].seg[seg].ptr; },
+                 [&](int set) { return a.set[set].bias0; }, [&](int set) { return a.set[set].bias1; });
+}
+
+__global__ __launch_bounds__(256) void pack_table_kernel(const PackJob* __restrict__ jobs, int njobs, const PackBases bases,
+                                                         char* packed) {
+    int lo = 0, hi = njobs - 1;
+    while (lo < hi) {
+        const int mid = (lo + hi + 1) >> 1;
+        if (jobs[mid].first_block <= (int)blockIdx.x) lo = mid; else hi = mid - 1;
+    }
+    const PackJob& j = jobs[lo];
+    const PackArgs& a = j.a;
+    const long long idx = (long long)((int)blockIdx.x - j.first_block) * 256 + threadIdx.x;
+    auto dynp = [&](const float* p, int dyn) -> const float* {
+        return dyn < 0 ? p : reinterpret_cast<const float*>(bases.b[dyn] + reinterpret_cast<size_t>(p));
+    };
+    pack_element(a, idx, reinterpret_cast<float*>(packed + reinterpret_cast<size_t>(a.wpacked)),
+                 reinterpret_cast<float*>(packed + reinterpret_cast<size_t>(a.bias)),
+                 [&](int set, int seg) { return dynp(a.set[set].seg[seg].ptr, j.seg_dyn[set][seg]); },
+                 [&](int set) { return dynp(a.set[set].bias0, j.bias_dyn[set][0]); },
+                 [&](int set) { return dynp(a.set[set].bias1, j.bias_dyn[set][1]); });
+}
+
+long long pack_job_blocks(const PackArgs& a) {
     long long n = a.total;
     const long long nb = (long long)a.nslab * a.MT * 32;
     if (nb > n) n = nb;
-    if (n <= 0) return hipSuccess;
-    hipLaunchKernelGGL(pack_kernel, dim3((unsigned)((n + 255) / 256)), dim3(256), 0, st, a);
+    return n <= 0 ? 0 : (n + 255) / 256;
+}
+
+hipError_t launch_pack(const PackArgs& a, hipStream_t st) {
+    const long long nblk = pack_job_blocks(a);
+    if (nblk <= 0) return hipSuccess;
+    hipLaunchKernelGGL(pack_kernel, dim3((unsigned)nblk), dim3(256), 0, st, a);
+    return hipGetLastError();
+}
+
+hipError_t launch_pack_table(const PackJob* jobs_dev, int njobs, int launch_blocks, const PackBases& bases, void* packed,
+                             hipStream_t st) {
+    if (njobs <= 0 || launch_blocks <= 0) return hipSuccess;
+    hipLaunchKernelGGL(pack_table_kernel, dim3((unsigned)launch_blocks), dim3(256), 0, st, jobs_dev, njobs, bases,
+                       reinterpret_cast<char*>(packed));
     return hipGetLastError();
 }
 
diff --git a/wavenet_speech_amd/functional.py b/wavenet_speech_amd/functional.py
--- a/wavenet_speech_amd/functional.py
+++ b/wavenet_speech_amd/functional.py
@@ -114,68 +114,224 @@
     return dx, grads
 
 
-def _stack_skip_sum(lib, specs, zs, skip_w, skip_b, S, batch, layout, device):
-    bias_total = torch.stack(skip_b).sum(0).contiguous()
+def _skipsum_shape(specs, idx, batch, layout):
+    shape = _lib.SkipSumShape(batch, layout.length, specs[0].ms, len(idx), layout.ld, layout.halo)
+    for i, l in enumerate(idx):
+        shape.channels[i] = specs[l].co
+    return shape
+
+
+def _stack_skip_sum(lib, specs, zs, skip_w, bias_total, S, batch, layout, device, packed_groups=None, leaky=None):
     G = _lib.MAX_STACK_GROUP
-    for g0 in range(0, len(specs), G):
+    assert leaky is None or len(specs) <= G
+    for gi, g0 in enumerate(range(0, len(specs), G)):
         idx = range(g0, min(g0 + G, len(specs)))
         n = len(idx)
-        shape = _lib.SkipSumShape(batch, layout.length, specs[0].ms, n, layout.ld, layout.halo)
-        for i, l in enumerate(idx):
-            shape.channels[i] = specs[l].co
-        nbytes = lib.wn_skipsum_packed_bytes(ctypes.byref(shape))
-        if nbytes == 0:
-            _lib.check(-1, "wn_skipsum_packed_bytes")
-        packed = torch.empty(nbytes, dtype=torch.uint8, device=device)
-        wptrs = (ctypes.c_void_p * n)(*[skip_w[l].data_ptr() for l in idx])
+        shape = _skipsum_shape(specs, idx, batch, layout)
         zptrs = (ctypes.c_void_p * n)(*[zs[l].ptr for l in idx])
-        _lib.check(lib.wn_skipsum_pack(ctypes.byref(shape), wptrs, _p(bias_total) if g0 == 0 else None, _p(packed),
-                                       _stream()), "wn_skipsum_pack")
-        _lib.check(lib.wn_skipsum_forward(ctypes.byref(shape), _p(packed), zptrs, _p(S), 0 if g0 == 0 else 1, _stream()),
-                   "wn_skipsum_forward")
+        if packed_groups is not None:
+            packed = packed_groups[gi]
+        else:
+            nbytes = lib.wn_skipsum_packed_bytes(ctypes.byref(shape))
+            if nbytes == 0:
+                _lib.check(-1, "wn_skipsum_packed_bytes")
+            packed = torch.empty(nbytes, dtype=torch.uint8, device=device)
+            wptrs = (ctypes.c_void_p * n)(*[skip_w[l].data_ptr() for l in idx])
+            _lib.check(lib.wn_skipsum_pack(ctypes.byref(shape), wptrs, _p(bias_total) if g0 == 0 else None, _p(packed),
+                                           _stream()), "wn_skipsum_pack")
+        if leaky is not None:
+            _lib.check(lib.wn_skipsum_forward_series(ctypes.byref(shape), _p(packed), zptrs, _p(S), ctypes.c_float(leaky), _stream()),
+                       "wn_skipsum_forward_series")
+        else:
+            _lib.check(lib.wn_skipsum_forward(ctypes.byref(shape), _p(packed), zptrs, _p(S), 0 if g0 == 0 else 1, _stream()),
+                       "wn_skipsum_forward")
+
+
+def _pack_conv(lib, shape, w, b, device):
+    nbytes = lib.wn_conv_packed_bytes(ctypes.byref(shape))
+    if nbytes == 0:
+        _lib.check(-1 if shape.kernel_width <= _lib.MAX_TAPS else -2, "wn_conv_packed_bytes")
+    packed = torch.empty(nbytes, dtype=torch.uint8, device=device)
+    _lib.check(lib.wn_conv_pack(ctypes.byref(shape), _p(w), _p(b), _p(packed), _stream()), "wn_conv_pack")
+    return packed
+
+
+def _conv_wgrad(lib, shape, xin, dy, wshape, has_bias, device):
+    dw = torch.empty(wshape, dtype=torch.float32, device=device)
+    db = torch.empty(wshape[0], dtype=torch.float32, device=device) if has_bias else None
+    ws_bytes = lib.wn_conv_wgrad_workspace_bytes(ctypes.byref(shape))
+    ws = torch.empty(max(ws_bytes, 16), dtype=torch.uint8, device=device)
+    _lib.check(lib.wn_conv_backward_weights(ctypes.byref(shape), _p(xin), _p(dy), _p(dw), _p(db), _p(ws), ws_bytes, _stream()),
+               "wn_conv_backward_weights")
+    return dw, db
+
+
+class StackPackTable(object):
+    MAX_DYNAMIC = 3
+
+    @staticmethod
+    def dynamic_storages(tensors):
+        seen = []
+        for t in tensors:
+            if t is not None and not isinstance(t, torch.nn.Parameter):
+                st = t.untyped_storage()
+                if all(st.data_ptr() != q.data_ptr() for q in seen):
+                    seen.append(st)
+        return seen if len(seen) <= StackPackTable.MAX_DYNAMIC else None
+
+    @staticmethod
+    def key_of(specs, B, layout, prepped, bias_total, convs, storages):
+        dyn = [(st.data_ptr(), st.nbytes()) for st in storages]
+
+        def rel(t):
+            if t is None:
+                return None
+            p = t.data_ptr()
+            for i, (b, n) in enumerate(dyn):
+                if b <= p < b + n:
+                    return ("d", i, p - b)
+            return p
+        return ("f32", B, layout.key(), tuple(n for _, n in dyn), tuple((s.ci, s.co, s.ms, s.k, s.d, s.causal) for s in specs),
+                tuple(rel(t) for blk in prepped for t in blk), rel(bias_total),
+                tuple((tuple(getattr(sh, f) for f, _ in sh._fields_), rel(w), rel(b)) for sh, w, b in convs))
+
+    def __init__(self, lib, specs, B, layout, prepped, bias_total, convs, storages, device):
+        n, nc = len(specs), len(convs)
+        shapes = (_lib.BlockShape * n)(*[_shape(s, B, layout) for s in specs])
+        params = (_lib.BlockParams * n)(*[_params_struct(blk) for blk in prepped])
+        carr = (_lib.PackConv * max(1, nc))(*[_lib.PackConv(sh, _p(w), _p(b)) for sh, w, b in convs])
+        dyn = (_lib.MemRange * max(1, len(storages)))(*[_lib.MemRange(st.data_ptr(), st.nbytes()) for st in storages])
+        nbytes = lib.wn_stack_pack_table_bytes(n, nc)
+        host = ctypes.create_string_buffer(nbytes)
+        offs = (ctypes.c_size_t * n)()
+        soffs = (ctypes.c_size_t * ((n + _lib.MAX_STACK_GROUP - 1) // _lib.MAX_STACK_GROUP))()
+        coffs = (ctypes.c_size_t * max(1, nc))()
+        total, njobs, nblocks = ctypes.c_size_t(0), ctypes.c_int(0), ctypes.c_int(0)
+        _lib.check(lib.wn_stack_pack_table_build(shapes, params, n, 1 if bias_total is not None else 0, _p(bias_total), carr, nc,
+                                                 dyn, len(storages), host, nbytes, offs, soffs, coffs, ctypes.byref(total),
+                                                 ctypes.byref(njobs), ctypes.byref(nblocks)), "wn_stack_pack_table_build")
+        self.table = torch.frombuffer(host, dtype=torch.uint8).to(device)
+        self.njobs, self.launch_blocks, self.ndyn = njobs.value, nblocks.value, len(storages)
+        self.block_offsets, self.conv_offsets = list(offs), list(coffs)[:nc]
+        self.skipsum_offsets = list(soffs) if bias_total is not None else []
+        self.total = total.value
+
+    def run(self, lib, storages, device, out=None):
+        packed = torch.empty(self.total, dtype=torch.uint8, device=device) if out is None else out
+        bases = (ctypes.c_void_p * max(1, self.ndyn))(*[st.data_ptr() for st in storages])
+        _lib.check(lib.wn_stack_pack_run(_p(self.table), self.njobs, self.launch_blocks, bases, self.ndyn, _p(packed), _stream()),
+                   "wn_stack_pack_run")
+        return packed
 
 
 class _ResidualStackFn(torch.autograd.Function):
 
     @staticmethod
     @_on_device_of_first_tensor
-    def forward(ctx, x, specs, grad_enabled, pack_cache, pool, *flat):
+    def forward(ctx, x, specs, grad_enabled, pack_cache, pool, head, front, *flat):
         lib = _lib.load()
         _require_device(x, "input")
         n = len(specs)
+        callers = list(flat)
+        front_params = head_params = None
+        if front is not None:
+            front_params = [None if t is None else t.detach().contiguous() for t in flat[-2:]]
+            flat = flat[:-2]
+        if head is not None:
+            head_params = [t.detach().contiguous() for t in flat[-4:]]
+            flat = flat[:-4]
         assert len(flat) == n * PARAMS_PER_BLOCK
         B, C0, L = x.shape
         ctx.pool, ctx.in_length = int(pool), L
         if pool > 1:
+            if front is not None:
+                raise RuntimeError("wavenet_speech_amd: pooling and a conv in front of one stack are not combined")
             L = L // pool
             if L < 1:
                 raise RuntimeError("wavenet_speech_amd: sequence shorter than the pooling window")
+        reach = max(s.reach() for s in specs)
+        if front is not None:
+            fk, fd, fcausal = front
+            fw, fb = front_params
+            _require_device(fw, "weight")
+            if fw.dim() != 3 or fw.shape[1] != C0 or fw.shape[2] != fk:
+                raise RuntimeError("wavenet_speech_amd: input has %d channels, conv expects %s" % (C0, tuple(fw.shape)))
+            Cin, C0 = C0, fw.shape[0]
+            reach = max(reach, max(abs(o) for o in _lib.tap_offsets(fk, fd, fcausal)))
         if C0 != specs[0].ci:
             raise RuntimeError("wavenet_speech_amd: input has %d channels, first block expects %d" % (C0, specs[0].ci))
         for l in range(1, n):
             if specs[l].ci != specs[l - 1].co:
                 raise RuntimeError("wavenet_speech_amd: block %d expects %d input channels but block %d produces %d"
                                    % (l, specs[l].ci, l - 1, specs[l - 1].co))
+        ms = specs[0].ms
+        for spec in specs:
+            if spec.ms != ms:
+                raise RuntimeError("wavenet_speech_amd: all blocks of a stack must share out_dim")
         dev = x.device
-        layout = SeriesLayout(L, max(s.reach() for s in specs))
+        layout = SeriesLayout(L, reach)
         training = bool(grad_enabled) and any(ctx.needs_input_grad)
         ctx.training = training
-        cur = Lease(B, C0, layout, dev)
-        if pool > 1:
-            _lib.check(lib.wn_series_load_pooled(_p(x.detach().contiguous()), _p(cur), B, C0, ctx.in_length, int(pool), layout.ld,
-                                                 layout.halo, _stream()), "wn_series_load_pooled")
+        prepped = [_prep_params(flat[l * PARAMS_PER_BLOCK:(l + 1) * PARAMS_PER_BLOCK], spec) for l, spec in enumerate(specs)]
+        skip_w = [p[6] for p in prepped]
+        bias_total = torch.stack([p[7] for p in prepped]).sum(0).contiguous() if training else None
+        convs = []
+        if front is not None:
+            fshape = _lib.ConvShape(B, L, Cin, C0, fk, fd, int(bool(fcausal)), layout.ld, layout.halo)
+            convs.append((fshape, fw, fb))
+        if head is not None:
+            w1, b1, w2, b2 = head_params
+            c1, c2 = w1.shape[0], w2.shape[0]
+            if w1.shape[1] != ms or w2.shape[1] != c1 or w1.shape[2] != 1 or w2.shape[2] != 1:
+                raise RuntimeError("wavenet_speech_amd: output block shapes %s, %s do not follow a stack of out_dim %d"
+                                   % (tuple(w1.shape), tuple(w2.shape), ms))
+            sh1 = _lib.ConvShape(B, L, ms, c1, 1, 1, 1, layout.ld, layout.halo)
+            sh2 = _lib.ConvShape(B, L, c1, c2, 1, 1, 1, layout.ld, layout.halo)
+            convs += [(sh1, w1, b1), (sh2, w2, b2)]
+        frozen = pack_cache is not None and pack_cache.frozen and not grad_enabled
+        table = packed_all = None
+        if pack_cache is not None and not frozen and os.environ.get("WN_PACK_TABLE", "1") != "0":
+            storages = StackPackTable.dynamic_storages(callers + [bias_total])
+            if storages is not None:
+                key = StackPackTable.key_of(specs, B, layout, prepped, bias_total, convs, storages)
+                table = pack_cache.tables.get(key)
+                if table is None:
+                    table = StackPackTable(lib, specs, B, layout, prepped, bias_total, convs, storages, dev)
+                    if len(pack_cache.tables) >= 8:
+                        pack_cache.tables.clear()
+                    pack_cache.tables[key] = table
+                packed_all = table.run(lib, storages, dev)
+        base = packed_all.data_ptr() if table is not None else 0
+        conv_packed = [base + o for o in table.conv_offsets] if table is not None else \
+            [_pack_conv(lib, sh, w, b, dev) for sh, w, b in convs]
+        ctx.packed_all = packed_all
+
+        ctx.front = None
+        if front is not None:
+            xin = Lease(B, Cin, layout, dev)
+            load_series(xin.t, x.detach(), layout)
+            cur = Lease(B, C0, layout, dev)
+            _lib.check(lib.wn_conv_forward(ctypes.byref(fshape), _p(conv_packed[0]), _p(xin), _p(cur), _stream()), "wn_conv_forward")
+            if training:
+                ctx.front = (xin, conv_packed[0], fshape, tuple(fw.shape), fb is not None)
         else:
-            load_series(cur.t, x.detach(), layout)
-        ms = specs[0].ms
-        S = fresh_series(B, ms, layout, dev)
-        saved, skip_w, skip_b = [], [], []
+            cur = Lease(B, C0, layout, dev)
+            if pool > 1:
+                _lib.check(lib.wn_series_load_pooled(_p(x.detach().contiguous()), _p(cur), B, C0, ctx.in_length, int(pool), layout.ld,
+                                                     layout.halo, _stream()), "wn_series_load_pooled")
+            else:
+                load_series(cur.t, x.detach(), layout)
+
+        series_head = head is not None and training and n <= _lib.MAX_STACK_GROUP
+        S = None if series_head else fresh_series(B, ms, layout, dev)
+        saved = []
         zbuf = None
         for l, spec in enumerate(specs):
-            if spec.ms != ms:
-                raise RuntimeError("wavenet_speech_amd: all blocks of a stack must share out_dim")
             shape = _shape(spec, B, layout)
-            params = _prep_params(flat[l * PARAMS_PER_BLOCK:(l + 1) * PARAMS_PER_BLOCK], spec)
-            if pack_cache is not None and pack_cache.frozen and not grad_enabled:
+            params = prepped[l]
+            if table is not None:
+                packed = base + table.block_offsets[l]
+            elif frozen:
                 packed = pack_cache.get(l, layout, B)
                 if packed is None:
                     packed = pack_cache.put(l, layout, B, _pack_block(lib, shape, params, dev))
@@ -193,39 +349,83 @@
                                             1, _p(sg), _p(z), _stream()), "wn_block_forward")
             if training:
                 saved.append((cur, sg, z, packed, shape))
-                skip_w.append(params[6])
-                skip_b.append(params[7])
             cur = r
+        groups = [base + o for o in table.skipsum_offsets] if (table is not None and training) else None
+        h0 = Lease(B, ms, layout, dev) if head is not None else None
         if training:
-            _stack_skip_sum(lib, specs, [sv[2] for sv in saved], skip_w, skip_b, S, B, layout, dev)
+            _stack_skip_sum(lib, specs, [sv[2] for sv in saved], skip_w, bias_total, h0 if series_head else S, B, layout, dev,
+                            packed_groups=groups, leaky=head[0] if series_head else None)
         ctx.specs, ctx.saved, ctx.layout, ctx.batch = specs, saved, layout, B
         ctx.param_shapes = [tuple(t.shape) for t in flat]
-        return window(S, ms, layout).clone(memory_format=torch.contiguous_format)
+        ctx.head = None
+        if head is None:
+            return window(S, ms, layout).clone(memory_format=torch.contiguous_format)
+        pk1, pk2 = conv_packed[-2], conv_packed[-1]
+        if not series_head:
+            window(h0.t, ms, layout).copy_(torch.nn.functional.leaky_relu(window(S, ms, layout), head[0]))
+        h1 = Lease(B, c1, layout, dev)
+        _lib.check(lib.wn_conv_forward_series(ctypes.byref(sh1), _p(pk1), _p(h0), _p(h1), ctypes.c_float(head[1]), _stream()),
+                   "wn_conv_forward_series")
+        y = Lease(B, c2, layout, dev)
+        _lib.check(lib.wn_conv_forward(ctypes.byref(sh2), _p(pk2), _p(h1), _p(y), _stream()), "wn_conv_forward")
+        if training:
+            ctx.head = (head, sh1, sh2, pk1, pk2, h0, h1, [tuple(t.shape) for t in head_params])
+        return _own(y.view())
 
     @staticmethod
     @once_differentiable
     @_on_device_of_first_tensor
-    def backward(ctx, d_skips):
+    def backward(ctx, d_out):
         lib = _lib.load()
         specs, layout, B = ctx.specs, ctx.layout, ctx.batch
-        dev = d_skips.device
-        dS = Lease(B, specs[0].ms, layout, dev)
-        load_series(dS.t, d_skips, layout)
+        dev = d_out.device
+        head_grads = []
+        if ctx.head is None:
+            dS = Lease(B, specs[0].ms, layout, dev)
+            load_series(dS.t, d_out, layout)
+        else:
+            (slope1, slope2), sh1, sh2, pk1, pk2, h0, h1, hshapes = ctx.head
+            dY = Lease(B, sh2.out_channels, layout, dev)
+            load_series(dY.t, d_out, layout)
+            dw2, db2 = _conv_wgrad(lib, sh2, h1, dY, hshapes[2], True, dev)
+            dh1 = Lease(B, sh1.out_channels, layout, dev)
+            _lib.check(lib.wn_conv_backward_data_series(ctypes.byref(sh2), _p(pk2), _p(dY), _p(h1), ctypes.c_float(slope2), _p(dh1),
+                                                        _stream()), "wn_conv_backward_data_series")
+            del dY
+            dw1, db1 = _conv_wgrad(lib, sh1, h0, dh1, hshapes[0], True, dev)
+            dS = Lease(B, specs[0].ms, layout, dev)
+            _lib.check(lib.wn_conv_backward_data_series(ctypes.byref(sh1), _p(pk1), _p(dh1), _p(h0), ctypes.c_float(slope1), _p(dS),
+                                                        _stream()), "wn_conv_backward_data_series")
+            del dh1, h0, h1
+            head_grads = [dw1, db1, dw2, db2]
+            ctx.head = None
         dr = None
         grads_flat = [None] * (len(specs) * PARAMS_PER_BLOCK)
         for l in range(len(specs) - 1, -1, -1):
             spec = specs[l]
             x, sg, z, packed, shape = ctx.saved[l]
-            want_dx = l > 0 or ctx.needs_input_grad[0]
+            want_dx = l > 0 or ctx.front is not None or ctx.needs_input_grad[0]
             dx, grads = _block_backward(lib, shape, spec, packed, x, sg, z, dr, dS, want_dx, layout, B, dev)
             grads_flat[l * PARAMS_PER_BLOCK:(l + 1) * PARAMS_PER_BLOCK] = grads
             dr = dx
             ctx.saved[l] = None
-        dx0 = window(dr.t, specs[0].ci, layout).clone(memory_format=torch.contiguous_format) if ctx.needs_input_grad[0] else None
+        front_grads = []
+        if ctx.front is not None:
+            xin, fpk, fshape, wshape, has_bias = ctx.front
+            dw, db = _conv_wgrad(lib, fshape, xin, dr, wshape, has_bias, dev)
+            front_grads = [dw, db]
+            if ctx.needs_input_grad[0]:
+                dxin = Lease(B, fshape.in_channels, layout, dev)
+                _lib.check(lib.wn_conv_backward_data(ctypes.byref(fshape), _p(fpk), _p(dr), _p(dxin), _stream()),
+                           "wn_conv_backward_data")
+                dr = dxin
+            ctx.front = None
+        dx0 = _own(dr.view()) if ctx.needs_input_grad[0] else None
         if dx0 is not None and ctx.pool > 1:
             dx0 = _unpool(lib, dx0, ctx.in_length, ctx.pool)
+        ctx.packed_all = None
         grads_flat = [None if g is None else g.view(shp) for g, shp in zip(grads_flat, ctx.param_shapes)]
-        return (dx0, None, None, None, None) + tuple(grads_flat)
+        return (dx0, None, None, None, None, None, None) + tuple(grads_flat) + tuple(head_grads) + tuple(front_grads)
 
 
 def _unpool(lib, dpooled, length, pool):
@@ -282,9 +482,15 @@
     if precision != "f32":
         from . import functional_half
         return functional_half.residual_stack(x, specs, flat_params, precision, pack_cache, head, front, pool)
-    if head is not None or front is not None:
-        raise ValueError("the fused output block / feature layer exist in the half-precision modes only")
-    return _ResidualStackFn.apply(x, tuple(specs), torch.is_grad_enabled(), pack_cache, int(pool), *flat_params)
+    flat = list(flat_params)
+    hs = fs = None
+    if head is not None:
+        hs = (float(head[0][0]), float(head[0][1]))
+        flat += list(head[1])
+    if front is not None:
+        fs = (int(front[0][0]), int(front[0][1]), bool(front[0][2]))
+        flat += list(front[1])
+    return _ResidualStackFn.apply(x, tuple(specs), torch.is_grad_enabled(), pack_cache, int(pool), hs, fs, *flat)
 
 
 class _ResidualBlockFn(torch.autograd.Function):
diff --git a/wavenet_speech_amd/modules/block.py b/wavenet_speech_amd/modules/block.py
--- a/wavenet_speech_amd/modules/block.py
+++ b/wavenet_speech_amd/modules/block.py
@@ -129,10 +129,12 @@
     import torch.nn as nn
     if head is None or os.environ.get("WN_SERIES_HEAD", "1") == "0":
         return None
-    if precision == "f32" or head_precision(precision) != precision:
+    if head_precision(precision) != precision:
         return None
     mods = list(head)
     if len(mods) != 4 or not (isinstance(mods[0], nn.LeakyReLU) and isinstance(mods[2], nn.LeakyReLU)):
+        return None
+    if precision == "f32" and any(m._forward_pre_hooks or m._forward_hooks for m in mods + [head]):
         return None
     for c in (mods[1], mods[3]):
         if not isinstance(c, nn.Conv1d) or c.kernel_size != (1,) or c.stride != (1,) or c.padding != (0,) or c.groups != 1 \
@@ -167,6 +169,18 @@
     if not (mods[1].negative_slope >= 0 and mods[3].negative_slope >= 0):
         return None
     return (mods[1].negative_slope, mods[3].negative_slope), [c0.weight, c0.bias, c1.weight, c1.bias]
+
+
+def fusable_entry(conv, precision, x):
+    import os
+    from .conv_ops import _DilatedConv1d
+    if precision != "f32" or os.environ.get("WN_SERIES_FRONT", "1") == "0":
+        return None
+    if not isinstance(conv, _DilatedConv1d) or conv.precision != "f32":
+        return None
+    if not isinstance(x, torch.Tensor) or x.dim() != 3 or not x.is_cuda or x.dtype != torch.float32:
+        return None
+    return (conv.kernel_width, conv.dilation, conv.causal), [conv.conv1d.weight, conv.conv1d.bias]
 
 
 def run_stack(out, blocks, bottlenecks, state=None, head=None, front=None, pool=1):
diff --git a/wavenet_speech_amd/modules/wavenet.py b/wavenet_speech_amd/modules/wavenet.py
--- a/wavenet_speech_amd/modules/wavenet.py
+++ b/wavenet_speech_amd/modules/wavenet.py
@@ -3,7 +3,7 @@
 import torch.nn.functional as F
 
 from .. import functional as HF
-from .block import ResidualBlock, StackState, run_stack, pointwise_precision, head_precision
+from .block import ResidualBlock, StackState, run_stack, pointwise_precision, head_precision, fusable_entry
 from .conv_ops import CausalConv1d
 from .pointwise import run_sequential
 
@@ -43,11 +43,12 @@
         return self._after_entry(out)
 
     def forward(self, signal):
-        out = self.entry_conv1d(signal)
-        return self._after_entry(out)
+        front = fusable_entry(self.entry_conv1d, self.stack_state.precision, signal)
+        out = signal if front is not None else self.entry_conv1d(signal)
+        return self._after_entry(out, front)
 
-    def _after_entry(self, out):
-        skips_sum, done = run_stack(out, self.convolutions, self.bottlenecks, self.stack_state, head=self.output_stack)
+    def _after_entry(self, out, front=None):
+        skips_sum, done = run_stack(out, self.convolutions, self.bottlenecks, self.stack_state, head=self.output_stack, front=front)
         output_seq = skips_sum if done else run_sequential(self.output_stack, skips_sum, head_precision(self.stack_state.precision))
         if not self.softmax:
             return output_seq
```

Result: faster. 100.3 samples/s (median of 6 runs) (+1.1%).
